# NazirNayal8/RbA

Measured on AMD Instinct MI355X. Metric: images/sec @1024x2048 Swin-B-1dl (RbA inference hot path), higher is better.
Workload: dtype f32 (f16x3 split-MFMA GEMMs, fp32 accumulate)

## Files before the change

include/rba_hip.h:

```cpp
#ifndef RBA_HIP_H
#define RBA_HIP_H

#include <stdint.h>

#ifdef __cplusplus
extern "C" {
#endif

int rba_hip_version(void);

int rba_set_concurrent_streams(int n);

int rba_reduce_f32(const float* mask, const float* cls_prob, float* rba, float* sem_seg, int32_t* argmax,
                   int Q, int K, int64_t HW, int score_mode, void* stream);

int rba_reduce_ws_f32(const float* mask, const float* cls_prob, float* rba, float* sem_seg, int32_t* argmax, int Q, int K,
                      int64_t HW, int score_mode, void* workspace, void* stream);

int rba_reduce_up4_f32(const float* mask_lowres, const float* cls_prob, float* rba, float* sem_seg,
                       int32_t* argmax, int Q, int K, int h, int w, int crop_h, int crop_w, int score_mode, void* stream);

int rba_reduce_bwd_workspace_f32(int Q, int K, int64_t HW, int64_t* bytes);
int rba_reduce_bwd_f32(const float* mask, const float* cls_prob, const float* grad_score,
                       float* grad_mask , float* grad_prob ,
                       int Q, int K, int64_t HW, int score_mode,
                       void* workspace, int64_t workspace_bytes, void* stream);

int rba_sem_seg_bwd_f32(const float* mask, const float* cls_prob, const float* grad_sem ,
                        float* grad_mask , float* grad_prob ,
                        int Q, int K, int64_t HW, void* workspace, int64_t workspace_bytes, void* stream);

int rba_resample_bilinear_f32(const float* in, const float* add, float* out, int C, int h, int w, int H, int W,
                              void* stream);

int rba_ms_deform_attn_fwd_f32(const float* value, const int64_t* spatial_shapes, const int64_t* level_start_index,
                               const float* sampling_loc, const float* attn_weight, float* out,
                               int N, int S, int M, int D, int L, int Lq, int P, void* stream);
int rba_ms_deform_attn_fwd_f64(const double* value, const int64_t* spatial_shapes, const int64_t* level_start_index,
                               const double* sampling_loc, const double* attn_weight, double* out,
                               int N, int S, int M, int D, int L, int Lq, int P, void* stream);

int rba_ms_deform_attn_bwd_f32(const float* value, const int64_t* spatial_shapes, const int64_t* level_start_index,
                               const float* sampling_loc, const float* attn_weight, const float* grad_out,
                               float* grad_value, float* grad_sampling_loc, float* grad_attn_weight,
                               int N, int S, int M, int D, int L, int Lq, int P, void* stream);
int rba_ms_deform_attn_bwd_f64(const double* value, const int64_t* spatial_shapes, const int64_t* level_start_index,
                               const double* sampling_loc, const double* attn_weight, const double* grad_out,
                               double* grad_value, double* grad_sampling_loc, double* grad_attn_weight,
                               int N, int S, int M, int D, int L, int Lq, int P, void* stream);

int rba_msda_prepare_f32(const float* raw, const float* reference_points, const int64_t* spatial_shapes, float* loc, float* attw,
                         int64_t rows, int M, int L, int P, void* stream);

int rba_msda_fused_f32(const float* value, const int64_t* spatial_shapes, const int64_t* level_start_index, const float* raw,
                       const float* reference_points, float* out, int N, int S, int M, int D, int L, int Lq, int P, void* stream);

int64_t rba_masked_xattn_workspace_bytes(int B, int Q, int S, int nH);
int rba_masked_xattn_f32(const float* q, const float* k, const float* v, const float* mask_logits, float* out,
                         float* workspace, int B, int Q, int S, int nH, int hd, void* stream);

int rba_mask_logits_f32(const float* embed, const float* feat, float* out, int B, int Q, int C, int64_t N,
                        void* stream);
int rba_mask_logits_f16x3_f32(const float* embed, const float* feat, float* out, int B, int Q, int C, int64_t N,
                              void* stream);

int rba_mask_logits_bwd_workspace_f32(int B, int Q, int C, int64_t N, int64_t* bytes);
int rba_mask_logits_bwd_f32(const float* embed, const float* feat, const float* grad_out,
                            float* grad_embed , float* grad_feat ,
                            int B, int Q, int C, int64_t N, void* workspace, int64_t workspace_bytes, void* stream);

int rba_point_sample_f32(const float* planes, const int64_t* plane_index , const float* coords, float* out,
                         int64_t num_planes, int N, int h, int w, int P, int shared_coords, void* stream);

int rba_mask_point_loss_fwd_f32(const float* pred_masks, const int64_t* plane_index, const float* coords, const float* labels,
                                float* sums, float* losses, int64_t num_planes, int N, int h, int w, int P, float num_masks, void* stream);
int rba_mask_point_loss_bwd_f32(const float* pred_masks, const int64_t* plane_index, const float* coords, const float* labels,
                                const float* sums, const float* grad_loss_mask , const float* grad_loss_dice ,
                                float* grad_masks, int64_t num_planes, int N, int h, int w, int P, float num_masks, void* stream);

int rba_match_cost_workspace_f32(int Q, int T, int P, int64_t* bytes);
int rba_match_cost_f32(const float* pred_masks, const float* tgt_masks, const float* coords, const float* cls_prob, const int64_t* tgt_ids,
                       float* cost, int Q, int T, int P, int h, int w, int H, int W, int K1, float w_mask, float w_class, float w_dice,
                       void* workspace, int64_t workspace_bytes, void* stream);

int rba_outlier_tail_workspace_f32(int B, int H, int W, int64_t* bytes);
int rba_outlier_tail_fwd_f32(const float* score, const void* labels, int label_bytes , int B, int h, int w, int H, int W, int func,
                             float thr_in, float thr_out, float* workspace, float* loss ,
                             float* stats , void* stream);
int rba_outlier_tail_bwd_f32(const float* score, const void* labels, int label_bytes, int B, int h, int w, int H, int W, int func,
                             float thr_in, float thr_out, const float* stats, const float* grad_loss ,
                             float* grad_score , void* stream);

int rba_dense_hybrid_loss_workspace_f32(int B, int H, int W, int64_t* bytes);
int rba_dense_hybrid_loss_fwd_f32(const float* sem, const float* ood, const void* labels, int label_bytes , int B, int K, int h, int w,
                                  int H, int W, float beta, float* workspace, float* losses , float* stats ,
                                  float* lse , void* stream);
int rba_dense_hybrid_loss_bwd_f32(const float* sem, const float* ood, const void* labels, int label_bytes, const float* lse, int B, int K, int h,
                                  int w, int H, int W, float beta, const float* stats, const float* grad_loss ,
                                  float* grad_sem , float* grad_ood , void* stream);

int rba_gambler_loss_workspace_f32(int B, int H, int W, int64_t* bytes);
int rba_gambler_loss_fwd_f32(const float* sem, const void* labels, int label_bytes , int B, int K, int h, int w, int H, int W,
                             float ood_reg, float* workspace, float* reward , float* losses , float* stats ,
                             float* R , void* stream);
int rba_gambler_loss_bwd_f32(const float* sem, const void* labels, int label_bytes, const float* R, int B, int K, int h, int w, int H, int W,
                             float ood_reg, const float* stats, const float* grad_loss , float* grad_R ,
                             float* grad_reward , float* grad_sem , void* stream);

int rba_gaussian_blur_planes_f32(const float* in, float* out, int B, int H, int W, int kernel_size, float sigma, void* stream);
int rba_gaussian_blur_planes_adjoint_f32(const float* grad_out, float* grad_in, int B, int H, int W, int kernel_size, float sigma, void* stream);

int rba_score_reg_workspace_f32(int B, int h, int w, int H, int W, int64_t* bytes);
int rba_score_reg_fwd_f32(const float* score, const void* labels , int label_bytes, int B, int h, int w, int H, int W, float* workspace,
                          float* losses , float* stats , void* stream);
int rba_score_reg_bwd_f32(const float* score, const void* labels , int label_bytes, int B, int h, int w, int H, int W,
                          const float* stats, const float* grad_smooth , const float* grad_sparse ,
                          float* grad_score , void* stream);

int rba_swin_window_attn_f32(const float* qkv, const float* qkv_bias, const float* bias, const float* bias_frag,
                             float* out, int B, int H, int W, int nH, int hd, int ws, int shift, void* stream);
int64_t rba_swin_bias_fragments_elems(int nH, int ws);
int rba_swin_bias_fragments_f32(const float* bias, float* frag, int nH, int ws, void* stream);

int64_t rba_group_norm_workspace_bytes(int B, int C, int HW, int G);
int rba_group_norm_f32(const float* x, const float* gamma, const float* beta, float* y, float* workspace,
                       int B, int C, int HW, int G, float eps, int relu, void* stream);

int64_t rba_group_norm_nhwc_workspace_bytes(int B, int P, int C, int G);
int rba_group_norm_nhwc_f32(const float* x, const float* gamma, const float* beta, float* y, float* workspace, int B, int P, int C,
                            int G, float eps, int relu, void* stream);
int rba_resample_bilinear_nhwc_f32(const float* in, const float* add, float* out, int C, int h, int w, int H, int W, void* stream);

int rba_add_layer_norm_f32(const float* x, const float* t, const float* t_bias, const float* gamma, const float* beta,
                           float* sum_out, float* y, int64_t rows, int C, float eps, void* stream);

int rba_merge_layer_norm_f32(const float* x, const float* gamma, const float* beta, float* y, int B, int H, int W, int Cin, float eps,
                             void* stream);

int rba_skinny_linear_f32(const float* x, const float* weight, const float* bias, float* out, int M, int N, int K,
                          int relu, void* stream);
int rba_skinny_linear_add_f32(const float* x, const float* x_add, int add_cols, const float* weight, const float* bias, float* out,
                              int M, int N, int K, int relu, int seg_n, void* stream);

int rba_split_weight_bf16x3(const float* weight, void* packed, int N, int K, void* stream);
int rba_split_linear_f32(const float* x, const void* weight_packed, const float* bias, float* out, int64_t M, int N, int K,
                         int act, void* stream);

int rba_split_weight_f16x2(const float* weight, void* packed, int N, int K, void* stream);
int rba_split_linear_f16x3_f32(const float* x, const void* weight_packed, const float* bias, float* out, int64_t M, int N, int K,
                               int act, void* stream);
int rba_split_linear_f16x3_res_f32(const float* x, const void* weight_packed, const float* bias, const float* residual, float* out,
                                   int64_t M, int N, int K, void* stream);

int rba_add_layer_norm_frag_f32(const float* x, const float* t, const float* t_bias, const float* gamma, const float* beta,
                                float* sum_out, void* y_frag, int64_t rows, int C, float eps, void* stream);
int rba_split_linear_f16x3_frag_f32(const void* x_frag, const void* weight_packed, const float* bias, const float* residual, float* out,
                                    int64_t M, int N, int K, int act, void* stream);
int rba_swin_window_attn_split_out_f32(const float* qkv, const float* qkv_bias, const float* bias_frag, void* out_frag, int B, int H, int W,
                                       int nH, int hd, int ws, int shift, void* stream);
int rba_swin_attn_block_supported(int C, int ws);
int64_t rba_swin_attn_block_weight_bytes(int C);
int rba_swin_attn_block_pack_f32(const float* qkv_weight, const float* proj_weight, void* image, int C, void* stream);
int rba_swin_attn_block_f32(float* x, float* y2, const float* norm1_weight, const float* norm1_bias, float eps1, const void* weight_image,
                            const float* qkv_bias, const float* bias_frag, const float* proj_bias, const float* norm2_weight,
                            const float* norm2_bias, float eps2, int B, int H, int W, int C, int ws, int shift, void* stream);
int rba_swin_attn_qkv_supported(int C, int ws);
int rba_swin_attn_qkv_split_out_f32(const float* x, void* out_frag, const float* norm1_weight, const float* norm1_bias, float eps1,
                                    const void* weight_image, const float* qkv_bias, const float* bias_frag, int B, int H, int W, int C, int ws,
                                    int shift, void* stream);
int rba_resample_bilinear_nhwc_split_out_f32(const float* in, const float* add, void* out_frag, int C, int h, int w, int H, int W,
                                             int64_t row0, void* stream);

int rba_resample_bilinear_nhwc_gn_f32(const float* in, const float* in_mr, const float* in_gamma, const float* in_beta, int in_relu,
                                      const float* add, const float* add_mr, const float* add_gamma, const float* add_beta, void* out,
                                      int split_out, int C, int G, int h, int w, int H, int W, int64_t row0, void* stream);
int rba_group_norm_nhwc_stats_f32(const float* x, float* mr, float* workspace, int B, int P, int C, int G, float eps, void* stream);
int rba_conv3x3_nhwc_f16x3_split_in_f32(const void* x_frag, const void* weight_packed, const float* bias, float* out, int B, int H, int W,
                                        int C, int N, void* stream);
int rba_swin_mlp_fused_f16x3_f32(const float* x, const void* w1_packed, const float* b1, const void* w2_packed, const float* b2,
                                 const float* residual, float* out, int64_t M, int C, int HID, void* stream);
int rba_swin_mlp_fused_ln_f16x3_f32(float* x, const float* norm_weight, const float* norm_bias, float eps, const void* w1_packed, const float* b1,
                                    const void* w2_packed, const float* b2, int64_t M, int C, int HID, void* stream);
int rba_split_linear_f16x3_gelu_split_out(const void* x, int x_is_split, const void* weight_packed, const float* bias, void* out_frag,
                                          int64_t M, int N, int K, void* stream);

int rba_split_linear_nchw_out_f32(const float* x, const void* weight_packed, const float* bias, float* out, int64_t M, int N,
                                  int K, int rows_per_image, void* stream);

int rba_split_linear_nchw_out_f16x3_f32(const float* x, const void* weight_packed, const float* bias, float* out, int64_t M, int N, int K,
                                        int rows_per_image, void* stream);

int rba_split_linear_nchw_out_gn_f16x3_f32(const float* x, const float* mr, const float* gamma, const float* beta, int G, int relu,
                                           const void* weight_packed, const float* bias, float* out, int64_t M, int N, int K,
                                           int rows_per_image, void* stream);

int rba_split_linear_nchw_out_gn_rows_f16x3_f32(const float* x, const float* mr, const float* gamma, const float* beta, int G, int relu,
                                                const void* weight_packed, int64_t weight_image_stride, const float* bias,
                                                int bias_image_stride, const int32_t* row_index, float* out, int B, int P, int R, int N,
                                                int K, void* stream);
int rba_compose_query_operand_f16x2(const float* embed, const float* weight, const float* bias, void* packed, float* bias_q, int B, int Q,
                                    int C, int K, void* stream);

int rba_conv3x3_nhwc_f32(const float* x, const void* weight_packed, const float* bias, float* out, int B, int H, int W, int C,
                         int N, void* stream);

int rba_conv3x3_nhwc_f16x3_f32(const float* x, const void* weight_packed, const float* bias, float* out, int B, int H, int W, int C,
                               int N, void* stream);

int rba_split_linear_f16x3_gn_moments_f32(const float* x, const void* weight_packed, const float* bias, float* out, int64_t M, int N, int K,
                                          int rows_per_image, int G, float* moments, void* stream);
int rba_conv3x3_nhwc_f16x3_split_in_gn_moments_f32(const void* x_frag, const void* weight_packed, const float* bias, float* out, int B, int H,
                                                   int W, int C, int N, int G, float* moments, void* stream);
int rba_group_norm_nhwc_merge_f32(const float* moments, float* mr, int B, int G, int splits, float eps, void* stream);

int rba_patch_im2col_u8(const uint8_t* image, float* out, int h, int w, int Hp, int Wp, const float* mean, const float* std, void* stream);
int rba_patch_im2col_f32(const float* image, float* out, int h, int w, int Hp, int Wp, const float* mean, const float* std, void* stream);

int rba_gaussian_blur_f32(const float* in, float* out, int H, int W, int kernel_size, float sigma, void* stream);

int rba_quad_mean_f32(const float* v, float* out, int64_t rows, int S, void* stream);
int rba_softmax_drop_last_f32(const float* logits, float* prob, int64_t rows, int K1, void* stream);

int rba_threshold_u8(const float* score, uint8_t* out, int64_t n, float threshold, void* stream);
int rba_morph3x3_u8(const uint8_t* in, uint8_t* out, int H, int W, int dilate, void* stream);
int rba_ccl4_roots_i32(const uint8_t* mask, int32_t* roots, int H, int W, void* stream);

int rba_bn_relu_conv1x1_f32(const float* x, const float* scale, const float* shift, const float* weight, const float* bias, float* out,
                            int B, int C, int O, int64_t P, void* stream);
int rba_resample_bilinear_ac_f32(const float* x, float* out, int C, int h, int w, int H, int W, void* stream);

typedef struct {
  const float* x_add;
  const void* packed;
  const float* bias;
  float* out;
  int N;
  int ld_out;
  int act;
} rba_token_linear_problem;
int rba_token_linear_pack_f16x2(const float* weight, void* packed, int N, int K, void* stream);
int rba_token_linear_f32(const float* x, const float* x_add, const void* packed, const float* bias, const float* residual,
                         const float* ln_weight, const float* ln_bias, float ln_eps, float* out, int64_t M, int N, int K, int act,
                         void* stream);
int rba_token_linear_multi_f32(const float* x, const rba_token_linear_problem* problems, int n_problems, int64_t M, int K, void* stream);

#define RBA_TTA_MAX_VIEWS 16
typedef struct {
  const float* sem[RBA_TTA_MAX_VIEWS];
  int h[RBA_TTA_MAX_VIEWS];
  int w[RBA_TTA_MAX_VIEWS];
  int flip[RBA_TTA_MAX_VIEWS];
} rba_tta_views;
int rba_tta_merge_f32(const rba_tta_views* views , int A, int K, int H, int W, int score_mode, float* score, float* sem_seg ,
                      int32_t* argmax , void* stream);

int rba_resize_u8_pil_bilinear(const uint8_t* in , uint8_t* out , uint8_t* tmp , int C, int h, int w,
                               int H, int W, const int32_t* kx, const int32_t* bx, int ksize_x, const int32_t* ky, const int32_t* by, int ksize_y,
                               int flip, void* stream);

int rba_confusion_accum(const int32_t* pred, const void* gt, int gt_bytes , int64_t n_pixels, int K,
                        int ignore_label , const uint8_t* lut , int64_t* conf ,
                        int64_t* bad , void* stream);

typedef struct {
  int enabled;
  int brightness;
  float beta;
  int order;
  int contrast;
  float contrast_alpha;
  int saturation;
  float saturation_alpha;
  int hue;
  int hue_delta;
} rba_train_view_color;
typedef struct {
  const uint8_t* img;
  const uint8_t* lab;
  const uint8_t* lut;
  const uint8_t* obj;
  const uint8_t* objmask;
  const int32_t* kx;
  const int32_t* bx;
  const int32_t* ky;
  const int32_t* by;
  const int32_t* ny;
  const int32_t* nx;
  uint8_t* image;
  int64_t* sem_seg;
  int64_t* outlier_mask;
  int32_t* hist;
  int h, w, bh, bw, py, px, new_h, new_w, ksize_x, ksize_y, y0, x0, ch, cw, flip, pad_h, pad_w, ignore_label, ood_label;
  rba_train_view_color color;
} rba_train_view;
int rba_train_view_u8(const rba_train_view* view , void* stream);

#ifdef __cplusplus
}
#endif
#endif
```

rba_amd/_lib.py:

```python
import ctypes
import os

_HERE = os.path.dirname(os.path.abspath(__file__))
LIB_PATH = os.environ.get("RBA_HIP_LIB") or os.path.join(_HERE, "csrc", "librba_hip.so")
KNOBS_LIB_PATH = os.path.join(_HERE, "csrc", "librba_hip_knobs.so")

_i = ctypes.c_int
_i64 = ctypes.c_int64
_vp = ctypes.c_void_p

SIGNATURES = {
    "rba_hip_version": [],
    "rba_set_concurrent_streams": [_i],
    "rba_reduce_f32": [_vp, _vp, _vp, _vp, _vp, _i, _i, _i64, _i, _vp],
    "rba_reduce_ws_f32": [_vp, _vp, _vp, _vp, _vp, _i, _i, _i64, _i, _vp, _vp],
    "rba_reduce_up4_f32": [_vp, _vp, _vp, _vp, _vp, _i, _i, _i, _i, _i, _i, _i, _vp],
    "rba_reduce_bwd_workspace_f32": [_i, _i, _i64, _vp],
    "rba_reduce_bwd_f32": [_vp, _vp, _vp, _vp, _vp, _i, _i, _i64, _i, _vp, _i64, _vp],
    "rba_sem_seg_bwd_f32": [_vp, _vp, _vp, _vp, _vp, _i, _i, _i64, _vp, _i64, _vp],
    "rba_resample_bilinear_f32": [_vp, _vp, _vp, _i, _i, _i, _i, _i, _vp],
    "rba_ms_deform_attn_fwd_f32": [_vp, _vp, _vp, _vp, _vp, _vp, _i, _i, _i, _i, _i, _i, _i, _vp],
    "rba_ms_deform_attn_fwd_f64": [_vp, _vp, _vp, _vp, _vp, _vp, _i, _i, _i, _i, _i, _i, _i, _vp],
    "rba_ms_deform_attn_bwd_f32": [_vp, _vp, _vp, _vp, _vp, _vp, _vp, _vp, _vp, _i, _i, _i, _i, _i, _i, _i, _vp],
    "rba_ms_deform_attn_bwd_f64": [_vp, _vp, _vp, _vp, _vp, _vp, _vp, _vp, _vp, _i, _i, _i, _i, _i, _i, _i, _vp],
    "rba_msda_prepare_f32": [_vp, _vp, _vp, _vp, _vp, _i64, _i, _i, _i, _vp],
    "rba_resample_bilinear_nhwc_gn_f32": [_vp, _vp, _vp, _vp, _i, _vp, _vp, _vp, _vp, _vp, _i, _i, _i, _i, _i, _i, _i, _i64, _vp],
    "rba_group_norm_nhwc_stats_f32": [_vp, _vp, _vp, _i, _i, _i, _i, ctypes.c_float, _vp],
    "rba_msda_fused_f32": [_vp, _vp, _vp, _vp, _vp, _vp, _i, _i, _i, _i, _i, _i, _i, _vp],
    "rba_masked_xattn_workspace_bytes": [_i, _i, _i, _i],
    "rba_masked_xattn_f32": [_vp, _vp, _vp, _vp, _vp, _vp, _i, _i, _i, _i, _i, _vp],
    "rba_mask_logits_f32": [_vp, _vp, _vp, _i, _i, _i, _i64, _vp],
    "rba_mask_logits_f16x3_f32": [_vp, _vp, _vp, _i, _i, _i, _i64, _vp],
    "rba_mask_logits_bwd_workspace_f32": [_i, _i, _i, _i64, _vp],
    "rba_mask_logits_bwd_f32": [_vp, _vp, _vp, _vp, _vp, _i, _i, _i, _i64, _vp, _i64, _vp],
    "rba_point_sample_f32": [_vp, _vp, _vp, _vp, _i64, _i, _i, _i, _i, _i, _vp],
    "rba_mask_point_loss_fwd_f32": [_vp, _vp, _vp, _vp, _vp, _vp, _i64, _i, _i, _i, _i, ctypes.c_float, _vp],
    "rba_mask_point_loss_bwd_f32": [_vp, _vp, _vp, _vp, _vp, _vp, _vp, _vp, _i64, _i, _i, _i, _i, ctypes.c_float, _vp],
    "rba_match_cost_workspace_f32": [_i, _i, _i, _vp],
    "rba_match_cost_f32": [_vp, _vp, _vp, _vp, _vp, _vp, _i, _i, _i, _i, _i, _i, _i, _i, ctypes.c_float, ctypes.c_float, ctypes.c_float, _vp, _i64, _vp],
    "rba_outlier_tail_workspace_f32": [_i, _i, _i, _vp],
    "rba_outlier_tail_fwd_f32": [_vp, _vp, _i, _i, _i, _i, _i, _i, _i, ctypes.c_float, ctypes.c_float, _vp, _vp, _vp, _vp],
    "rba_outlier_tail_bwd_f32": [_vp, _vp, _i, _i, _i, _i, _i, _i, _i, ctypes.c_float, ctypes.c_float, _vp, _vp, _vp, _vp],
    "rba_dense_hybrid_loss_workspace_f32": [_i, _i, _i, _vp],
    "rba_dense_hybrid_loss_fwd_f32": [_vp, _vp, _vp, _i, _i, _i, _i, _i, _i, _i, ctypes.c_float, _vp, _vp, _vp, _vp, _vp],
    "rba_dense_hybrid_loss_bwd_f32": [_vp, _vp, _vp, _i, _vp, _i, _i, _i, _i, _i, _i, ctypes.c_float, _vp, _vp, _vp, _vp, _vp],
    "rba_gambler_loss_workspace_f32": [_i, _i, _i, _vp],
    "rba_gambler_loss_fwd_f32": [_vp, _vp, _i, _i, _i, _i, _i, _i, _i, ctypes.c_float, _vp, _vp, _vp, _vp, _vp, _vp],
    "rba_gambler_loss_bwd_f32": [_vp, _vp, _i, _vp, _i, _i, _i, _i, _i, _i, ctypes.c_float, _vp, _vp, _vp, _vp, _vp, _vp],
    "rba_gaussian_blur_planes_f32": [_vp, _vp, _i, _i, _i, _i, ctypes.c_float, _vp],
    "rba_gaussian_blur_planes_adjoint_f32": [_vp, _vp, _i, _i, _i, _i, ctypes.c_float, _vp],
    "rba_score_reg_workspace_f32": [_i, _i, _i, _i, _i, _vp],
    "rba_score_reg_fwd_f32": [_vp, _vp, _i, _i, _i, _i, _i, _i, _vp, _vp, _vp, _vp],
    "rba_score_reg_bwd_f32": [_vp, _vp, _i, _i, _i, _i, _i, _i, _vp, _vp, _vp, _vp, _vp],
    "rba_tta_merge_f32": [_vp, _i, _i, _i, _i, _i, _vp, _vp, _vp, _vp],
    "rba_resize_u8_pil_bilinear": [_vp, _vp, _vp, _i, _i, _i, _i, _i, _vp, _vp, _i, _vp, _vp, _i, _i, _vp],
    "rba_confusion_accum": [_vp, _vp, _i, _i64, _i, _i, _vp, _vp, _vp, _vp],
    "rba_train_view_u8": [_vp, _vp],
    "rba_swin_window_attn_f32": [_vp, _vp, _vp, _vp, _vp, _i, _i, _i, _i, _i, _i, _i, _vp],
    "rba_swin_window_attn_split_out_f32": [_vp, _vp, _vp, _vp, _i, _i, _i, _i, _i, _i, _i, _vp],
    "rba_swin_bias_fragments_elems": [_i, _i],
    "rba_swin_attn_block_supported": [_i, _i],
    "rba_swin_attn_block_weight_bytes": [_i],
    "rba_swin_attn_qkv_supported": [_i, _i],
    "rba_swin_attn_qkv_split_out_f32": [_vp, _vp, _vp, _vp, ctypes.c_float, _vp, _vp, _vp, _i, _i, _i, _i, _i, _i, _vp],
    "rba_swin_attn_block_pack_f32": [_vp, _vp, _vp, _i, _vp],
    "rba_swin_attn_block_f32": [_vp, _vp, _vp, _vp, ctypes.c_float, _vp, _vp, _vp, _vp, _vp, _vp, ctypes.c_float, _i, _i, _i, _i, _i, _i, _vp],
    "rba_swin_bias_fragments_f32": [_vp, _vp, _i, _i, _vp],
    "rba_skinny_linear_f32": [_vp, _vp, _vp, _vp, _i, _i, _i, _i, _vp],
    "rba_skinny_linear_add_f32": [_vp, _vp, _i, _vp, _vp, _vp, _i, _i, _i, _i, _i, _vp],
    "rba_split_weight_bf16x3": [_vp, _vp, _i, _i, _vp],
    "rba_split_linear_f32": [_vp, _vp, _vp, _vp, _i64, _i, _i, _i, _vp],
    "rba_split_weight_f16x2": [_vp, _vp, _i, _i, _vp],
    "rba_split_linear_f16x3_f32": [_vp, _vp, _vp, _vp, _i64, _i, _i, _i, _vp],
    "rba_split_linear_f16x3_res_f32": [_vp, _vp, _vp, _vp, _vp, _i64, _i, _i, _vp],
    "rba_split_linear_f16x3_frag_f32": [_vp, _vp, _vp, _vp, _vp, _i64, _i, _i, _i, _vp],
    "rba_swin_mlp_fused_f16x3_f32": [_vp, _vp, _vp, _vp, _vp, _vp, _vp, _i64, _i, _i, _vp],
    "rba_swin_mlp_fused_ln_f16x3_f32": [_vp, _vp, _vp, ctypes.c_float, _vp, _vp, _vp, _vp, _i64, _i, _i, _vp],
    "rba_split_linear_f16x3_gelu_split_out": [_vp, _i, _vp, _vp, _vp, _i64, _i, _i, _vp],
    "rba_split_linear_nchw_out_f32": [_vp, _vp, _vp, _vp, _i64, _i, _i, _i, _vp],
    "rba_split_linear_nchw_out_f16x3_f32": [_vp, _vp, _vp, _vp, _i64, _i, _i, _i, _vp],
    "rba_split_linear_f16x3_gn_moments_f32": [_vp, _vp, _vp, _vp, _i64, _i, _i, _i, _i, _vp, _vp],
    "rba_conv3x3_nhwc_f16x3_split_in_gn_moments_f32": [_vp, _vp, _vp, _vp, _i, _i, _i, _i, _i, _i, _vp, _vp],
    "rba_group_norm_nhwc_merge_f32": [_vp, _vp, _i, _i, _i, ctypes.c_float, _vp],
    "rba_split_linear_nchw_out_gn_f16x3_f32": [_vp, _vp, _vp, _vp, _i, _i, _vp, _vp, _vp, _i64, _i, _i, _i, _vp],
    "rba_split_linear_nchw_out_gn_rows_f16x3_f32": [_vp, _vp, _vp, _vp, _i, _i, _vp, _i64, _vp, _i, _vp, _vp, _i, _i, _i, _i, _i, _vp],
    "rba_compose_query_operand_f16x2": [_vp, _vp, _vp, _vp, _vp, _i, _i, _i, _i, _vp],
    "rba_conv3x3_nhwc_f32": [_vp, _vp, _vp, _vp, _i, _i, _i, _i, _i, _vp],
    "rba_conv3x3_nhwc_f16x3_f32": [_vp, _vp, _vp, _vp, _i, _i, _i, _i, _i, _vp],
    "rba_conv3x3_nhwc_f16x3_split_in_f32": [_vp, _vp, _vp, _vp, _i, _i, _i, _i, _i, _vp],
    "rba_resample_bilinear_nhwc_split_out_f32": [_vp, _vp, _vp, _i, _i, _i, _i, _i, _i64, _vp],
    "rba_patch_im2col_u8": [_vp, _vp, _i, _i, _i, _i, _vp, _vp, _vp],
    "rba_patch_im2col_f32": [_vp, _vp, _i, _i, _i, _i, _vp, _vp, _vp],
    "rba_group_norm_nhwc_workspace_bytes": [_i, _i, _i, _i],
    "rba_group_norm_nhwc_f32": [_vp, _vp, _vp, _vp, _vp, _i, _i, _i, _i, ctypes.c_float, _i, _vp],
    "rba_resample_bilinear_nhwc_f32": [_vp, _vp, _vp, _i, _i, _i, _i, _i, _vp],
    "rba_bn_relu_conv1x1_f32": [_vp, _vp, _vp, _vp, _vp, _vp, _i, _i, _i, _i64, _vp],
    "rba_resample_bilinear_ac_f32": [_vp, _vp, _i, _i, _i, _i, _i, _vp],
    "rba_gaussian_blur_f32": [_vp, _vp, _i, _i, _i, ctypes.c_float, _vp],
    "rba_quad_mean_f32": [_vp, _vp, _i64, _i, _vp],
    "rba_softmax_drop_last_f32": [_vp, _vp, _i64, _i, _vp],
    "rba_threshold_u8": [_vp, _vp, _i64, ctypes.c_float, _vp],
    "rba_morph3x3_u8": [_vp, _vp, _i, _i, _i, _vp],
    "rba_ccl4_roots_i32": [_vp, _vp, _i, _i, _vp],
    "rba_add_layer_norm_f32": [_vp, _vp, _vp, _vp, _vp, _vp, _vp, _i64, _i, ctypes.c_float, _vp],
    "rba_add_layer_norm_frag_f32": [_vp, _vp, _vp, _vp, _vp, _vp, _vp, _i64, _i, ctypes.c_float, _vp],
    "rba_merge_layer_norm_f32": [_vp, _vp, _vp, _vp, _i, _i, _i, _i, ctypes.c_float, _vp],
    "rba_group_norm_workspace_bytes": [_i, _i, _i, _i],
    "rba_group_norm_f32": [_vp, _vp, _vp, _vp, _vp, _i, _i, _i, _i, ctypes.c_float, _i, _vp],
    "rba_token_linear_pack_f16x2": [_vp, _vp, _i, _i, _vp],
    "rba_token_linear_f32": [_vp, _vp, _vp, _vp, _vp, _vp, _vp, ctypes.c_float, _vp, _i64, _i, _i, _i, _vp],
    "rba_token_linear_multi_f32": [_vp, _vp, _i, _i64, _i, _vp],
}

class TokenLinearProblem(ctypes.Structure):
    _fields_ = [("x_add", ctypes.c_void_p), ("packed", ctypes.c_void_p), ("bias", ctypes.c_void_p), ("out", ctypes.c_void_p),
                ("N", ctypes.c_int), ("ld_out", ctypes.c_int), ("act", ctypes.c_int)]


TTA_MAX_VIEWS = 16


class TtaViews(ctypes.Structure):
    _fields_ = [("sem", ctypes.c_void_p * TTA_MAX_VIEWS), ("h", ctypes.c_int * TTA_MAX_VIEWS), ("w", ctypes.c_int * TTA_MAX_VIEWS),
                ("flip", ctypes.c_int * TTA_MAX_VIEWS)]


class TrainViewColor(ctypes.Structure):
    _fields_ = [("enabled", ctypes.c_int), ("brightness", ctypes.c_int), ("beta", ctypes.c_float), ("order", ctypes.c_int),
                ("contrast", ctypes.c_int), ("contrast_alpha", ctypes.c_float), ("saturation", ctypes.c_int), ("saturation_alpha", ctypes.c_float),
                ("hue", ctypes.c_int), ("hue_delta", ctypes.c_int)]


TRAIN_VIEW_POINTERS = ("img", "lab", "lut", "obj", "objmask", "kx", "bx", "ky", "by", "ny", "nx", "image", "sem_seg", "outlier_mask", "hist")
TRAIN_VIEW_INTS = ("h", "w", "bh", "bw", "py", "px", "new_h", "new_w", "ksize_x", "ksize_y", "y0", "x0", "ch", "cw", "flip", "pad_h", "pad_w",
                   "ignore_label", "ood_label")


class TrainView(ctypes.Structure):
    _fields_ = ([(n, ctypes.c_void_p) for n in TRAIN_VIEW_POINTERS] + [(n, ctypes.c_int) for n in TRAIN_VIEW_INTS] + [("color", TrainViewColor)])


EXPECTED_ABI = 191

_lib = None


class RbaHipError(RuntimeError):
    pass


def load():
    global _lib
    if _lib is not None:
        return _lib
    _lib = _open(LIB_PATH)
    return _lib


_handles = {}


def _open(path):
    if path in _handles:
        return _handles[path]
    import torch
    if not os.path.exists(path):
        raise RbaHipError(
            f"{path} not found: build it with `python -m rba_amd.csrc.build` (hipcc --offload-arch=gfx950; --knobs for the knobs build). "
            "rba_amd has no CPU or PyTorch fallback for its HIP kernels.")
    lib = ctypes.CDLL(path)
    for name, argtypes in SIGNATURES.items():
        try:
            fn = getattr(lib, name)
        except AttributeError as e:
            raise RbaHipError(f"{path} does not export {name}; rebuild it") from e
        fn.argtypes = argtypes
        fn.restype = ctypes.c_int64 if name.endswith(("_bytes", "_elems")) else ctypes.c_int
    abi = int(lib.rba_hip_version())
    if abi != EXPECTED_ABI:
        raise RbaHipError(f"{path} has ABI version {abi}, these bindings are written for {EXPECTED_ABI}; rebuild it "
                          "(python -m rba_amd.csrc.build)")
    _handles[path] = lib
    return lib


class use_library:

    def __init__(self, path):
        self.path = path

    def __enter__(self):
        global _lib
        self.prev = _lib
        _lib = _open(self.path)
        return _lib

    def __exit__(self, *exc):
        global _lib
        _lib = self.prev
        return False


def knob(name):
    try:
        return ctypes.c_int.in_dll(load(), name)
    except ValueError as e:
        raise RbaHipError(f"{name} is a compile-time constant in the product library: run on the knobs build (RBA_HIP_LIB={KNOBS_LIB_PATH} or "
                          "rba_amd._lib.use_library(KNOBS_LIB_PATH); python -m rba_amd.csrc.build --knobs)") from e


def hip_error_string(code: int) -> str:
    try:
        hip = ctypes.CDLL("libamdhip64.so")
        hip.hipGetErrorString.restype = ctypes.c_char_p
        hip.hipGetErrorString.argtypes = [ctypes.c_int]
        return hip.hipGetErrorString(code).decode()
    except Exception:
        return "hipError"


def check(code: int, what: str):
    if code != 0:
        raise RbaHipError(f"{what} failed: hipError {code} ({hip_error_string(code)})")
```

rba_amd/csrc/build.py:

```python
import os
import subprocess
import sys
from concurrent.futures import ThreadPoolExecutor

HERE = os.path.dirname(os.path.abspath(__file__))
SOURCES = ["rba_reduce.hip", "rba_reduce_bwd.hip", "resample.hip", "ms_deform_attn.hip", "ms_deform_attn_bwd.hip", "masked_xattn.hip", "mask_logits.hip", "mask_logits_bwd.hip", "point_loss.hip", "outlier_tail.hip", "dense_hybrid_loss.hip", "pebal_loss.hip", "tta_merge.hip", "resize_u8.hip", "confusion.hip", "train_view.hip",
           "swin_window_attn.hip", "swin_attn_block.hip", "group_norm.hip", "layer_norm.hip", "skinny_linear.hip", "split_linear.hip", "split_linear_dma.hip", "split_linear_gnf.hip", "gaussian_blur.hip", "open_panoptic.hip", "dense_hybrid.hip", "patch_embed.hip", "token_linear.hip", "decoder_small.hip"]
HEADERS = ["common.h", "knobs.h", "bilinear_ac.h", "rba_reduce_kernels.h", "split_linear_dma.h", "split_linear_h3.h", "split_linear_h3q.h", "mlp_fused_h3.h", "swin_window_attn_h3.h", "swin_attn_block.h",
           os.path.join("..", "..", "include", "rba_hip.h")]
TUNE_SOURCES = [os.path.join("tune", "rba_reduce_tune.hip"), os.path.join("tune", "split_linear_tune.hip"), os.path.join("tune", "split_linear_ws.hip"), os.path.join("tune", "mlp_fused_h1.hip"), os.path.join("tune", "k5_timing.hip"), os.path.join("tune", "k5_wpe_ab.hip"), os.path.join("tune", "k5_wpe_plain.hip"), os.path.join("tune", "k5_persist.hip"), os.path.join("tune", "k7_timing.hip")] + [os.path.join("tune", f"gnf_form{f}_dbg{d}.hip") for f in (0, 1) for d in (0, 1)] + [os.path.join("tune", "gnf_form0_dbg1_unpacked.hip"), os.path.join("tune", "gnf_form1_dbg0_unpacked.hip")]
TUNE_LIB = os.path.join(HERE, "tune", "librba_tune.so")
LIB = os.path.join(HERE, "librba_hip.so")
KNOBS_LIB = os.path.join(HERE, "librba_hip_knobs.so")
KNOBS = ["-DRBA_TUNE_KNOBS"]
OBJ = os.path.join(HERE, "build")
HIPCC = os.environ.get("HIPCC", "/opt/rocm/bin/hipcc")
FLAGS = ["--offload-arch=gfx950", "-O3", "-std=c++17", "-fPIC", "-ffp-contract=fast", "-Wno-unused-result"]
NO_PACKED_FP32 = ["-Xclang", "-target-feature", "-Xclang", "-packed-fp32-ops"]
MFMA_SOURCES = ({"split_linear.hip", "split_linear_dma.hip", "mask_logits.hip", "mask_logits_bwd.hip", "masked_xattn.hip", "skinny_linear.hip"}
                if os.environ.get("RBA_NO_PACKED_FP32") == "1" else set())
UNPACKED_ALWAYS = {"split_linear_gnf.hip", "ms_deform_attn_bwd.hip", "point_loss.hip", "outlier_tail.hip", "dense_hybrid_loss.hip"}
UNPACKED_SOURCES = MFMA_SOURCES | UNPACKED_ALWAYS


def _run(cmd):
    r = subprocess.run(cmd, cwd=HERE, stderr=subprocess.PIPE, text=True)
    err = "\n".join(ln for ln in r.stderr.splitlines() if "not a recognized feature for this target" not in ln)
    if err.strip():
        print(err, file=sys.stderr, flush=True)
    if r.returncode:
        raise subprocess.CalledProcessError(r.returncode, cmd)


def _stale(target, deps) -> bool:
    if not os.path.exists(target):
        return True
    t = os.path.getmtime(target)
    return any(os.path.getmtime(d) > t for d in deps)


def stale() -> bool:
    return _stale(LIB, [os.path.join(HERE, f) for f in SOURCES + HEADERS])


def build(force: bool = False, verbose: bool = True, knobs: bool = False) -> str:
    lib = KNOBS_LIB if knobs else LIB
    if not force and not _stale(lib, [os.path.join(HERE, f) for f in SOURCES + HEADERS]):
        return lib
    obj_dir = os.path.join(OBJ, "knobs") if knobs else OBJ
    os.makedirs(obj_dir, exist_ok=True)
    hdrs = [os.path.join(HERE, h) for h in HEADERS]

    def compile_one(src):
        s, o = os.path.join(HERE, src), os.path.join(obj_dir, src.replace(".hip", ".o"))
        if force or _stale(o, [s] + hdrs):
            cmd = [HIPCC] + FLAGS + (KNOBS if knobs else []) + (NO_PACKED_FP32 if src in UNPACKED_SOURCES else []) + ["-c", s, "-o", o]
            if verbose:
                print(" ".join(cmd), flush=True)
            _run(cmd)
        return o

    with ThreadPoolExecutor(max_workers=min(8, os.cpu_count() or 1)) as ex:
        objs = list(ex.map(compile_one, SOURCES))
    _link_and_gate(objs, lib, verbose)
    return lib


def _link_and_gate(objs, lib, verbose):
    tmp = lib + ".unscanned"
    cmd = [HIPCC, "--offload-arch=gfx950", "-shared", "-fPIC"] + objs + ["-o", tmp]
    if verbose:
        print(" ".join(cmd), flush=True)
    subprocess.run(cmd, check=True, cwd=HERE)
    try:
        from . import isa_hazards
    except ImportError:
        sys.path.insert(0, HERE)
        import isa_hazards
    try:
        r = isa_hazards.gate(tmp)
    except Exception:
        os.remove(tmp)
        raise
    if verbose:
        print(f"isa_hazards: {os.path.basename(lib)}: {r['code_objects']} code objects clean (rules D, T, P)", flush=True)
    os.replace(tmp, lib)


def build_knobs(force: bool = False, verbose: bool = True) -> str:
    return build(force=force, verbose=verbose, knobs=True)


def build_tune(force: bool = False, verbose: bool = True) -> str:
    deps = [os.path.join(HERE, f) for f in TUNE_SOURCES + HEADERS + [os.path.join("tune", "split_linear_experiments.h"), os.path.join("tune", "rba_reduce_experiments.h")]]
    if not force and not _stale(TUNE_LIB, deps):
        return TUNE_LIB
    os.makedirs(OBJ, exist_ok=True)
    objs = []
    for src in TUNE_SOURCES:
        o = os.path.join(OBJ, "tune_" + os.path.basename(src).replace(".hip", ".o"))
        cmd = [HIPCC] + FLAGS + KNOBS + (NO_PACKED_FP32 if (MFMA_SOURCES and "split_linear" in src) or src.endswith("split_linear_ws.hip") or src.endswith("_unpacked.hip") or (src.endswith("mlp_fused_h1.hip") and os.environ.get("RBA_MLP1_UNPACKED") == "1") else []) + ["-c", os.path.join(HERE, src), "-o", o]
        if verbose:
            print(" ".join(cmd), flush=True)
        _run(cmd)
        objs.append(o)
    cmd = [HIPCC, "--offload-arch=gfx950", "-shared", "-fPIC"] + objs + ["-o", TUNE_LIB]
    if verbose:
        print(" ".join(cmd), flush=True)
    subprocess.run(cmd, check=True, cwd=HERE)
    return TUNE_LIB


if __name__ == "__main__":
    print(build(force="--force" in sys.argv))
    if "--knobs" in sys.argv:
        print(build_knobs(force="--force" in sys.argv))
    if "--tune" in sys.argv:
        print(build_tune(force="--force" in sys.argv))
```

rba_amd/csrc/layer_norm.hip:

```cpp
#include "common.h"
#include "../../include/rba_hip.h"

namespace {

struct MergeGeom {
  int H, W, Cin;
};

template <int G, int NV, bool MERGE = false, bool FRAG = false, int WAVES = 4>
__global__ __launch_bounds__(64 * WAVES) void add_layer_norm_kernel(const float* x, const float* __restrict__ t,
                                                             const float* __restrict__ tb, const float* __restrict__ gamma,
                                                             const float* __restrict__ beta, float* sum_out ,
                                                             float* __restrict__ y, int64_t rows, int C, float eps,
                                                             MergeGeom mg = MergeGeom{0, 0, 0}) {
  constexpr int RPW = 64 / G;
  const int lane = threadIdx.x & 63, sub = lane % G, rsel = lane / G;
  const int64_t row = ((int64_t)blockIdx.x * WAVES + (threadIdx.x >> 6)) * RPW + rsel;
  constexpr bool TR = FRAG && WAVES == 8 && G == 64;
  __shared__ __attribute__((aligned(16))) rba_u32x4 tr_lds[TR ? NV * 64 * 8 : 1];
  const bool rvalid = row < rows;
  const int64_t base = (rvalid ? row : 0) * C;
  const int nv4 = C >> 2;
  int mi = 0, mj = 0;
  int64_t mb = 0;
  if (MERGE) {
    const int H2 = (mg.H + 1) >> 1, W2 = (mg.W + 1) >> 1;
    const int64_t r = rvalid ? row : 0;
    const int64_t bimg = r / ((int64_t)H2 * W2);
    const int rem = (int)(r - bimg * H2 * W2);
    mi = rem / W2;
    mj = rem - mi * W2;
    mb = bimg * mg.H * mg.W;
  }
  constexpr bool EARLY = NV <= 2;
  f32x4 v[NV], g4[EARLY ? NV : 1], b4[EARLY ? NV : 1];
  float sum = 0.f;
#pragma unroll
  for (int j = 0; j < (EARLY ? NV : 0); ++j) {
    const int c4 = sub + j * G;
    g4[j] = b4[j] = (f32x4){0.f, 0.f, 0.f, 0.f};
    if (c4 < nv4) {
      g4[j] = *reinterpret_cast<const f32x4*>(gamma + 4 * c4);
      b4[j] = *reinterpret_cast<const f32x4*>(beta + 4 * c4);
    }
  }
#pragma unroll
  for (int j = 0; j < NV; ++j) {
    const int c4 = sub + j * G;
    f32x4 a = {0.f, 0.f, 0.f, 0.f};
    if (c4 < nv4) {
      if (MERGE) {
        const int seg = (4 * c4) / mg.Cin, off = 4 * c4 - seg * mg.Cin;
        const int si = 2 * mi + (seg & 1), sj = 2 * mj + (seg >> 1);
        if (si < mg.H && sj < mg.W) a = *reinterpret_cast<const f32x4*>(x + (mb + (int64_t)si * mg.W + sj) * mg.Cin + off);
      } else {
        a = *reinterpret_cast<const f32x4*>(x + base + 4 * c4);
      }
      if (t) a += *reinterpret_cast<const f32x4*>(t + base + 4 * c4);
      if (tb) a += *reinterpret_cast<const f32x4*>(tb + 4 * c4);
      sum += (a.x + a.y) + (a.z + a.w);
    }
    v[j] = a;
  }
#pragma unroll
  for (int o = G / 2; o > 0; o >>= 1) sum += __shfl_xor(sum, o, RBA_WAVE);
  const float mean = sum / (float)C;
  float sq = 0.f;
#pragma unroll
  for (int j = 0; j < NV; ++j) {
    const int c4 = sub + j * G;
    if (c4 < nv4) {
      const f32x4 d = v[j] - mean;
      sq += (d.x * d.x + d.y * d.y) + (d.z * d.z + d.w * d.w);
    }
  }
#pragma unroll
  for (int o = G / 2; o > 0; o >>= 1) sq += __shfl_xor(sq, o, RBA_WAVE);
  const float rstd = 1.0f / sqrtf(sq / (float)C + eps);
  if (!TR && !rvalid) return;
#pragma unroll
  for (int j = 0; j < NV; ++j) {
    const int c4 = sub + j * G;
    if (c4 < nv4) {
      if (sum_out && rvalid) *reinterpret_cast<f32x4*>(sum_out + base + 4 * c4) = v[j];
      const f32x4 gj = EARLY ? g4[EARLY ? j : 0] : *reinterpret_cast<const f32x4*>(gamma + 4 * c4);
      const f32x4 bj = EARLY ? b4[EARLY ? j : 0] : *reinterpret_cast<const f32x4*>(beta + 4 * c4);
      const f32x4 o = (v[j] - mean) * rstd * gj + bj;
      if (FRAG) {
        uint32_t h[2], l[2];
        rba_split_f16x2(o.x, o.y, h[0], l[0]);
        rba_split_f16x2(o.z, o.w, h[1], l[1]);
        const bool odd = c4 & 1;
        const uint32_t s0 = odd ? h[0] : l[0], s1 = odd ? h[1] : l[1];
        const uint32_t r0 = __builtin_amdgcn_mov_dpp(s0, 0xB1, 0xf, 0xf, true), r1 = __builtin_amdgcn_mov_dpp(s1, 0xB1, 0xf, 0xf, true);
        const rba_u32x4 piece = odd ? (rba_u32x4){r0, r1, l[0], l[1]} : (rba_u32x4){h[0], h[1], r0, r1};
        const int k8 = c4 >> 1;
        if (TR) {
          const int pcol = (((k8 >> 2) * 4 + (k8 & 1) * 2 + (odd ? 1 : 0)) << 1) + ((k8 >> 1) & 1);
          const int r8 = threadIdx.x >> 6;
          tr_lds[pcol * 8 + (r8 ^ (pcol & 7))] = piece;
        } else {
          const int64_t off = ((row >> 5) * (int64_t)(C >> 5) + (k8 >> 2)) * 4096 + ((k8 & 1) * 2 + (odd ? 1 : 0)) * 1024 +
                              (((k8 >> 1) & 1) * 32 + (int)(row & 31)) * 16;
          *reinterpret_cast<rba_u32x4*>(reinterpret_cast<char*>(y) + off) = piece;
        }
      } else {
        *reinterpret_cast<f32x4*>(y + base + 4 * c4) = o;
      }
    }
  }
  if (TR) {
    __syncthreads();
    const int64_t row0 = (int64_t)blockIdx.x * 8;
    char* img = reinterpret_cast<char*>(y) + ((row0 >> 5) * (int64_t)(C >> 5)) * 4096 + (int)(row0 & 31) * 16;
    const int npc = nv4;
    for (int u = threadIdx.x; u < npc * 8; u += 64 * WAVES) {
      const int pcol = u >> 3, r8 = u & 7;
      const int x = pcol >> 1;
      if (row0 + r8 < rows)
        *reinterpret_cast<rba_u32x4*>(img + (int64_t)(x >> 2) * 4096 + (x & 3) * 1024 + (pcol & 1) * 512 + r8 * 16) = tr_lds[pcol * 8 + (r8 ^ (pcol & 7))];
    }
  }
}

template <int G, int NV, bool FRAG = false>
int launch(const float* x, const float* t, const float* tb, const float* gamma, const float* beta, float* sum_out, float* y,
           int64_t rows, int C, float eps, hipStream_t st) {
  const int64_t rpb = 4 * (64 / G);
  const int64_t blocks = (rows + rpb - 1) / rpb;
  if (blocks > 0x7fffffffLL) return (int)hipErrorInvalidValue;
  hipLaunchKernelGGL((add_layer_norm_kernel<G, NV, false, FRAG>), dim3((unsigned)blocks), dim3(256), 0, st, x, t, tb, gamma, beta, sum_out, y,
                     rows, C, eps);
  return rba_launch_status();
}

template <int NV>
int launch_frag8(const float* x, const float* t, const float* tb, const float* gamma, const float* beta, float* sum_out, float* y,
                 int64_t rows, int C, float eps, hipStream_t st) {
  const int64_t blocks = (rows + 7) / 8;
  if (blocks > 0x7fffffffLL) return (int)hipErrorInvalidValue;
  hipLaunchKernelGGL((add_layer_norm_kernel<64, NV, false, true, 8>), dim3((unsigned)blocks), dim3(512), 0, st, x, t, tb, gamma, beta, sum_out,
                     y, rows, C, eps);
  return rba_launch_status();
}

template <int G, int NV>
int launch_merge(const float* x, const float* gamma, const float* beta, float* y, int64_t rows, int C, float eps, MergeGeom mg,
                 hipStream_t st) {
  const int64_t rpb = 4 * (64 / G);
  const int64_t blocks = (rows + rpb - 1) / rpb;
  if (blocks > 0x7fffffffLL) return (int)hipErrorInvalidValue;
  hipLaunchKernelGGL((add_layer_norm_kernel<G, NV, true>), dim3((unsigned)blocks), dim3(256), 0, st, x, nullptr, nullptr, gamma, beta, nullptr,
                     y, rows, C, eps, mg);
  return rba_launch_status();
}

}

extern "C" int rba_merge_layer_norm_f32(const float* x, const float* gamma, const float* beta, float* y, int B, int H, int W, int Cin,
                                        float eps, void* stream) {
  RBA_CHECK_ARG(B >= 0 && H >= 1 && W >= 1 && Cin >= 4 && Cin % 4 == 0 && 4 * Cin <= 8192);
  if (B == 0) return 0;
  RBA_CHECK_ARG(x && gamma && beta && y);
  RBA_CHECK_ARG((((uintptr_t)x | (uintptr_t)gamma | (uintptr_t)beta | (uintptr_t)y) & 15) == 0);
  rba_begin();
  hipStream_t st = (hipStream_t)stream;
  const int C = 4 * Cin, nv4 = C / 4;
  const int64_t rows = (int64_t)B * ((H + 1) / 2) * ((W + 1) / 2);
  const MergeGeom mg{H, W, Cin};
#define RBA_L(G, NV) return launch_merge<G, NV>(x, gamma, beta, y, rows, C, eps, mg, st)
  if (nv4 <= 16) RBA_L(16, 1);
  if (nv4 <= 32) RBA_L(32, 1);
  if (nv4 <= 64) RBA_L(64, 1);
  if (nv4 <= 128) RBA_L(64, 2);
  if (nv4 <= 256) RBA_L(64, 4);
  if (nv4 <= 512) RBA_L(64, 8);
  if (nv4 <= 1024) RBA_L(64, 16);
  RBA_L(64, 32);
#undef RBA_L
}

extern "C" int rba_add_layer_norm_f32(const float* x, const float* t, const float* t_bias, const float* gamma, const float* beta,
                                      float* sum_out, float* y, int64_t rows, int C, float eps, void* stream) {
  RBA_CHECK_ARG(rows >= 0 && C >= 4 && C % 4 == 0 && C <= 8192);
  if (rows == 0) return 0;
  RBA_CHECK_ARG(x && gamma && beta && y);
  RBA_CHECK_ARG((((uintptr_t)x | (uintptr_t)t | (uintptr_t)t_bias | (uintptr_t)gamma | (uintptr_t)beta | (uintptr_t)sum_out |
                  (uintptr_t)y) & 15) == 0);
  rba_begin();
  hipStream_t st = (hipStream_t)stream;
  const int nv4 = C / 4;
#define RBA_L(G, NV) return launch<G, NV>(x, t, t_bias, gamma, beta, sum_out, y, rows, C, eps, st)
  if (nv4 <= 16) RBA_L(16, 1);
  if (nv4 <= 32) RBA_L(32, 1);
  if (nv4 <= 64) RBA_L(64, 1);
  if (nv4 <= 128) RBA_L(64, 2);
  if (nv4 <= 256) RBA_L(64, 4);
  if (nv4 <= 512) RBA_L(64, 8);
  if (nv4 <= 1024) RBA_L(64, 16);
  RBA_L(64, 32);
#undef RBA_L
}

extern "C" int rba_add_layer_norm_frag_f32(const float* x, const float* t, const float* t_bias, const float* gamma, const float* beta,
                                           float* sum_out, void* y_frag, int64_t rows, int C, float eps, void* stream) {
  RBA_CHECK_ARG(rows >= 0 && C >= 32 && C % 32 == 0 && C <= 8192);
  if (rows == 0) return 0;
  RBA_CHECK_ARG(x && gamma && beta && y_frag);
  RBA_CHECK_ARG((((uintptr_t)x | (uintptr_t)t | (uintptr_t)t_bias | (uintptr_t)gamma | (uintptr_t)beta | (uintptr_t)sum_out |
                  (uintptr_t)y_frag) & 15) == 0);
  rba_begin();
  hipStream_t st = (hipStream_t)stream;
  const int nv4 = C / 4;
  float* y = reinterpret_cast<float*>(y_frag);
  if (nv4 > 64 && nv4 <= 128) return launch_frag8<2>(x, t, t_bias, gamma, beta, sum_out, y, rows, C, eps, st);
  if (nv4 > 128 && nv4 <= 256) return launch_frag8<4>(x, t, t_bias, gamma, beta, sum_out, y, rows, C, eps, st);
  if (nv4 > 256 && nv4 <= 512) return launch_frag8<8>(x, t, t_bias, gamma, beta, sum_out, y, rows, C, eps, st);
#define RBA_L(G, NV) return launch<G, NV, true>(x, t, t_bias, gamma, beta, sum_out, y, rows, C, eps, st)
  if (nv4 <= 16) RBA_L(16, 1);
  if (nv4 <= 32) RBA_L(32, 1);
  if (nv4 <= 64) RBA_L(64, 1);
  if (nv4 <= 128) RBA_L(64, 2);
  if (nv4 <= 256) RBA_L(64, 4);
  if (nv4 <= 512) RBA_L(64, 8);
  if (nv4 <= 1024) RBA_L(64, 16);
  RBA_L(64, 32);
#undef RBA_L
}
```

rba_amd/csrc/split_linear_gnf.hip:

```cpp
#include "split_linear_h3.h"

extern "C" int rba_split_linear_nchw_out_gn_f16x3_f32(const float* x, const float* mr, const float* gamma, const float* beta, int G, int relu,
                                                      const void* weight_packed, const float* bias, float* out, int64_t M, int N, int K,
                                                      int rows_per_image, void* stream) {
  RBA_CHECK_ARG(N >= 1 && rows_per_image >= 1 && G >= 1 && (K % G) == 0 && ((K / G) % 4) == 0);
  RBA_GEMM_PROLOGUE(M, K, x && mr && gamma && beta && weight_packed && out && (M % rows_per_image) == 0 && (rows_per_image % 128) == 0, x, weight_packed, out,
                    gamma, beta);
  H3Args a{x, reinterpret_cast<const u32x4_t*>(weight_packed), bias, out, M, N, K, (hipStream_t)stream};
  a.rows_per_image = rows_per_image;
  a.gn = GnFold{mr, gamma, beta, G, K / G, relu ? 1 : 0};
  return rba_gemm_status(h3_wide(M, N) ? launch_h3l<0, 4, H3_NCHW | H3_GNF>(a) : launch_h3l<0, 2, H3_NCHW | H3_GNF>(a));
}

extern "C" int rba_split_linear_nchw_out_gn_rows_f16x3_f32(const float* x, const float* mr, const float* gamma, const float* beta, int G, int relu,
                                                           const void* weight_packed, int64_t weight_image_stride, const float* bias, int bias_image_stride,
                                                           const int32_t* row_index, float* out, int B, int P, int R, int N, int K, void* stream) {
  RBA_CHECK_ARG(B >= 0 && N >= 1 && P >= 1 && R >= 1 && G >= 1 && (K % G) == 0 && ((K / G) % 4) == 0);
  RBA_CHECK_ARG(weight_image_stride >= 0 && (weight_image_stride % 16) == 0 && bias_image_stride >= 0 && (row_index || R == P));
  const int64_t M = (int64_t)B * R;
  RBA_GEMM_PROLOGUE(M, K, x && mr && gamma && beta && weight_packed && out && (P % 128) == 0 && (R % 128) == 0 && (int64_t)P * K < (int64_t)1 << 30, x,
                    weight_packed, out, gamma, beta);
  H3Args a{x, reinterpret_cast<const u32x4_t*>(weight_packed), bias, out, M, N, K, (hipStream_t)stream};
  a.rows_per_image = R;
  a.gn = GnFold{mr, gamma, beta, G, K / G, relu ? 1 : 0};
  a.rw = H3Rows{row_index, P, bias_image_stride, weight_image_stride};
  const bool per_image = weight_image_stride != 0 || bias_image_stride != 0, wide = h3_wide(M, N);
  constexpr unsigned F = H3_NCHW | H3_GNF;
  if (row_index && per_image) return rba_gemm_status(wide ? launch_h3l<0, 4, F | H3_ROWIDX | H3_PERIMG>(a) : launch_h3l<0, 2, F | H3_ROWIDX | H3_PERIMG>(a));
  if (row_index) return rba_gemm_status(wide ? launch_h3l<0, 4, F | H3_ROWIDX>(a) : launch_h3l<0, 2, F | H3_ROWIDX>(a));
  if (per_image) return rba_gemm_status(wide ? launch_h3l<0, 4, F | H3_PERIMG>(a) : launch_h3l<0, 2, F | H3_PERIMG>(a));
  return rba_gemm_status(wide ? launch_h3l<0, 4, F>(a) : launch_h3l<0, 2, F>(a));
}
```

rba_amd/csrc/split_linear_h3.h:

```cpp
#pragma once
#include <type_traits>

#include "split_linear_dma.h"

RBA_KNOB_EXTERN(rba_k6_stagger, 0);

namespace {

typedef _Float16 f16x8_t __attribute__((ext_vector_type(8)));

__device__ __forceinline__ void split_h3(const f32x4 u, const f32x4 v, f16x8_t& h, f16x8_t& l) {
  const float x[8] = {u.x, u.y, u.z, u.w, v.x, v.y, v.z, v.w};
  u32x4_t hp, lp;
#pragma unroll
  for (int i = 0; i < 4; ++i) {
    uint32_t a, r;
    rba_split_f16x2(x[2 * i], x[2 * i + 1], a, r);
    hp[i] = a;
    lp[i] = r;
  }
  h = __builtin_bit_cast(f16x8_t, hp);
  l = __builtin_bit_cast(f16x8_t, lp);
}

__device__ __forceinline__ f32x2 gelu_erf2(f32x2 v) {
  const f32x2 a = {fabsf(v.x), fabsf(v.y)};
  const f32x2 d = a * 0.23164189f + 1.0f;
  const f32x2 t = {__builtin_amdgcn_rcpf(d.x), __builtin_amdgcn_rcpf(d.y)};
  f32x2 p = t * 0.5307027145f + -0.7265760135f;
  p = p * t + 0.7107068705f;
  p = p * t + -0.142248368f;
  p = p * t + 0.127414796f;
  const f32x2 u = a * 0.8493218003f;
  const f32x2 s = -u * u;
  const f32x2 ex = {__builtin_amdgcn_exp2f(s.x), __builtin_amdgcn_exp2f(s.y)};
  const f32x2 q = p * t * ex;
  const f32x2 r = (v + a) * 0.5f;
  return r - a * q;
}

#ifndef RBA_H3_HELPERS_ONLY
__global__ void split_weight_f16x2_kernel(const float* __restrict__ w, u32x4_t* __restrict__ packed, int N, int K) {
  const int S = K >> 4;
  const int64_t total = (int64_t)((N + 127) >> 7) * S * 256;
  for (int64_t i = (int64_t)blockIdx.x * blockDim.x + threadIdx.x; i < total; i += (int64_t)gridDim.x * blockDim.x) {
    const int slot = (int)(i & 1), r = (int)((i >> 1) & 127);
    const int64_t ts = i >> 8;
    const int s = (int)(ts % S), nt = (int)(ts / S);
    const int h = slot ^ ((r >> 3) & 1);
    const int k0 = 32 * (s >> 1) + 16 * h + 8 * (s & 1);
    const int n = nt * 128 + r;
    f16x8_t p0, p1;
    if (n < N) {
      const f32x4* src = reinterpret_cast<const f32x4*>(w + (int64_t)n * K + k0);
      split_h3(src[0], src[1], p0, p1);
    } else {
#pragma unroll
      for (int e = 0; e < 8; ++e) p0[e] = p1[e] = (_Float16)0.f;
    }
    u32x4_t* dst = packed + ts * 512 + r * 2 + slot;
    dst[0] = __builtin_bit_cast(u32x4_t, p0);
    dst[256] = __builtin_bit_cast(u32x4_t, p1);
  }
}

#endif

struct GnMoments {
  float* ws;
  int G, cpg, P;
};
template <int ACT, int CT, int PROBE, bool RES, bool GNM = false>
__device__ __forceinline__ void h3_epilogue(const f32x16_t (&accm)[CT], const f32x16_t (&accl)[CT], const float* __restrict__ bias,
                                            float* C, const float* R, int M, int N, int m0, int n0, int BM, int BN, int wave, int l31,
                                            int lh, GnMoments gm = GnMoments{nullptr, 1, 1, 128}, float* sh = nullptr) {
  const bool interior = m0 + BM <= M && n0 + BN <= N;
  if (GNM) __syncthreads();
#pragma unroll
  for (int j = 0; j < CT; ++j) {
    const int col = n0 + 32 * j + l31;
    const float bv = (bias && col < N) ? bias[col] : 0.f;
    const int rbase = m0 + 32 * wave + 4 * lh;
    float* dst = C + (int64_t)rbase * N + col;
    f32x16_t res;
    if (RES) {
      const float* src = R + (int64_t)rbase * N + col;
#pragma unroll
      for (int r = 0; r < 16; ++r) {
        const int ro = 8 * (r >> 2) + (r & 3);
        res[r] = (interior || (col < N && rbase + ro < M)) ? src[(int64_t)ro * N] : 0.f;
      }
    }
    f32x16_t v;
#pragma unroll
    for (int r = 0; r < 16; r += 2) {
      f32x2 y = (f32x2){accl[j][r], accl[j][r + 1]} * 0.00048828125f + (f32x2){accm[j][r], accm[j][r + 1]};
      if (RES) y = (f32x2){res[r], res[r + 1]} + y;
      y = y + bv;
      if (ACT == 1) y = gelu_erf2(y);
      if (ACT == 2) y = (f32x2){rba_relu(y.x), rba_relu(y.y)};
      v[r] = y.x;
      v[r + 1] = y.y;
    }
    if (GNM) {
      float sm = 0.f, sq = 0.f;
#pragma unroll
      for (int r = 0; r < 16; ++r) {
        sm += v[r];
        sq = fmaf(v[r], v[r], sq);
      }
      sm += __shfl_xor(sm, 32, 64);
      sq += __shfl_xor(sq, 32, 64);
      for (int o = 1; o < gm.cpg; o <<= 1) {
        sm += __shfl_xor(sm, o, 64);
        sq += __shfl_xor(sq, o, 64);
      }
      if (lh == 0 && (l31 & (gm.cpg - 1)) == 0) {
        float* d = sh + ((wave * (BN / gm.cpg)) + (32 * j + l31) / gm.cpg) * 2;
        d[0] = sm;
        d[1] = sq;
      }
    }
    if (PROBE & 4) {
      float sum = 0.f;
#pragma unroll
      for (int r = 0; r < 16; ++r) sum += v[r];
      if (sum == 1234.5f) dst[0] = sum;
    } else if (interior) {
#pragma unroll
      for (int r = 0; r < 16; ++r) dst[(int64_t)(8 * (r >> 2) + (r & 3)) * N] = v[r];
    } else if (col < N) {
#pragma unroll
      for (int r = 0; r < 16; ++r) {
        const int ro = 8 * (r >> 2) + (r & 3);
        if (rbase + ro < M) dst[(int64_t)ro * N] = v[r];
      }
    }
  }
  if (GNM) {
    __syncthreads();
    const int gpt = BN / gm.cpg, t = 64 * wave + 32 * lh + l31;
    if (t < gpt && m0 < M) {
      double ds = 0, dq = 0;
#pragma unroll
      for (int w = 0; w < 4; ++w) {
        ds += (double)sh[(w * gpt + t) * 2];
        dq += (double)sh[(w * gpt + t) * 2 + 1];
      }
      const double n = 128.0 * gm.cpg, mean = ds / n, m2 = dq - ds * mean;
      const int b = m0 / gm.P, sp = (m0 - b * gm.P) >> 7, splits = gm.P >> 7, g = n0 / gm.cpg + t;
      float* o = gm.ws + (((int64_t)b * gm.G + g) * splits + sp) * 3;
      o[0] = (float)n;
      o[1] = (float)mean;
      o[2] = (float)(m2 > 0 ? m2 : 0);
    }
  }
}

#ifndef RBA_H3_HELPERS_ONLY
template <int CT>
__device__ __forceinline__ void h3_epilogue_nchw(const f32x16_t (&accm)[CT], const f32x16_t (&accl)[CT], const float* __restrict__ bias, float* C,
                                                 int M, int N, int P, int m0, int n0, int wave, int l31, int lh) {
  const bool vec = (P & 3) == 0;
#pragma unroll
  for (int j = 0; j < CT; ++j) {
    const int col = n0 + 32 * j + l31;
    if (col >= N) continue;
    const float bv = bias ? bias[col] : 0.f;
#pragma unroll
    for (int q = 0; q < 4; ++q) {
      const int row = m0 + 32 * wave + 8 * q + 4 * lh;
      if (row >= M) continue;
      f32x4 v;
#pragma unroll
      for (int i = 0; i < 4; ++i) v[i] = fmaf(accl[j][4 * q + i], 0.00048828125f, accm[j][4 * q + i]) + bv;
      if (vec && row + 3 < M) {
        const int b = row / P, p = row - b * P;
        *reinterpret_cast<f32x4*>(C + ((int64_t)b * N + col) * P + p) = v;
      } else {
#pragma unroll
        for (int i = 0; i < 4; ++i)
          if (row + i < M) {
            const int b = (row + i) / P, p = row + i - b * P;
            C[((int64_t)b * N + col) * P + p] = v[i];
          }
      }
    }
  }
}

enum : unsigned {
  H3_TIMING = 1u << 0,
  H3_RES = 1u << 1,
  H3_GNM = 1u << 2,
  H3_CONV = 1u << 3,
  H3_NCHW = 1u << 4,
  H3_GNF = 1u << 5,
  H3_PRE = 1u << 6,
  H3_FOUT = 1u << 7,
  H3_CONVP = 1u << 8,
  H3_OCC1 = 1u << 9,
  H3_KS2 = 1u << 10,
  H3_RS2 = 1u << 11,
  H3_ROWIDX = 1u << 12,
  H3_PERIMG = 1u << 13,
  H3_PROBE_SHIFT = 16,
};
constexpr unsigned h3_probe(int p) { return (unsigned)p << H3_PROBE_SHIFT; }
constexpr int h3_probe_of(unsigned form) { return (int)(form >> H3_PROBE_SHIFT); }
constexpr unsigned H3_FORMS = H3_TIMING | H3_RES, H3L_FORMS = H3_FORMS | H3_GNM | H3_CONV | H3_NCHW | H3_GNF | H3_ROWIDX | H3_PERIMG,
                   H3P_FORMS = H3_FORMS | H3_GNM | H3_PRE | H3_FOUT | H3_CONVP | H3_OCC1 | H3_KS2 | H3_RS2;
constexpr bool h3_form_within(unsigned form, unsigned allowed) { return (form & ~allowed & ((1u << H3_PROBE_SHIFT) - 1)) == 0; }
constexpr int h3_tile_rows(unsigned form) { return (form & H3_RS2) ? 256 : 128; }
constexpr int h3_threads(unsigned form) { return (form & (H3_KS2 | H3_RS2)) ? 512 : 256; }
constexpr int h3_occupancy(unsigned form) { return (form & (H3_KS2 | H3_RS2 | H3_OCC1)) ? 1 : 2; }

template <int ACT, int CT, unsigned FORM = 0>
__global__ __launch_bounds__(256, 2) void split_linear_h3_kernel(const float* __restrict__ A, const u32x4_t* __restrict__ Wp,
                                                                const float* __restrict__ bias, float* C, int M, int N,
                                                                int K, int MT, int NT, unsigned long long* dbg = nullptr,
                                                                const float* R = nullptr) {
  static_assert(h3_form_within(FORM, H3_FORMS), "split_linear_h3_kernel: H3_TIMING, H3_RES, h3_probe()");
  constexpr int PROBE = h3_probe_of(FORM);
  constexpr bool TIMING = FORM & H3_TIMING, RES = FORM & H3_RES;
  unsigned long long tm[4];
  if (TIMING) tm[0] = wall_clock64();
  constexpr int BM = 128, BN = 32 * CT;
  constexpr int SUBW = 4 * BN;
  constexpr int BLK = 2 * SUBW;
  constexpr int UPL = BLK / 256;
  static_assert(BLK % 256 == 0 && 128 % BN == 0, "tile width");
  __shared__ __attribute__((aligned(16))) u32x4_t lds[2 * BLK];

  const int tid = threadIdx.x, lane = tid & 63;
  const int wave = __builtin_amdgcn_readfirstlane(tid >> 6);
  int bid = blockIdx.x;
  const int nb = MT * NT;
  if ((nb & 7) == 0) bid = (bid & 7) * (nb >> 3) + (bid >> 3);
  const int mt = bid / NT, nt = bid - mt * NT;
  const int m0 = mt * BM, n0 = nt * BN;
  const int NB = K >> 5, S16 = K >> 4;
  const int l31 = lane & 31, lh = lane >> 5;

  constexpr int QSTEP = (CT == 4) ? 256 : 512;
  const char* wbase = reinterpret_cast<const char*>(Wp + (int64_t)(n0 >> 7) * S16 * 512 + (n0 & 127) * 2);
  uint32_t woff;
  {
    const int g = tid / SUBW, rem = tid - g * SUBW, p = rem / (2 * BN), rr = rem - p * (2 * BN);
    woff = (uint32_t)(g * 512 + p * 256 + rr) * 16u;
  }
  int row = m0 + 32 * wave + l31;
  row = (row < M ? row : M - 1) - m0;
  const char* xbase = reinterpret_cast<const char*>(A + (int64_t)m0 * K);
  const uint32_t xoff = ((uint32_t)row * (uint32_t)K + 16u * lh) * 4u;

  f32x16_t accm[CT], accl[CT];
#pragma unroll
  for (int j = 0; j < CT; ++j)
#pragma unroll
    for (int r = 0; r < 16; ++r) accm[j][r] = accl[j][r] = 0.f;

  u32x4_t wr[UPL];
  f32x4 xr[2][4];
  const int last = NB - 1;
  auto wload = [&](int c, u32x4_t (&r)[UPL]) {
    const char* src = wbase + (int64_t)(c < last ? c : last) * 16384;
#pragma unroll
    for (int q = 0; q < UPL; ++q) r[q] = *reinterpret_cast<const u32x4_t*>(src + q * (QSTEP * 16) + woff);
  };
  auto xload = [&](int c, f32x4 (&r)[4]) {
    const char* src = xbase + (c < last ? c : last) * 128;
#pragma unroll
    for (int q = 0; q < 4; ++q) r[q] = *reinterpret_cast<const f32x4*>(src + q * 16 + xoff);
  };
  wload(0, wr);
  xload(0, xr[0]);
  xload(1, xr[1]);
#pragma unroll
  for (int q = 0; q < UPL; ++q) lds[tid + 256 * q] = wr[q];
  wload(1, wr);
  asm volatile("s_waitcnt lgkmcnt(0)\n\ts_barrier" ::: "memory");

  const int fb = l31 * 2 + (lh ^ ((l31 >> 3) & 1));
  if (TIMING) tm[1] = wall_clock64();
  auto block = [&](int b, const u32x4_t* img, u32x4_t* nxt, f32x4 (&xc)[4]) {
    if (!(PROBE & 32)) {
#pragma unroll
      for (int q = 0; q < UPL; ++q) nxt[tid + 256 * q] = wr[q];
    }
    if (!(PROBE & 1)) wload(b + 2, wr);
    f16x8_t ah[2], al[2];
    if (PROBE & 16) {
      ah[0] = __builtin_bit_cast(f16x8_t, xc[0]); al[0] = __builtin_bit_cast(f16x8_t, xc[1]);
      ah[1] = __builtin_bit_cast(f16x8_t, xc[2]); al[1] = __builtin_bit_cast(f16x8_t, xc[3]);
    } else {
      split_h3(xc[0], xc[1], ah[0], al[0]);
      split_h3(xc[2], xc[3], ah[1], al[1]);
    }
    if (!(PROBE & 2)) xload(b + 2, xc);
#pragma unroll
    for (int g = 0; g < 2; ++g) {
      __builtin_amdgcn_sched_barrier(0);
      f16x8_t bh[CT], bl[CT];
#pragma unroll
      for (int j = 0; j < CT; ++j) {
        const u32x4_t* im = (PROBE & 8) ? lds : img;
        bh[j] = __builtin_bit_cast(f16x8_t, im[g * SUBW + fb + 64 * j]);
        bl[j] = __builtin_bit_cast(f16x8_t, im[g * SUBW + fb + 2 * BN + 64 * j]);
      }
#pragma unroll
      for (int j = 0; j < CT; ++j) accm[j] = __builtin_amdgcn_mfma_f32_32x32x16_f16(ah[g], bh[j], accm[j], 0, 0, 0);
#pragma unroll
      for (int j = 0; j < CT; ++j) accl[j] = __builtin_amdgcn_mfma_f32_32x32x16_f16(ah[g], bl[j], accl[j], 0, 0, 0);
#pragma unroll
      for (int j = 0; j < CT; ++j) accl[j] = __builtin_amdgcn_mfma_f32_32x32x16_f16(al[g], bh[j], accl[j], 0, 0, 0);
    }
    if (!(PROBE & 64)) asm volatile("s_waitcnt lgkmcnt(0)\n\ts_barrier" ::: "memory");
  };
  int b = 0;
  if (NB & 1) {
    block(0, lds, lds + BLK, xr[0]);
    b = 1;
    for (; b < NB; b += 2) {
      block(b, lds + BLK, lds, xr[1]);
      block(b + 1, lds, lds + BLK, xr[0]);
    }
  } else {
    for (; b < NB; b += 2) {
      block(b, lds, lds + BLK, xr[0]);
      block(b + 1, lds + BLK, lds, xr[1]);
    }
  }

  if (TIMING) tm[2] = wall_clock64();
  h3_epilogue<ACT, CT, PROBE, RES>(accm, accl, bias, C, R, M, N, m0, n0, BM, BN, wave, l31, lh);
  if (TIMING && tid == 0) {
    tm[3] = wall_clock64();
    unsigned xcc;
    asm volatile("s_getreg_b32 %0, hwreg(HW_REG_XCC_ID)" : "=s"(xcc));
    unsigned hw;
    asm volatile("s_getreg_b32 %0, hwreg(HW_REG_HW_ID)" : "=s"(hw));
#pragma unroll
    for (int i = 0; i < 4; ++i) dbg[6 * blockIdx.x + i] = tm[i];
    dbg[6 * blockIdx.x + 4] = xcc;
    dbg[6 * blockIdx.x + 5] = hw;
  }
}

struct ConvShape {
  int H, W, Cin;
};
struct GnFold {
  const float* mr;
  const float* gamma;
  const float* beta;
  int G, cpg, relu;
};
struct H3Rows {
  const int* idx;
  int P;
  int bstride;
  int64_t wstride;
};
template <int ACT, int CT, unsigned FORM = 0>
__global__ __launch_bounds__(256, 2) void split_linear_h3l_kernel(const float* __restrict__ A, const u32x4_t* __restrict__ Wp,
                                                                 const float* __restrict__ bias, float* C, int M, int N,
                                                                 int K, int MT, int NT, unsigned long long* dbg = nullptr,
                                                                 ConvShape cs = ConvShape{0, 0, 0}, const float* R = nullptr, int rows_per_image = 0,
                                                                 GnFold gn = GnFold{nullptr, nullptr, nullptr, 1, 1, 0},
                                                                 GnMoments gm = GnMoments{nullptr, 1, 1, 128}, H3Rows rw = H3Rows{nullptr, 0, 0, 0}) {
  static_assert(h3_form_within(FORM, H3L_FORMS), "split_linear_h3l_kernel: H3_TIMING, H3_RES, H3_GNM, H3_CONV, H3_NCHW, H3_GNF, H3_ROWIDX, H3_PERIMG, h3_probe()");
  constexpr int PROBE = h3_probe_of(FORM);
  constexpr bool TIMING = FORM & H3_TIMING, CONV = FORM & H3_CONV, RES = FORM & H3_RES, NCHW = FORM & H3_NCHW, GNF = FORM & H3_GNF, GNM = FORM & H3_GNM;
  constexpr bool ROWIDX = FORM & H3_ROWIDX, PERIMG = FORM & H3_PERIMG;
  static_assert(!(ROWIDX || PERIMG) || (NCHW && GNF && !CONV && !RES && !GNM), "H3_ROWIDX / H3_PERIMG: forms of the GroupNorm-folded channel-major projection");
  unsigned long long tm[4];
  if (TIMING) tm[0] = wall_clock64();
  constexpr int BM = 128, BN = 32 * CT;
  constexpr int SUBW = 4 * BN;
  constexpr int BLK = 2 * SUBW;
  constexpr int UPL = BLK / 256;
  constexpr int XBLK = BM * 8;
  constexpr int BUF = BLK + XBLK;
  static_assert(BLK % 256 == 0 && 128 % BN == 0, "tile width");
  __shared__ __attribute__((aligned(16))) u32x4_t lds[2 * BUF];

  const int tid = threadIdx.x, lane = tid & 63;
  const int wave = __builtin_amdgcn_readfirstlane(tid >> 6);
  int bid = blockIdx.x;
  const int nb = MT * NT;
  if ((nb & 7) == 0) bid = (bid & 7) * (nb >> 3) + (bid >> 3);
  const int mt = bid / NT, nt = bid - mt * NT;
  const int m0 = mt * BM, n0 = nt * BN;
  const int NB = K >> 5, S16 = K >> 4;
  const int l31 = lane & 31, lh = lane >> 5;

  constexpr int QSTEP = (CT == 4) ? 256 : 512;
  const char* wbase = reinterpret_cast<const char*>(Wp + (int64_t)(n0 >> 7) * S16 * 512 + (n0 & 127) * 2);
  const int img = (ROWIDX || PERIMG) ? m0 / rows_per_image : 0;
  if (PERIMG) {
    wbase += (int64_t)img * rw.wstride;
    if (bias) bias += (int64_t)img * rw.bstride;
  }
  uint32_t woff;
  {
    const int g = tid / SUBW, rem = tid - g * SUBW, p = rem / (2 * BN), rr = rem - p * (2 * BN);
    woff = (uint32_t)(g * 512 + p * 256 + rr) * 16u;
  }
  const char* xbase = reinterpret_cast<const char*>(CONV ? A : ROWIDX ? A + (int64_t)img * rw.P * K : A + (int64_t)m0 * K);
  uint32_t xoff[4];
  int py[4], px[4];
#pragma unroll
  for (int q = 0; q < 4; ++q) {
    int r = m0 + (tid >> 3) + 32 * q;
    r = r < M ? r : M - 1;
    if (CONV) {
      const int pix = r % (cs.H * cs.W);
      py[q] = pix / cs.W;
      px[q] = pix - py[q] * cs.W;
      xoff[q] = ((uint32_t)r * (uint32_t)cs.Cin + 4u * (tid & 7)) * 4u;
    } else if (ROWIDX) {
      int s = rw.idx[r];
      s = s < 0 ? 0 : (s < rw.P ? s : rw.P - 1);
      xoff[q] = ((uint32_t)s * (uint32_t)K + 4u * (tid & 7)) * 4u;
    } else {
      xoff[q] = ((uint32_t)(r - m0) * (uint32_t)K + 4u * (tid & 7)) * 4u;
    }
  }
  const int xdst = BLK + (tid >> 3) * 8 + ((tid & 7) ^ ((tid >> 4) & 7));
  const int frow = 32 * wave + l31;
  const int fa = BLK + frow * 8, fsw = (frow >> 1) & 7;

  f32x16_t accm[CT], accl[CT];
#pragma unroll
  for (int j = 0; j < CT; ++j)
#pragma unroll
    for (int r = 0; r < 16; ++r) accm[j][r] = accl[j][r] = 0.f;

  u32x4_t wr[UPL];
  f32x4 xr[4];
  f32x4 gga = {0.f, 0.f, 0.f, 0.f}, gbe = {0.f, 0.f, 0.f, 0.f};
  float gmean = 0.f, grstd = 0.f;
  const float* gmr = GNF ? gn.mr + (int64_t)(m0 / rows_per_image) * gn.G * 2 : nullptr;
  const int last = NB - 1;
  auto gload = [&](int c) {
    const int cc = c < last ? c : last;
    const char* ws = wbase + (int64_t)cc * 16384;
#pragma unroll
    for (int q = 0; q < UPL; ++q) wr[q] = *reinterpret_cast<const u32x4_t*>(ws + q * (QSTEP * 16) + woff);
    if (GNF) {
      const int ch = cc * 32 + 4 * (tid & 7);
      gga = *reinterpret_cast<const f32x4*>(gn.gamma + ch);
      gbe = *reinterpret_cast<const f32x4*>(gn.beta + ch);
      const int g = ch / gn.cpg;
      gmean = gmr[2 * g];
      grstd = gmr[2 * g + 1];
    }
    if (CONV) {
      const int k0 = cc * 32, tap = k0 / cs.Cin, ch0 = k0 - tap * cs.Cin;
      const int ky = tap / 3, dy = ky - 1, dx = tap - 3 * ky - 1;
      const int delta = ((dy * cs.W + dx) * cs.Cin + ch0) * 4;
#pragma unroll
      for (int q = 0; q < 4; ++q) {
        const bool ok = (unsigned)(py[q] + dy) < (unsigned)cs.H && (unsigned)(px[q] + dx) < (unsigned)cs.W;
        const f32x4 v = *reinterpret_cast<const f32x4*>(xbase + (int64_t)(ok ? delta : ch0 * 4) + xoff[q]);
        xr[q] = ok ? v : (f32x4){0.f, 0.f, 0.f, 0.f};
      }
    } else {
      const char* xs = xbase + cc * 128;
#pragma unroll
      for (int q = 0; q < 4; ++q) xr[q] = *reinterpret_cast<const f32x4*>(xs + xoff[q]);
    }
  };
  f32x4 xst[4];
#if defined(RBA_GNF_DEBUG)
  int gnf_blk = 0;
#endif
  auto lstore = [&](u32x4_t* buf) {
#pragma unroll
    for (int q = 0; q < UPL; ++q) buf[tid + 256 * q] = wr[q];
    if (GNF) {
      f32x4 a, b;
      const float relu_floor = gn.relu ? 0.f : -INFINITY;
      const float poison = (grstd - grstd) + (gmean - gmean);
#pragma unroll
      for (int i = 0; i < 4; ++i) {
        a[i] = gga[i] * grstd;
        b[i] = fmaf(-gmean, a[i], gbe[i]);
      }
#pragma unroll
      for (int q = 0; q < 4; ++q)
#pragma unroll
        for (int i = 0; i < 4; ++i) {
#if defined(RBA_GNF_FORM) && RBA_GNF_FORM == 1
          const float y = fmaf(xr[q][i], a[i], b[i]);
          xst[q][i] = fmaxf(y, relu_floor) + (y - y);
#else
          xst[q][i] = fmaxf(fmaf(xr[q][i], a[i], b[i]), relu_floor) + poison;
#endif
        }
#if defined(RBA_GNF_DEBUG)
      if (dbg && gnf_blk < NB) {
        float* d = reinterpret_cast<float*>(dbg) + (((int64_t)(mt * NT + nt) * NB + gnf_blk) * 256 + tid) * 40;
#pragma unroll
        for (int q = 0; q < 4; ++q) {
          *reinterpret_cast<f32x4*>(d + 4 * q) = xr[q];
          *reinterpret_cast<f32x4*>(d + 16 + 4 * q) = xst[q];
        }
        *reinterpret_cast<f32x4*>(d + 32) = a;
        *reinterpret_cast<f32x4*>(d + 36) = b;
      }
      ++gnf_blk;
#endif
#pragma unroll
      for (int q = 0; q < 4; ++q) buf[xdst + 256 * q] = __builtin_bit_cast(u32x4_t, xst[q]);
    } else {
#pragma unroll
      for (int q = 0; q < 4; ++q) buf[xdst + 256 * q] = __builtin_bit_cast(u32x4_t, xr[q]);
    }
  };
  gload(0);
  lstore(lds);
  gload(1);
  asm volatile("s_waitcnt lgkmcnt(0)\n\ts_barrier" ::: "memory");

  const int fb = l31 * 2 + (lh ^ ((l31 >> 3) & 1));
  if (TIMING) tm[1] = wall_clock64();
  for (int b = 0; b < NB; ++b) {
    const u32x4_t* img = lds + (b & 1) * BUF;
    if (!(PROBE & 32)) lstore(lds + ((b + 1) & 1) * BUF);
    if (!(PROBE & 1)) gload(b + 2);
    f16x8_t ah[2], al[2];
#pragma unroll
    for (int g = 0; g < 2; ++g) {
      const f32x4 u = __builtin_bit_cast(f32x4, img[fa + ((4 * lh + 2 * g) ^ fsw)]);
      const f32x4 v = __builtin_bit_cast(f32x4, img[fa + ((4 * lh + 2 * g + 1) ^ fsw)]);
      if (PROBE & 16) {
        ah[g] = __builtin_bit_cast(f16x8_t, u);
        al[g] = __builtin_bit_cast(f16x8_t, v);
      } else {
        split_h3(u, v, ah[g], al[g]);
      }
    }
#pragma unroll
    for (int g = 0; g < 2; ++g) {
      if (PROBE & 128) __builtin_amdgcn_sched_barrier(0);
      f16x8_t bh[CT], bl[CT];
#pragma unroll
      for (int j = 0; j < CT; ++j) {
        bh[j] = __builtin_bit_cast(f16x8_t, img[g * SUBW + fb + 64 * j]);
        bl[j] = __builtin_bit_cast(f16x8_t, img[g * SUBW + fb + 2 * BN + 64 * j]);
      }
#pragma unroll
      for (int j = 0; j < CT; ++j) accm[j] = __builtin_amdgcn_mfma_f32_32x32x16_f16(ah[g], bh[j], accm[j], 0, 0, 0);
#pragma unroll
      for (int j = 0; j < CT; ++j) accl[j] = __builtin_amdgcn_mfma_f32_32x32x16_f16(ah[g], bl[j], accl[j], 0, 0, 0);
#pragma unroll
      for (int j = 0; j < CT; ++j) accl[j] = __builtin_amdgcn_mfma_f32_32x32x16_f16(al[g], bh[j], accl[j], 0, 0, 0);
    }
    if (!(PROBE & 64)) asm volatile("s_waitcnt lgkmcnt(0)\n\ts_barrier" ::: "memory");
  }

  if (TIMING) tm[2] = wall_clock64();
  if (NCHW) h3_epilogue_nchw<CT>(accm, accl, bias, C, M, N, rows_per_image, m0, n0, wave, l31, lh);
  else h3_epilogue<ACT, CT, PROBE, RES, GNM>(accm, accl, bias, C, R, M, N, m0, n0, BM, BN, wave, l31, lh, gm, reinterpret_cast<float*>(lds));
  if (TIMING && tid == 0) {
    tm[3] = wall_clock64();
#pragma unroll
    for (int i = 0; i < 4; ++i) dbg[6 * blockIdx.x + i] = tm[i];
    dbg[6 * blockIdx.x + 4] = dbg[6 * blockIdx.x + 5] = 0;
  }
}

#endif

template <int ACT, int CT>
__device__ __forceinline__ void h3_epilogue_split(const f32x16_t (&accm)[CT], const f32x16_t (&accl)[CT], const float* __restrict__ bias,
                                                  void* out_frag, int M, int N, int m0, int n0, int wave, int l31, int lh) {
  const int row = m0 + 32 * wave + l31;
  const bool full = m0 + 128 <= M;
  const int NBo = N >> 5;
  char* base = reinterpret_cast<char*>(out_frag) + ((int64_t)((m0 >> 5) + wave) * NBo) * 4096 + l31 * 16 + lh * 1024;
#pragma unroll
  for (int j = 0; j < CT; ++j) {
    const int nj = n0 + 32 * j;
    if (nj >= N) break;
#pragma unroll
    for (int q = 0; q < 4; ++q) {
      const int n = nj + 8 * q + 4 * lh;
      const f32x4 bv = bias ? *reinterpret_cast<const f32x4*>(bias + n) : (f32x4){0.f, 0.f, 0.f, 0.f};
      f32x2 y0 = (f32x2){accl[j][4 * q], accl[j][4 * q + 1]} * 0.00048828125f + (f32x2){accm[j][4 * q], accm[j][4 * q + 1]};
      f32x2 y1 = (f32x2){accl[j][4 * q + 2], accl[j][4 * q + 3]} * 0.00048828125f + (f32x2){accm[j][4 * q + 2], accm[j][4 * q + 3]};
      y0 = y0 + (f32x2){bv.x, bv.y};
      y1 = y1 + (f32x2){bv.z, bv.w};
      if (ACT == 1) {
        y0 = gelu_erf2(y0);
        y1 = gelu_erf2(y1);
      }
      if (ACT == 2) {
        y0 = (f32x2){rba_relu(y0.x), rba_relu(y0.y)};
        y1 = (f32x2){rba_relu(y1.x), rba_relu(y1.y)};
      }
      uint32_t h0, l0, h1, l1;
      rba_split_f16x2(y0.x, y0.y, h0, l0);
      rba_split_f16x2(y1.x, y1.y, h1, l1);
      const auto p0 = __builtin_amdgcn_permlane32_swap(h0, l0, false, false), p1 = __builtin_amdgcn_permlane32_swap(h1, l1, false, false);
      const u32x4_t piece = {p0[0], p1[0], p0[1], p1[1]};
      if (full || row < M) *reinterpret_cast<u32x4_t*>(base + (int64_t)((nj >> 5)) * 4096 + (q & 1) * 2048 + (q >> 1) * 512) = piece;
    }
  }
}

#ifndef RBA_H3_HELPERS_ONLY
template <int ACT, unsigned FORM = 0>
__global__ __launch_bounds__(h3_threads(FORM), h3_occupancy(FORM)) void split_linear_h3p_kernel(const float* __restrict__ A, const u32x4_t* __restrict__ Wp,
                                                                 const float* __restrict__ bias, float* C, int M, int N,
                                                                 int K, int MT, int NT, unsigned long long* dbg = nullptr,
                                                                 const float* R = nullptr, ConvShape cs = ConvShape{0, 0, 0}, int stagger = 0,
                                                                 GnMoments gm = GnMoments{nullptr, 1, 1, 128}) {
  static_assert(h3_form_within(FORM, H3P_FORMS), "split_linear_h3p_kernel: H3_TIMING, H3_RES, H3_GNM, H3_PRE, H3_FOUT, H3_CONVP, H3_OCC1, H3_KS2, H3_RS2, h3_probe()");
  constexpr int PROBE = h3_probe_of(FORM), OCC = (FORM & H3_OCC1) ? 1 : 2, KS = (FORM & H3_KS2) ? 2 : 1, RS = (FORM & H3_RS2) ? 2 : 1;
  constexpr bool TIMING = FORM & H3_TIMING, RES = FORM & H3_RES, PRE = FORM & H3_PRE, FOUT = FORM & H3_FOUT, CONVP = FORM & H3_CONVP, GNM = FORM & H3_GNM;
  static_assert(!GNM || (KS == 1 && !FOUT), "output moments: fp32-row epilogue, one wave set per K");
  unsigned long long tm[4];
  if (TIMING) tm[0] = wall_clock64();
  if (stagger > 0 && blockIdx.x >= 256 && blockIdx.x < 512) {
    const unsigned long long t0 = wall_clock64();
    while (wall_clock64() - t0 < (unsigned long long)stagger) __builtin_amdgcn_s_sleep(8);
  }
  constexpr int CT = 4, BM = 128, BN = 128;
  constexpr int SUBW = 4 * BN, BLK = 2 * SUBW, UPL = BLK / 256;
  __shared__ __attribute__((aligned(16))) u32x4_t lds_all[2 * BLK * KS];

  static_assert(KS * RS <= 2, "K split and row split are alternatives");
  const int tid = threadIdx.x & 255, lane = tid & 63;
  const int ks = KS == 2 ? __builtin_amdgcn_readfirstlane(threadIdx.x >> 8) : 0;
  const int rs = RS == 2 ? __builtin_amdgcn_readfirstlane(threadIdx.x >> 8) : 0;
  const int wtid = RS == 2 ? (int)threadIdx.x : tid;
  constexpr int UPLW = UPL / RS;
  u32x4_t* const lds = lds_all + ks * 2 * BLK;
  const int wave = __builtin_amdgcn_readfirstlane(tid >> 6);
  int bid = blockIdx.x;
  const int nb = MT * NT;
  if ((nb & 7) == 0) bid = (bid & 7) * (nb >> 3) + (bid >> 3);
  const int mt = bid / NT, nt = bid - mt * NT;
  const int m0 = (mt * RS + rs) * BM, n0 = nt * BN;
  const int NB = (K >> 5) / KS, S16 = K >> 4;
  const int l31 = lane & 31, lh = lane >> 5;

  const char* wbase = reinterpret_cast<const char*>(Wp + (int64_t)(n0 >> 7) * S16 * 512);
  const uint32_t woff = (uint32_t)wtid * 16u;
  int row = m0 + 32 * wave + l31;
  row = (row < M ? row : M - 1) - m0;
  const char* xbase = reinterpret_cast<const char*>(A + (int64_t)m0 * K);
  const uint32_t xoff = ((uint32_t)row * (uint32_t)K + 16u * lh) * 4u;

  f32x16_t accm[CT], accl[CT];
#pragma unroll
  for (int j = 0; j < CT; ++j)
#pragma unroll
    for (int r = 0; r < 16; ++r) accm[j][r] = accl[j][r] = 0.f;

  u32x4_t wr[UPLW];
  constexpr bool TWO = OCC == 2 || KS == 2 || RS == 2;
  constexpr bool DEEP = !TWO;
  constexpr bool DIRECT = PRE && TWO;
  f32x4 xr[DEEP ? 2 : 1][4];
  f16x8_t ah[2][2], al[2][2];
  u32x4_t bq[2][4];
  const int last = NB - 1;
  auto bix = [&](int c) { return (c < last ? c : last) * KS + ks; };
  auto wload = [&](int c) {
    const char* src = wbase + (int64_t)bix(c) * 16384;
#pragma unroll
    for (int q = 0; q < UPLW; ++q) wr[q] = *reinterpret_cast<const u32x4_t*>(src + q * (4096 * RS) + woff);
  };
  const int rgrp = min((m0 >> 5) + wave, ((M + 31) >> 5) - 1);
  const char* fbase = reinterpret_cast<const char*>(A) + ((int64_t)rgrp * (K >> 5)) * 4096 + lane * 16;
  auto xload = [&](int c, f32x4 (&d)[4]) {
    if (PRE) {
      const char* src = fbase + bix(c) * 4096;
#pragma unroll
      for (int q = 0; q < 4; ++q) d[q] = *reinterpret_cast<const f32x4*>(src + q * 1024);
      return;
    }
    if (PROBE & 2048) {
      const char* src = xbase + (uint32_t)(32 * wave) * (uint32_t)K * 4u + bix(c) * 4096 + lane * 16;
#pragma unroll
      for (int q = 0; q < 4; ++q) d[q] = *reinterpret_cast<const f32x4*>(src + q * 1024);
      return;
    }
    const char* src = xbase + bix(c) * 128;
#pragma unroll
    for (int q = 0; q < 4; ++q) d[q] = *reinterpret_cast<const f32x4*>(src + q * 16 + xoff);
  };
  const int fb = l31 * 2 + (lh ^ ((l31 >> 3) & 1));
  auto bread = [&](const u32x4_t* img, int j, u32x4_t (&d)[4]) {
    d[0] = img[fb + 64 * j];
    d[1] = img[fb + 2 * BN + 64 * j];
    d[2] = img[SUBW + fb + 64 * j];
    d[3] = img[SUBW + fb + 2 * BN + 64 * j];
  };

  int cpy = 0, cpx = 0, crow = 0, cNB = 1, cinv = 0;
  if (CONVP) {
    crow = min(m0 + 32 * wave + l31, M - 1);
    const int pix = crow % (cs.H * cs.W);
    cpy = pix / cs.W;
    cpx = pix - cpy * cs.W;
    cNB = cs.Cin >> 5;
    cinv = (65536 + cNB - 1) / cNB;
  }
  auto xloadset = [&](int c, int p) {
    if (CONVP) {
      const int cc = bix(c);
      const int tap = (cc * cinv) >> 16, cb = cc - tap * cNB;
      const int ky = (tap * 11) >> 5, dy = ky - 1, dx = tap - 3 * ky - 1;
      const bool ok = (unsigned)(cpy + dy) < (unsigned)cs.H && (unsigned)(cpx + dx) < (unsigned)cs.W;
      const int rs = ok ? crow + dy * cs.W + dx : crow;
      const char* src = reinterpret_cast<const char*>(A) + ((int64_t)(rs >> 5) * cNB + cb) * 4096 + (lh * 32 + (rs & 31)) * 16;
      const f16x8_t z = {0, 0, 0, 0, 0, 0, 0, 0};
      const f16x8_t v0 = *reinterpret_cast<const f16x8_t*>(src), v1 = *reinterpret_cast<const f16x8_t*>(src + 1024);
      const f16x8_t v2 = *reinterpret_cast<const f16x8_t*>(src + 2048), v3 = *reinterpret_cast<const f16x8_t*>(src + 3072);
      ah[p][0] = ok ? v0 : z;
      al[p][0] = ok ? v1 : z;
      ah[p][1] = ok ? v2 : z;
      al[p][1] = ok ? v3 : z;
      return;
    }
    const char* src = fbase + bix(c) * 4096;
    ah[p][0] = *reinterpret_cast<const f16x8_t*>(src);
    al[p][0] = *reinterpret_cast<const f16x8_t*>(src + 1024);
    ah[p][1] = *reinterpret_cast<const f16x8_t*>(src + 2048);
    al[p][1] = *reinterpret_cast<const f16x8_t*>(src + 3072);
  };
  auto psplit = [&](const f32x4 u, const f32x4 v, f16x8_t& h, f16x8_t& l) {
    if (PRE || (PROBE & 512)) {
      h = __builtin_bit_cast(f16x8_t, u);
      l = __builtin_bit_cast(f16x8_t, v);
    } else {
      split_h3(u, v, h, l);
    }
  };
  auto pbread = [&](const u32x4_t* img, int j, u32x4_t (&d)[4]) {
    if (!(PROBE & 1024)) bread(img, j, d);
  };
  wload(0);
  if (DIRECT) xloadset(0, 0);
  else xload(0, xr[0]);
#pragma unroll
  for (int q = 0; q < UPLW; ++q) lds[wtid + 256 * RS * q] = wr[q];
  if (!DIRECT) {
    psplit(xr[0][0], xr[0][1], ah[0][0], al[0][0]);
    psplit(xr[0][2], xr[0][3], ah[0][1], al[0][1]);
  }
  wload(1);
  if (DIRECT) {
  } else if (DEEP) {
    xload(1, xr[DEEP ? 1 : 0]);
    xload(2, xr[0]);
  } else {
    xload(1, xr[0]);
  }
  asm volatile("s_waitcnt lgkmcnt(0)\n\ts_barrier" ::: "memory");
  bread(lds, 0, bq[0]);
  bread(lds, 1, bq[1]);
  unsigned long long cyc = 0;
  if (TIMING) {
    tm[1] = wall_clock64();
    cyc = __builtin_readcyclecounter();
  }

  auto mm = [](const f16x8_t a, const f16x8_t b, const f32x16_t c) {
    return FOUT ? __builtin_amdgcn_mfma_f32_32x32x16_f16(b, a, c, 0, 0, 0) : __builtin_amdgcn_mfma_f32_32x32x16_f16(a, b, c, 0, 0, 0);
  };
#define RBA_MFMA6(J, Q, P)                                                                                              \
  {                                                                                                                     \
    const f16x8_t bh0 = __builtin_bit_cast(f16x8_t, bq[Q][0]), bl0 = __builtin_bit_cast(f16x8_t, bq[Q][1]);             \
    const f16x8_t bh1 = __builtin_bit_cast(f16x8_t, bq[Q][2]), bl1 = __builtin_bit_cast(f16x8_t, bq[Q][3]);             \
    accm[J] = mm(ah[P][0], bh0, accm[J]);                                                                               \
    accl[J] = mm(ah[P][0], bl0, accl[J]);                                                                               \
    accm[J] = mm(ah[P][1], bh1, accm[J]);                                                                               \
    accl[J] = mm(al[P][0], bh0, accl[J]);                                                                               \
    accl[J] = mm(ah[P][1], bl1, accl[J]);                                                                               \
    accl[J] = mm(al[P][1], bh1, accl[J]);                                                                               \
  }
#define RBA_PIPE_MFMA_DSR                                                                                               \
  _Pragma("unroll") for (int i_ = 0; i_ < 4; ++i_) {                                                                    \
    __builtin_amdgcn_sched_group_barrier(0x008, 1, 0);                                                                  \
    __builtin_amdgcn_sched_group_barrier(0x100, 1, 0);                                                                  \
  }                                                                                                                     \
  __builtin_amdgcn_sched_group_barrier(0x008, 2, 0);
#define RBA_PIPE_MFMA_DSR_VALU                                                                                          \
  _Pragma("unroll") for (int i_ = 0; i_ < 4; ++i_) {                                                                    \
    __builtin_amdgcn_sched_group_barrier(0x008, 1, 0);                                                                  \
    __builtin_amdgcn_sched_group_barrier(0x100, 1, 0);                                                                  \
    __builtin_amdgcn_sched_group_barrier(0x002, 4, 0);                                                                  \
  }                                                                                                                     \
  __builtin_amdgcn_sched_group_barrier(0x008, 1, 0);                                                                    \
  __builtin_amdgcn_sched_group_barrier(0x002, 4, 0);                                                                    \
  __builtin_amdgcn_sched_group_barrier(0x008, 1, 0);
#define RBA_XI(P) (DEEP ? (P) ^ 1 : 0)
#define RBA_BLOCK(B, P, CUR, NXT)                                                                                       \
  {                                                                                                                     \
    if (!(PROBE & 256)) { _Pragma("unroll") for (int q = 0; q < UPLW; ++q)(NXT)[wtid + 256 * RS * q] = wr[q]; }        \
    if (!(PROBE & 1)) wload((B) + 2);                                                                                   \
    if (DIRECT) xloadset((B) + 1, (P) ^ 1);                                                                             \
    __builtin_amdgcn_sched_barrier(0);                                                                                  \
    RBA_MFMA6(0, 0, P)                                                                                                  \
    pbread(CUR, 2, bq[0]);                                                                                              \
    if (!DIRECT) psplit(xr[RBA_XI(P)][0], xr[RBA_XI(P)][1], ah[(P) ^ 1][0], al[(P) ^ 1][0]);                                                           \
    RBA_PIPE_MFMA_DSR_VALU                                                                                              \
    __builtin_amdgcn_sched_barrier(0);                                                                                  \
    RBA_MFMA6(1, 1, P)                                                                                                  \
    pbread(CUR, 3, bq[1]);                                                                                              \
    if (!DIRECT) psplit(xr[RBA_XI(P)][2], xr[RBA_XI(P)][3], ah[(P) ^ 1][1], al[(P) ^ 1][1]);                                                           \
    RBA_PIPE_MFMA_DSR_VALU                                                                                              \
    __builtin_amdgcn_sched_barrier(0);                                                                                  \
    if (!DIRECT && !(PROBE & 2)) xload((B) + (DEEP ? 3 : 2), xr[RBA_XI(P)]);                                                                                 \
    RBA_MFMA6(2, 0, P)                                                                                                  \
    if (!(PROBE & 64)) asm volatile("s_waitcnt lgkmcnt(0)\n\ts_barrier" ::: "memory");                               \
    __builtin_amdgcn_sched_barrier(0);                                                                                  \
    RBA_MFMA6(3, 1, P)                                                                                                  \
    pbread(NXT, 0, bq[0]);                                                                                              \
    RBA_PIPE_MFMA_DSR                                                                                                   \
    __builtin_amdgcn_sched_barrier(0);                                                                                  \
    pbread(NXT, 1, bq[1]);                                                                                              \
    __builtin_amdgcn_sched_barrier(0);                                                                                  \
  }
  int b = 0;
  if (NB & 1) {
    RBA_BLOCK(0, 0, lds, lds + BLK)
    for (b = 1; b < NB; b += 2) {
      RBA_BLOCK(b, 1, lds + BLK, lds)
      RBA_BLOCK(b + 1, 0, lds, lds + BLK)
    }
  } else {
    for (; b < NB; b += 2) {
      RBA_BLOCK(b, 0, lds, lds + BLK)
      RBA_BLOCK(b + 1, 1, lds + BLK, lds)
    }
  }
#undef RBA_BLOCK
#undef RBA_XI
#undef RBA_PIPE_MFMA_DSR
#undef RBA_PIPE_MFMA_DSR_VALU
#undef RBA_MFMA6

  if (TIMING) {
    tm[2] = wall_clock64();
    cyc = __builtin_readcyclecounter() - cyc;
  }
  if (KS == 2) {
    f32x4* red = reinterpret_cast<f32x4*>(lds_all);
#pragma unroll
    for (int pass = 0; pass < 2; ++pass) {
      __syncthreads();
      if (ks == 1) {
#pragma unroll
        for (int j = 0; j < CT; ++j)
#pragma unroll
          for (int q = 0; q < 4; ++q) {
            const f32x16_t& a = pass ? accl[j] : accm[j];
            red[(j * 4 + q) * 256 + tid] = (f32x4){a[4 * q], a[4 * q + 1], a[4 * q + 2], a[4 * q + 3]};
          }
      }
      __syncthreads();
      if (ks == 0) {
#pragma unroll
        for (int j = 0; j < CT; ++j)
#pragma unroll
          for (int q = 0; q < 4; ++q) {
            const f32x4 v = red[(j * 4 + q) * 256 + tid];
            f32x16_t& a = pass ? accl[j] : accm[j];
            a[4 * q] += v.x;
            a[4 * q + 1] += v.y;
            a[4 * q + 2] += v.z;
            a[4 * q + 3] += v.w;
          }
      }
    }
    if (ks == 1) return;
  }
  if (FOUT) h3_epilogue_split<ACT, CT>(accm, accl, bias, C, M, N, m0, n0, wave, l31, lh);
  else h3_epilogue<ACT, CT, PROBE, RES, GNM>(accm, accl, bias, C, R, M, N, m0, n0, BM, BN, wave, l31, lh, gm, reinterpret_cast<float*>(lds_all) + rs * 512);
  if (TIMING && tid == 0) {
    tm[3] = wall_clock64();
#pragma unroll
    for (int i = 0; i < 4; ++i) dbg[6 * blockIdx.x + i] = tm[i];
    dbg[6 * blockIdx.x + 4] = cyc;
    dbg[6 * blockIdx.x + 5] = 0;
  }
}

struct H3Args {
  const void* x;
  const u32x4_t* wp;
  const float* bias;
  void* out;
  int64_t M;
  int N, K;
  hipStream_t stream;
  const float* res = nullptr;
  unsigned long long* dbg = nullptr;
  ConvShape cs = ConvShape{0, 0, 0};
  int rows_per_image = 0;
  GnFold gn = GnFold{nullptr, nullptr, nullptr, 1, 1, 0};
  GnMoments gm = GnMoments{nullptr, 1, 1, 128};
  int stagger = 0;
  H3Rows rw = H3Rows{nullptr, 0, 0, 0};
};

inline bool h3_grid(const H3Args& a, int rows, int cols, int& MT, int& NT) {
  const int64_t mt = (a.M + rows - 1) / rows;
  MT = (int)mt;
  NT = (a.N + cols - 1) / cols;
  return mt * NT < (int64_t)1 << 31;
}

template <int ACT, int CT, unsigned FORM = 0>
int launch_h3(const H3Args& a) {
  int MT, NT;
  if (!h3_grid(a, 128, 32 * CT, MT, NT)) return (int)hipErrorInvalidValue;
  hipLaunchKernelGGL((split_linear_h3_kernel<ACT, CT, FORM>), dim3((unsigned)MT * NT), dim3(256), 0, a.stream, reinterpret_cast<const float*>(a.x), a.wp, a.bias,
                     reinterpret_cast<float*>(a.out), (int)a.M, a.N, a.K, MT, NT, a.dbg, a.res);
  return 0;
}

template <int ACT, int CT, unsigned FORM = 0>
int launch_h3l(const H3Args& a) {
  int MT, NT;
  if (!h3_grid(a, 128, 32 * CT, MT, NT)) return (int)hipErrorInvalidValue;
  hipLaunchKernelGGL((split_linear_h3l_kernel<ACT, CT, FORM>), dim3((unsigned)MT * NT), dim3(256), 0, a.stream, reinterpret_cast<const float*>(a.x), a.wp, a.bias,
                     reinterpret_cast<float*>(a.out), (int)a.M, a.N, a.K, MT, NT, a.dbg, a.cs, a.res, a.rows_per_image, a.gn, a.gm, a.rw);
  return 0;
}

template <int ACT, unsigned FORM = 0>
int launch_h3p(const H3Args& a) {
  int MT, NT;
  if (!h3_grid(a, h3_tile_rows(FORM), 128, MT, NT)) return (int)hipErrorInvalidValue;
  hipLaunchKernelGGL((split_linear_h3p_kernel<ACT, FORM>), dim3((unsigned)MT * NT), dim3(h3_threads(FORM)), 0, a.stream, reinterpret_cast<const float*>(a.x), a.wp,
                     a.bias, reinterpret_cast<float*>(a.out), (int)a.M, a.N, a.K, MT, NT, a.dbg, a.res, a.cs, h3_threads(FORM) == 256 ? a.stagger : 0, a.gm);
  return 0;
}

template <class F>
int h3_with_act(int act, F&& f) {
  if (act == 1) return f(std::integral_constant<int, 1>{});
  if (act == 2) return f(std::integral_constant<int, 2>{});
  return f(std::integral_constant<int, 0>{});
}

inline int64_t tiles128(int64_t M, int N) { return ((M + 127) / 128) * ((N + 127) / 128); }

RBA_KNOB_EXTERN(rba_k6_occ, 2);
inline bool h3p_single_resident(int64_t M, int N) { return rba_k6_occ == 1 && tiles128(M, N) <= 256; }

RBA_KNOB_EXTERN(rba_k6_rs, 0);
RBA_KNOB_EXTERN(rba_k6_rs_min_k, 512);
extern "C" int rba_concurrent_streams_hint;
inline bool h3p_multi_stream() { return rba_k6_rs == 3 || (rba_k6_rs == 0 && rba_concurrent_streams_hint >= 2); }
inline bool h3p_use_rs2(int64_t M, int N, int K) {
  if (rba_k6_rs == 1 || K < rba_k6_rs_min_k) return false;
  const int64_t t = ((M + 255) / 256) * ((N + 127) / 128);
  if (h3p_multi_stream()) return t >= 64;
  if (t < 160) return false;
  if (rba_k6_rs == 2) return true;
  const int64_t last = t % 256;
  return last == 0 || last >= 192;
}

RBA_KNOB_EXTERN(rba_k6_ks, 0);
inline bool h3p_use_ks2(int64_t M, int N, int K) {
  if (rba_k6_ks == 1 || (K & 63) || K < 128) return false;
  if (rba_k6_ks == 2) return true;
  const int64_t t = tiles128(M, N);
  return !h3p_multi_stream() && t > 128 && t <= 256 && K >= 1024;
}

template <int ACT, unsigned FORM, unsigned ALT>
int launch_h3p_by_shape(const H3Args& a) {
  static_assert((ALT & ~(H3_OCC1 | H3_KS2 | H3_RS2)) == 0 && (FORM & (H3_OCC1 | H3_KS2 | H3_RS2)) == 0, "FORM: the base form; ALT: geometry bits");
  if constexpr ((ALT & H3_OCC1) != 0) {
    if (h3p_single_resident(a.M, a.N)) return launch_h3p<ACT, FORM | H3_OCC1>(a);
  }
  if constexpr ((ALT & H3_KS2) != 0) {
    if (h3p_use_ks2(a.M, a.N, a.K)) return launch_h3p<ACT, FORM | H3_KS2>(a);
  }
  if constexpr ((ALT & H3_RS2) != 0) {
    if ((!(FORM & H3_GNM) || (a.M & 255) == 0) && h3p_use_rs2(a.M, a.N, a.K)) return launch_h3p<ACT, FORM | H3_RS2>(a);
  }
  return launch_h3p<ACT, FORM>(a);
}

inline bool h3_wide(int64_t M, int N) { return tiles128(M, N) >= 160 || N <= 64; }
template <int ACT, unsigned FORM>
int launch_h3_rows(const H3Args& a) {
  const bool wide = h3_wide(a.M, a.N);
  if (a.K <= 256) return wide ? launch_h3l<ACT, 4, FORM>(a) : launch_h3l<ACT, 2, FORM>(a);
  return wide ? launch_h3p_by_shape<ACT, FORM, H3_OCC1>(a) : launch_h3<ACT, 2, FORM>(a);
}

inline int h3_forms_compiled_in_every_unit(const H3Args& a) {
  return h3_with_act(0, [&](auto ACT) { return launch_h3p_by_shape<ACT, 0, H3_OCC1>(a); }) | launch_h3p_by_shape<0, H3_RES, H3_OCC1>(a) |
         launch_h3p_by_shape<0, H3_PRE | H3_CONVP, H3_RS2>(a) | launch_h3p_by_shape<0, H3_PRE | H3_CONVP | H3_GNM, H3_RS2>(a) | launch_h3l<0, 4, H3_GNM>(a);
}

#endif

}
```

rba_amd/maskformer_model.py:

```python
import itertools

import torch
import torch.nn as nn
import torch.nn.functional as F

from . import ops
from .h2d import to_device
from .arch import backbone_name as _backbone_name, complete
from .graph_replay import GraphKey, GraphReplay, capture
from .lru import ShapeCache
from .modeling.backbone import resnet as _resnet
from .modeling.backbone import swin as _swin
from .modeling.meta_arch import mask_former_head as _head
from .registry import BACKBONE_REGISTRY, META_ARCH_REGISTRY, SEM_SEG_HEADS_REGISTRY

_REGISTRATIONS = [0]
_EPOCHS = itertools.count(1)


def _registered(*_):
    _REGISTRATIONS[0] += 1


for _hook in (nn.modules.module.register_module_parameter_registration_hook, nn.modules.module.register_module_buffer_registration_hook,
              nn.modules.module.register_module_module_registration_hook):
    _hook(_registered)


def _class_prob(mask_cls):
    if 2 <= mask_cls.shape[-1] <= 64:
        return ops.softmax_drop_last(mask_cls.contiguous())
    return F.softmax(mask_cls, dim=-1)[..., :-1].contiguous()


@META_ARCH_REGISTRY.register()
class MaskFormer(nn.Module):
    def __init__(self, arch, backbone_name=None, head_name="MaskFormerHead"):
        super().__init__()
        a = complete(arch)
        self.arch = a
        self.backbone = BACKBONE_REGISTRY.get(backbone_name or _backbone_name(a))(a)
        self.sem_seg_head = SEM_SEG_HEADS_REGISTRY.get(head_name)(a)
        self.num_queries = a["num_queries"]
        self.size_divisibility = a["size_divisibility"] if a["size_divisibility"] > 0 else self.backbone.size_divisibility
        self.register_buffer("pixel_mean", torch.tensor(a["pixel_mean"], dtype=torch.float32).view(-1, 1, 1), False)
        self.register_buffer("pixel_std", torch.tensor(a["pixel_std"], dtype=torch.float32).view(-1, 1, 1), False)
        self._mean3 = tuple(float(torch.tensor(v, dtype=torch.float32)) for v in a["pixel_mean"])
        self._std3 = tuple(float(torch.tensor(v, dtype=torch.float32)) for v in a["pixel_std"])
        self.fused_front_end = True
        self.graph_replay = "auto"
        self.fused_upsample = True
        self.panoptic_on, self.open_panoptic = bool(a["panoptic_on"]), bool(a["open_panoptic"])
        self.sem_seg_postprocess_before_inference = bool(a["postprocess_before_inference"]) or self.panoptic_on
        self.object_mask_threshold, self.overlap_threshold = float(a["object_mask_threshold"]), float(a["overlap_threshold"])
        self.thing_classes = frozenset(int(c) for c in a["thing_classes"])
        self.eval()

    @property
    def device(self):
        return self.pixel_mean.device

    def preprocess(self, batched_inputs):
        images = [(to_device(x["image"], self.device).float() - self.pixel_mean) / self.pixel_std for x in batched_inputs]
        sizes = [tuple(int(v) for v in im.shape[-2:]) for im in images]
        d = self.size_divisibility
        H = (max(s[0] for s in sizes) + d - 1) // d * d
        W = (max(s[1] for s in sizes) + d - 1) // d * d
        batch = images[0].new_zeros((len(images), images[0].shape[0], H, W))
        for i, im in enumerate(images):
            batch[i, :, : sizes[i][0], : sizes[i][1]] = im
        return batch, sizes

    @torch.no_grad()
    def _predict_outputs(self, batched_inputs):
        pe = getattr(self.backbone, "patch_embed", None)
        if (self.fused_front_end and pe is not None and hasattr(self.backbone, "forward_images") and pe.fused_ok()
                and all(x["image"].dim() == 3 and x["image"].shape[0] == 3 and x["image"].dtype in (torch.uint8, torch.float32)
                        for x in batched_inputs)):
            images = [to_device(x["image"], self.device).contiguous() for x in batched_inputs]
            sizes = [tuple(int(v) for v in im.shape[-2:]) for im in images]
            d = self.size_divisibility
            H = (max(s[0] for s in sizes) + d - 1) // d * d
            W = (max(s[1] for s in sizes) + d - 1) // d * d
            features = self.backbone.forward_images(images, self._mean3, self._std3, H, W)
            return self.sem_seg_head(features), sizes, (H, W)
        batch, sizes = self.preprocess(batched_inputs)
        features = self.backbone(batch)
        return self.sem_seg_head(features), sizes, tuple(batch.shape[-2:])

    @torch.no_grad()
    def predict(self, batched_inputs):
        outputs, sizes, padded = self._predict_outputs(batched_inputs)
        return outputs["pred_logits"], outputs["pred_masks"], sizes, padded

    def finetune_outputs(self, batched_inputs):
        predictor = self.sem_seg_head.predictor
        if not getattr(predictor, "differentiable_heads", False):
            if getattr(predictor, "deep_supervision", False):
                raise ops.RbaHipError("finetune_outputs: predictor.deep_supervision is set without predictor.differentiable_heads; deep supervision "
                                      "is the differentiable heads' aux_outputs, so set differentiable_heads = True as well")
            raise ops.RbaHipError("finetune_outputs: set model.sem_seg_head.predictor.differentiable_heads = True first (without it the outputs "
                                  "carry no autograd graph)")
        with torch.no_grad():
            pe = getattr(self.backbone, "patch_embed", None)
            if (self.fused_front_end and pe is not None and hasattr(self.backbone, "forward_images") and pe.fused_ok()
                    and all(x["image"].dim() == 3 and x["image"].shape[0] == 3 and x["image"].dtype in (torch.uint8, torch.float32)
                            for x in batched_inputs)):
                images = [to_device(x["image"], self.device).contiguous() for x in batched_inputs]
                sizes = [tuple(int(v) for v in im.shape[-2:]) for im in images]
                d = self.size_divisibility
                padded = ((max(s[0] for s in sizes) + d - 1) // d * d, (max(s[1] for s in sizes) + d - 1) // d * d)
                features = self.backbone.forward_images(images, self._mean3, self._std3, *padded)
            else:
                batch, sizes = self.preprocess(batched_inputs)
                padded = tuple(batch.shape[-2:])
                features = self.backbone(batch)
            mask_features, _, multi_scale_features = self.sem_seg_head.pixel_decoder.forward_features(features)
        return predictor(multi_scale_features, mask_features), sizes, padded

    def prepare_targets(self, batched_inputs, padded):
        h_pad, w_pad = int(padded[0]), int(padded[1])
        dev = self.device
        new_targets = []
        for x in batched_inputs:
            gt_masks = to_device(x["instances"].gt_masks, dev)
            if gt_masks.shape[1] > h_pad or gt_masks.shape[2] > w_pad:
                raise ValueError(f"prepare_targets: masks of size {tuple(gt_masks.shape[1:])} do not fit the padded size {(h_pad, w_pad)}")
            padded_masks = torch.zeros((gt_masks.shape[0], h_pad, w_pad), dtype=gt_masks.dtype, device=dev)
            padded_masks[:, : gt_masks.shape[1], : gt_masks.shape[2]] = gt_masks
            entry = {"labels": to_device(x["instances"].gt_classes, dev), "masks": padded_masks}
            if "outlier_mask" in x:
                entry["outlier_masks"] = to_device(x["outlier_mask"], dev)
            if "sem_seg" in x:
                entry["sem_seg"] = to_device(x["sem_seg"], dev)
            new_targets.append(entry)
        return new_targets

    def _post(self, mask_cls, mask_pred, image_size, padded, want_sem_seg, want_argmax, score="rba"):
        prob = _class_prob(mask_cls)
        H, W = padded
        exact4 = mask_pred.shape[-2] * 4 == H and mask_pred.shape[-1] * 4 == W
        if self.fused_upsample and exact4 and prob.shape[1] <= 32:
            return ops.rba_reduce_up4(mask_pred.contiguous(), prob, image_size, want_sem_seg, want_argmax, score)
        up = ops.resample_bilinear(mask_pred.contiguous(), (H, W))
        rba, sem, arg = ops.rba_reduce(up, prob, want_sem_seg, want_argmax, score)
        h, w = image_size
        if (h, w) != (H, W):
            rba = rba[:h, :w].contiguous()
            sem = sem[:, :h, :w].contiguous() if sem is not None else None
            arg = arg[:h, :w].contiguous() if arg is not None else None
        return rba, sem, arg

    @torch.no_grad()
    def panoptic_inference(self, mask_cls, mask_pred, open_panoptic=False, ood_threshold=-0.1, pixel_min=300,
                           return_ood_pred=False):
        Q, H, W = mask_pred.shape
        K = mask_cls.shape[-1] - 1
        prob_all = F.softmax(mask_cls, dim=-1)
        scores, labels = prob_all.max(-1)
        keep = labels.ne(K) & (scores > self.object_mask_threshold)
        panoptic_seg = torch.zeros((H, W), dtype=torch.int32, device=mask_pred.device)
        segments_info = []
        if not bool(keep.any()):
            return panoptic_seg, segments_info
        cur_scores, cur_classes = scores[keep], labels[keep]
        cur_masks = mask_pred[keep].sigmoid()
        cur_mask_ids = (cur_scores.view(-1, 1, 1) * cur_masks).argmax(0)
        current = 0
        stuff_ids = {}
        for k in range(cur_classes.shape[0]):
            cls = int(cur_classes[k])
            won = cur_mask_ids == k
            solid = cur_masks[k] >= 0.5
            mask = won & solid
            mask_area, original_area, inter = int(won.sum()), int(solid.sum()), int(mask.sum())
            if mask_area == 0 or original_area == 0 or inter == 0 or mask_area / original_area < self.overlap_threshold:
                continue
            isthing = cls in self.thing_classes
            if not isthing:
                if cls in stuff_ids:
                    panoptic_seg[mask] = stuff_ids[cls]
                    continue
                stuff_ids[cls] = current + 1
            current += 1
            panoptic_seg[mask] = current
            segments_info.append({"id": current, "isthing": bool(isthing), "category_id": cls})
        if not open_panoptic:
            return panoptic_seg, segments_info
        ood_mask = ops.rba_reduce(mask_pred.contiguous(), prob_all[:, :-1].contiguous())[0]
        comp, n = ops.ood_components(ood_mask, ood_threshold)
        if n:
            free = panoptic_seg == 0
            sizes = torch.bincount(comp[free].long(), minlength=n + 1)
            ok = sizes >= pixel_min
            ok[0] = False
            new_id = current + torch.cumsum(ok.to(torch.int32), 0, dtype=torch.int32)
            sel = free & ok[comp.long()]
            panoptic_seg[sel] = new_id[comp.long()][sel]
            for _ in range(int(ok.sum())):
                current += 1
                segments_info.append({"id": current, "isthing": True, "category_id": 255})
        if return_ood_pred:
            return panoptic_seg, segments_info, ood_mask
        return panoptic_seg, segments_info

    @torch.no_grad()
    def forward(self, batched_inputs, include_void=False, return_separately=False, return_aux=False,
                return_ood_pred=False, return_argmax=False, panoptic_ood_threshold=-0.3, panoptic_pixel_min=200,
                return_panoptic_ood=False, **kwargs):
        if include_void or return_separately or return_aux or kwargs:
            raise NotImplementedError("only the semantic and (open-set) panoptic inference paths of MaskFormer.forward are provided")
        outputs, sizes, padded = self._predict_outputs(batched_inputs)
        mask_cls, mask_pred = outputs["pred_logits"], outputs["pred_masks"]
        ood_pred = None
        if return_ood_pred:
            if "ood_pred" not in outputs:
                raise KeyError("ood_pred: the model has no DenseHybrid head (MODEL.MASK_FORMER.DENSE_HYBRID_LOSS)")
            ood_pred = ops.resample_bilinear_ac(outputs["ood_pred"].contiguous(), sizes[0])
        results = []
        for i, inp in enumerate(batched_inputs):
            height, width = inp.get("height", sizes[i][0]), inp.get("width", sizes[i][1])
            if (height, width) != sizes[i] and self.sem_seg_postprocess_before_inference:
                up = ops.resample_bilinear(mask_pred[i].contiguous(), padded)[:, : sizes[i][0], : sizes[i][1]].contiguous()
                up = ops.resample_bilinear(up, (height, width))
                prob = _class_prob(mask_cls[i])
                rba, sem, arg = ops.rba_reduce(up, prob, True, return_argmax)
            else:
                rba, sem, arg = self._post(mask_cls[i], mask_pred[i], sizes[i], padded, True, return_argmax)
                if (height, width) != sizes[i]:
                    sem = ops.resample_bilinear(sem, (height, width))
                    rba = -sem.tanh().sum(dim=0)
                    arg = sem.argmax(0).to(torch.int32) if return_argmax else None
            r = {"sem_seg": sem, "rba": rba}
            if return_argmax:
                r["argmax"] = arg
            if self.panoptic_on:
                mp = ops.resample_bilinear(mask_pred[i].contiguous(), padded)[:, : sizes[i][0], : sizes[i][1]].contiguous()
                if (height, width) != sizes[i]:
                    mp = ops.resample_bilinear(mp, (height, width))
                r["panoptic_seg"] = self.panoptic_inference(mask_cls[i], mp, self.open_panoptic, panoptic_ood_threshold,
                                                            panoptic_pixel_min, return_panoptic_ood)
            results.append(r)
        if return_ood_pred:
            return results, ood_pred
        return results

    GRAPH_MAX = 8
    GRAPH_THRASH_MAX = 4
    LAUNCH_BOUND_RATIO = 0.95
    GRAPH_REMEASURE_EVERY = 32

    def _replay_state(self):
        return self.__dict__.get("_replay") or self.__dict__.setdefault("_replay", GraphReplay())

    def graph_decisions(self):
        return dict(self._replay_state().decisions)

    def _measured_eager(self, key, batched_inputs, return_argmax, score):
        import time
        dev = self.device
        e0, e1 = torch.cuda.Event(enable_timing=True), torch.cuda.Event(enable_timing=True)
        t0 = time.perf_counter()
        e0.record(torch.cuda.current_stream(dev))
        out = self._rba_scores_eager(batched_inputs, return_argmax, score)
        e1.record(torch.cuda.current_stream(dev))
        self._replay_state().measured(key, time.perf_counter() - t0, e0, e1)
        return out

    def _weights_version(self):
        st = self.__dict__.get("_param_flat")
        gen = _REGISTRATIONS[0]
        if st is None or st[0] != gen:
            flat = list(self.parameters()) + list(self.buffers())
            same = st is not None and len(flat) == len(st[2]) and all(a is b for a, b in zip(flat, st[2]))
            st = self.__dict__["_param_flat"] = [gen, st[1] if same else next(_EPOCHS), flat, st[3] if same else None]
        v = 0
        for t_ in st[2]:
            v += t_._version
        ptrs = [t_.data_ptr() for t_ in st[2]]
        if ptrs != st[3]:
            if st[3] is not None:
                st[1] = next(_EPOCHS)
            st[3] = ptrs
        return st[1], v

    def _graph_key(self, image, return_argmax, score):
        return GraphKey(tuple(image.shape), image.dtype, image.device, torch.cuda.current_stream(image.device).cuda_stream, bool(return_argmax), score,
                        self.fused_upsample, self.fused_front_end, ops.SPLIT_MODE, ops.SPLIT_ACTIVATIONS, ops.TILES_MIN, ops.MLP_FUSED_MIN_ROWS,
                        ops.concurrent_streams(), ops.SWIN_ATTN_FUSED,
                        (getattr(self.sem_seg_head.predictor, "sparse_intermediate_heads", None), ops.COMPOSED_MASK_HEAD), self._weights_version())

    def drop_graphs(self, release_constants=False):
        if release_constants:
            for m_ in self.modules():
                for v_ in vars(m_).values():
                    if isinstance(v_, ShapeCache):
                        v_.unpin()
        self._replay_state().drop()

    _TRANSIENT = ("_replay", "_param_flat")

    def __getstate__(self):
        st = dict(super().__getstate__() if hasattr(super(), "__getstate__") else self.__dict__)
        for k in self._TRANSIENT:
            st.pop(k, None)
        return st

    def __deepcopy__(self, memo):
        import copy
        cls = self.__class__
        new = cls.__new__(cls)
        memo[id(self)] = new
        for k, v in self.__dict__.items():
            if k not in self._TRANSIENT:
                new.__dict__[k] = copy.deepcopy(v, memo)
        return new

    def _apply(self, fn, *args, **kwargs):
        self.__dict__.pop("_param_flat", None)
        self.drop_graphs(release_constants=True)
        return super()._apply(fn, *args, **kwargs)

    def _graphed_scores(self, image, return_argmax, score):
        state = self._replay_state()
        key = self._graph_key(image, return_argmax, score)
        what = state.step(key, self.graph_replay == "auto", self)
        if what == "measure":
            return key
        if what == "capture":
            try:
                cap = torch.cuda.Stream(device=image.device)
                state.captured(key, *capture(lambda x: self._rba_scores_eager([{"image": x}], return_argmax, score)[0], image, cap), stream=cap)
            except Exception as e:
                import sys
                print(f"[rba_amd] hipGraph capture failed for image shape {tuple(image.shape)} ({type(e).__name__}: {e}); eager launches",
                      file=sys.stderr)
                torch.cuda.synchronize(image.device)
                state.captured(key)
        rec = state.graphs.get(key) if what in ("replay", "capture") else None
        if rec is None or rec.state != "captured":
            return None
        rec.static_in.copy_(image, non_blocking=True)
        rec.graph.replay()
        r = rec.static_out
        return (r[0].clone(), r[1].clone()) if return_argmax else r.clone()

    def live_graphs(self):
        return self._replay_state().live()

    @torch.no_grad()
    def rba_scores(self, batched_inputs, return_argmax=False, score="rba"):
        if (self.graph_replay and len(batched_inputs) == 1 and self.device.type == "cuda"
                and not torch.cuda.is_current_stream_capturing()):
            image = batched_inputs[0]["image"]
            if torch.is_tensor(image) and image.dim() == 3 and image.dtype in (torch.uint8, torch.float32) \
                    and set(batched_inputs[0]) <= {"image"}:
                image = to_device(image, self.device).contiguous()
                batched_inputs = [{"image": image}]
                if self.graph_replay == "auto":
                    fast = self._replay_state().eager_left
                    fk = (tuple(image.shape), image.dtype, bool(return_argmax), score, ops.SPLIT_MODE, torch.cuda.current_stream(image.device).cuda_stream)
                    left = fast.get(fk, 0)
                    if left > 0:
                        fast[fk] = left - 1
                        return self._rba_scores_eager(batched_inputs, return_argmax, score)
                r = self._graphed_scores(image, return_argmax, score)
                if isinstance(r, GraphKey):
                    return self._measured_eager(r, batched_inputs, return_argmax, score)
                if r is not None:
                    return [r]
        return self._rba_scores_eager(batched_inputs, return_argmax, score)

    @torch.no_grad()
    def _rba_scores_eager(self, batched_inputs, return_argmax=False, score="rba"):
        mask_cls, mask_pred, sizes, padded = self.predict(batched_inputs)
        out = []
        for i in range(len(batched_inputs)):
            rba, _, arg = self._post(mask_cls[i], mask_pred[i], sizes[i], padded, False, return_argmax, score)
            out.append((rba, arg) if return_argmax else rba)
        return out
```

rba_amd/modeling/backbone/swin.py:

```python
from types import SimpleNamespace

import torch
import torch.nn as nn
import torch.nn.functional as F

from ... import ops
from ...lru import derived
from ...registry import BACKBONE_REGISTRY


def relative_position_index(ws: int) -> torch.Tensor:
    ar = torch.arange(ws)
    gy, gx = torch.meshgrid(ar, ar, indexing="ij")
    gy, gx = gy.reshape(-1), gx.reshape(-1)
    dy = gy[:, None] - gy[None, :] + (ws - 1)
    dx = gx[:, None] - gx[None, :] + (ws - 1)
    return dy * (2 * ws - 1) + dx


class WindowAttention(nn.Module):
    def __init__(self, dim, window_size, num_heads):
        super().__init__()
        self.dim, self.window_size, self.num_heads = dim, window_size, num_heads
        self.relative_position_bias_table = nn.Parameter(torch.zeros((2 * window_size - 1) ** 2, num_heads))
        self.register_buffer("relative_position_index", relative_position_index(window_size))
        self.qkv = nn.Linear(dim, dim * 3)
        self.proj = nn.Linear(dim, dim)

    def block_image(self):
        wq, wp = self.qkv.weight, self.proj.weight
        return derived(self, "block_image", (wq, wp), lambda: ops.swin_attn_block_weights(wq.detach().contiguous(), wp.detach().contiguous()))

    def gathered_bias(self):
        t, idx = self.relative_position_bias_table, self.relative_position_index

        def build():
            N = self.window_size ** 2
            b = t[idx.view(-1)].view(N, N, -1).permute(2, 0, 1).contiguous()
            return b, ops.swin_bias_fragments(b, self.window_size) if b.is_cuda else None

        return derived(self, "gathered_bias", (t, idx), build)


class Mlp(nn.Module):
    def __init__(self, dim, hidden):
        super().__init__()
        self.fc1 = nn.Linear(dim, hidden)
        self.fc2 = nn.Linear(hidden, dim)


class SwinTransformerBlock(nn.Module):
    def __init__(self, dim, num_heads, window_size, shift_size, mlp_ratio):
        super().__init__()
        self.window_size, self.shift_size, self.num_heads = window_size, shift_size, num_heads
        self.norm1 = nn.LayerNorm(dim)
        self.attn = WindowAttention(dim, window_size, num_heads)
        self.norm2 = nn.LayerNorm(dim)
        self.mlp = Mlp(dim, int(dim * mlp_ratio))

    def forward(self, x, H, W, pending=None):
        M, C, hidden = x.numel() // x.shape[-1], x.shape[-1], self.mlp.fc2.in_features
        attn, mlp = self._select(x, pending, M, C, hidden)
        x, y = self._attention(attn, mlp, x, H, W, pending, M, C)
        return self._mlp(mlp, x, y, M, C, hidden)

    def _select(self, x, pending, M, C, hidden):
        if x.is_cuda and x.dim() == 3:
            if ops.swin_attn_block_ok(C, self.num_heads, self.window_size):
                return "A1", "M1" if ops.mlp_fused_ok(M, C, hidden) else "M2" if ops.linear_residual_fused(M, C, hidden) else "M3"
            if pending is None and ops.swin_attn_qkv_ok(C, self.num_heads, self.window_size) and ops.linear_residual_fused(M, C, C) and ops.linear_takes_split(M, C, C):
                return "A2", "M4"
        if not ops.linear_residual_fused(M, C, C):
            return "A3", "M6"
        return "A3", "M5" if ops.mlp_fused_ok(M, C, hidden) else "M4"

    def _attention(self, path, mlp, x, H, W, pending, M, C):
        a, n1, n2 = self.attn, self.norm1, self.norm2
        if path == "A1":
            if pending is not None:
                x = x + pending[0] + pending[1]
            bias_frag = a.gathered_bias()[1]
            return ops.swin_attn_block(x.contiguous(), (n1.weight, n1.bias, n1.eps), a.block_image(), a.qkv.bias, bias_frag, a.proj.bias, H, W,
                                       self.window_size, self.shift_size, norm2=None if mlp == "M1" else (n2.weight, n2.bias, n2.eps))
        if path == "A2":
            x = x.contiguous()
            y = ops.swin_attn_qkv(x, (n1.weight, n1.bias, n1.eps), a.block_image(), a.qkv.bias, a.gathered_bias()[1], H, W, self.window_size, self.shift_size)
            return ops.linear(y, a.proj, residual=x), None
        t, tb = pending if pending is not None else (None, None)
        x, y = ops.add_layer_norm(x, n1.weight, n1.bias, n1.eps, t, tb, inplace_sum=True, frag=ops.linear_takes_split(M, 3 * C, C))
        qkv = ops.linear(y, a.qkv)
        bias, bias_frag = a.gathered_bias()
        y = ops.swin_window_attn(qkv, a.qkv.bias, bias, H, W, self.num_heads, self.window_size, self.shift_size, bias_frag=bias_frag,
                                 split_out=mlp != "M6" and bias_frag is not None and ops.linear_takes_split(M, C, C) and
                                 ops.swin_window_attn_split_ok(C // self.num_heads, self.window_size))
        if mlp == "M6":
            return x, ops.linear(y, a.proj, use_bias=False)
        return ops.linear(y, a.proj, residual=x), None

    def _mlp(self, path, x, y, M, C, hidden):
        fc1, fc2, n2 = self.mlp.fc1, self.mlp.fc2, self.norm2
        if path == "M1":
            return ops.mlp_fused_ln(x, (n2.weight, n2.bias, n2.eps), fc1, fc2), None
        if path == "M5":
            y = ops.add_layer_norm(x, n2.weight, n2.bias, n2.eps)[1]
            return ops.mlp_fused(y, fc1, fc2, x), None
        if path in ("M2", "M4"):
            if path == "M4":
                y = ops.add_layer_norm(x, n2.weight, n2.bias, n2.eps, frag=ops.linear_takes_split(M, hidden, C))[1]
            y = ops.linear(y, fc1, gelu=True, split_out=ops.linear_takes_split(M, C, hidden))
            return ops.linear(y, fc2, residual=x), None
        if path == "M6":
            x, y = ops.add_layer_norm(x, n2.weight, n2.bias, n2.eps, y, self.attn.proj.bias, inplace_sum=True)
        y = ops.linear(y, fc1, gelu=True)
        return x, (ops.linear(y, fc2, use_bias=False), fc2.bias)


class PatchMerging(nn.Module):
    def __init__(self, dim):
        super().__init__()
        self.reduction = nn.Linear(4 * dim, 2 * dim, bias=False)
        self.norm = nn.LayerNorm(4 * dim)

    def forward(self, x, H, W):
        x = ops.merge_layer_norm(x.contiguous(), H, W, self.norm.weight, self.norm.bias, self.norm.eps)
        return ops.linear(x, self.reduction)


class BasicLayer(nn.Module):
    def __init__(self, dim, depth, num_heads, window_size, mlp_ratio, downsample):
        super().__init__()
        self.blocks = nn.ModuleList(
            SwinTransformerBlock(dim, num_heads, window_size, 0 if i % 2 == 0 else window_size // 2, mlp_ratio)
            for i in range(depth))
        self.downsample = PatchMerging(dim) if downsample else None


class PatchEmbed(nn.Module):
    def __init__(self, patch_size, in_chans, embed_dim):
        super().__init__()
        self.patch_size = patch_size
        self.proj = nn.Conv2d(in_chans, embed_dim, kernel_size=patch_size, stride=patch_size)
        self.norm = nn.LayerNorm(embed_dim)

    def forward(self, x):
        ps = self.patch_size
        _, _, H, W = x.shape
        if W % ps or H % ps:
            x = F.pad(x, (0, (ps - W % ps) % ps, 0, (ps - H % ps) % ps))
        B, Cin, H, W = x.shape
        Wh, Ww = H // ps, W // ps
        cols = x.reshape(B, Cin, Wh, ps, Ww, ps).permute(0, 2, 4, 1, 3, 5).reshape(B, Wh * Ww, Cin * ps * ps).contiguous()
        x = ops.linear(cols, self._linear_view())
        return ops.add_layer_norm(x, self.norm.weight, self.norm.bias, self.norm.eps)[1], Wh, Ww

    def _linear_view(self):
        w, b = self.proj.weight, self.proj.bias
        return derived(self, "linear_view", (w, b), lambda: SimpleNamespace(weight=w.detach().reshape(w.shape[0], -1), bias=b))

    def fused_ok(self):
        w = self.proj.weight
        return self.patch_size == 4 and w.shape[1] == 3 and w.is_cuda and w.dtype == torch.float32 and ops.SPLIT_MODE == "f16x3"

    def forward_images(self, images, mean, std, Hp, Wp):
        w = self.proj.weight

        def build():
            w64 = torch.zeros((w.shape[0], 64), dtype=torch.float32, device=w.device)
            w64[:, :48] = w.detach().reshape(w.shape[0], 48)
            return ops.split_weight(w64, mode="f16x3")

        planes = derived(self, "planes64", (w,), build)
        cols = torch.stack([ops.patch_im2col(im, mean, std, Hp, Wp) for im in images]) if len(images) > 1 \
            else ops.patch_im2col(images[0], mean, std, Hp, Wp)[None]
        x = ops.split_linear(cols, planes, self.proj.bias, out_features=w.shape[0])
        return ops.add_layer_norm(x, self.norm.weight, self.norm.bias, self.norm.eps)[1], Hp // 4, Wp // 4


@BACKBONE_REGISTRY.register()
class D2SwinTransformer(nn.Module):

    def __init__(self, arch):
        super().__init__()
        E, depths = arch["embed_dim"], arch["depths"]
        self.patch_embed = PatchEmbed(arch["patch_size"], 3, E)
        self.layers = nn.ModuleList(
            BasicLayer(E * 2 ** i, depths[i], arch["num_heads"][i], arch["window_size"], arch["mlp_ratio"],
                       downsample=i < len(depths) - 1) for i in range(len(depths)))
        self.num_features = [E * 2 ** i for i in range(len(depths))]
        for i, c in enumerate(self.num_features):
            self.add_module(f"norm{i}", nn.LayerNorm(c))

    @property
    def size_divisibility(self):
        return 32

    def forward_images(self, images, mean, std, Hp, Wp):
        return self._stages(*self.patch_embed.forward_images(images, mean, std, Hp, Wp))

    def forward(self, x):
        if x.dim() != 4:
            raise ValueError(f"SwinTransformer takes an input of shape (N, C, H, W). Got {tuple(x.shape)} instead!")
        return self._stages(*self.patch_embed(x))

    def _stages(self, x, Wh, Ww):
        outs = {}
        for i, layer in enumerate(self.layers):
            pending = None
            for blk in layer.blocks:
                x, pending = blk(x, Wh, Ww, pending)
            norm = getattr(self, f"norm{i}")
            t, tb = pending if pending is not None else (None, None)
            x, y = ops.add_layer_norm(x, norm.weight, norm.bias, norm.eps, t, tb, inplace_sum=True)
            outs[f"res{i + 2}"] = y.view(-1, Wh, Ww, self.num_features[i]).permute(0, 3, 1, 2)
            if layer.downsample is not None:
                x = layer.downsample(x, Wh, Ww)
                Wh, Ww = (Wh + 1) // 2, (Ww + 1) // 2
        return outs
```

rba_amd/modeling/pixel_decoder/msdeformattn.py:

```python
import torch
import torch.nn as nn
import torch.nn.functional as F

from ... import ops
from ...arch import FEATURE_NAMES, feature_channels, num_fpn_levels
from ...lru import ShapeCache, derived, source_key
from ...registry import SEM_SEG_HEADS_REGISTRY
from ..transformer_decoder.position_encoding import PositionEmbeddingSine
from .ops.ms_deform_attn import MSDeformAttn


class DeferredMaskFeatures:

    def __init__(self, prev, mr, norm, conv, planes, hw, num_groups=32, relu=True):
        self.prev, self.mr, self.norm, self.conv, self.planes, self.hw = prev, mr, norm, conv, planes, hw
        self.num_groups, self.relu = num_groups, relu
        self.batch = mr.shape[0]
        self._tensor = None

    @property
    def shape(self):
        return torch.Size((self.batch, self.conv.weight.shape[0]) + tuple(self.hw))

    @property
    def device(self):
        return self.prev.device

    @property
    def rows_per_image(self):
        return self.hw[0] * self.hw[1]

    def _project(self, planes, bias, N, rows=None):
        return ops.split_linear_nchw_out_gn_rows(self.prev, self.mr, self.norm.weight, self.norm.bias, self.num_groups, self.relu, planes, bias,
                                                 self.rows_per_image, out_features=N, rows=rows)

    def materialize(self):
        if self._tensor is None:
            md = self.conv.weight.shape[0]
            self._tensor = ops.split_linear_nchw_out_gn(self.prev, self.mr, self.norm.weight, self.norm.bias, self.num_groups, self.relu, self.planes,
                                                        self.conv.bias, self.rows_per_image, out_features=md).view(self.shape)
        return self._tensor

    def gather(self, rows):
        return self._project(self.planes, self.conv.bias, self.conv.weight.shape[0], rows)

    def contract(self, embed):
        w = self.conv.weight
        planes, bias_q = ops.compose_query_operand(embed, w.detach().view(w.shape[0], -1), self.conv.bias)
        return self._project(planes, bias_q, embed.shape[1]).view((self.batch, embed.shape[1]) + tuple(self.hw))


class _LinearView:

    def __init__(self, weight, bias):
        self.weight, self.bias = weight, bias


def _cached_linear_view(mod):
    w, b = mod.weight, mod.bias
    return derived(mod, "linear_view", (w, b), lambda: _LinearView(w.view(w.shape[0], -1), b))


def _conv3x3_planes(mod):
    w = mod.weight
    return derived(mod, ("conv3x3", ops.SPLIT_MODE), (w, mod.bias), lambda: ops.conv3x3_weight(w.detach()))


def _conv1x1_nchw(x, mod):
    B, C, h, w = x.shape
    y = ops.linear(x.permute(0, 2, 3, 1).reshape(B * h * w, C), _cached_linear_view(mod))
    return y.view(B, h, w, -1).permute(0, 3, 1, 2).contiguous()


class ConvNorm(nn.Module):

    def __init__(self, cin, cout, k, bias, norm, relu=False):
        super().__init__()
        self.weight = nn.Parameter(torch.zeros(cout, cin, k, k))
        self.bias = nn.Parameter(torch.zeros(cout)) if bias else None
        self.norm = nn.GroupNorm(32, cout) if norm else None
        self.padding, self.relu = k // 2, relu

    def forward(self, x):
        if self.padding == 0:
            x = _conv1x1_nchw(x, self)
        elif self.weight.shape[1] % 32 == 0:
            y = ops.conv3x3_nhwc(x.permute(0, 2, 3, 1).contiguous(), _conv3x3_planes(self), self.bias, out_features=self.weight.shape[0])
            x = y.permute(0, 3, 1, 2).contiguous()
        else:
            x = F.conv2d(x, self.weight, self.bias, padding=self.padding)
        if self.norm is not None:
            return ops.group_norm(x.contiguous(), 32, self.norm.weight, self.norm.bias, self.norm.eps, relu=self.relu)
        return F.relu(x) if self.relu else x


class MSDeformAttnTransformerEncoderLayer(nn.Module):
    def __init__(self, d_model, d_ffn, n_levels, n_heads, n_points):
        super().__init__()
        self.self_attn = MSDeformAttn(d_model, n_levels, n_heads, n_points)
        self.norm1 = nn.LayerNorm(d_model)
        self.linear1 = nn.Linear(d_model, d_ffn)
        self.linear2 = nn.Linear(d_ffn, d_model)
        self.norm2 = nn.LayerNorm(d_model)

    def forward(self, src, pos, reference_points, spatial_shapes, level_start_index):
        src = self.self_attn(src, reference_points, src, spatial_shapes, level_start_index, query_pos=pos, post=(src, self.norm1))
        hid = ops.linear(src, self.linear1, relu=True)
        N2, K2 = self.linear2.weight.shape
        if ops.token_linear_pays(hid.numel() // K2, N2, K2):
            return ops.token_linear(hid, self.linear2, residual=src, norm=self.norm2)
        src2 = ops.linear(hid, self.linear2, use_bias=False)
        return ops.add_layer_norm(src, self.norm2.weight, self.norm2.bias, self.norm2.eps, src2, self.linear2.bias)[1]


class MSDeformAttnTransformerEncoder(nn.Module):
    def __init__(self, layer_args, num_layers):
        super().__init__()
        self.layers = nn.ModuleList(MSDeformAttnTransformerEncoderLayer(*layer_args) for _ in range(num_layers))

    @staticmethod
    def get_reference_points(spatial_shapes, device):
        refs = []
        for H_, W_ in spatial_shapes:
            ry = (torch.arange(H_, dtype=torch.float32, device=device) + 0.5) / H_
            rx = (torch.arange(W_, dtype=torch.float32, device=device) + 0.5) / W_
            refs.append(torch.stack((rx[None, :].expand(H_, W_), ry[:, None].expand(H_, W_)), -1).reshape(-1, 2))
        ref = torch.cat(refs, 0)[None]
        return ref[:, :, None, :].repeat(1, 1, len(spatial_shapes), 1).contiguous()


class MSDeformAttnTransformerEncoderOnly(nn.Module):
    def __init__(self, d_model, nhead, num_encoder_layers, dim_feedforward, num_feature_levels, enc_n_points):
        super().__init__()
        self.encoder = MSDeformAttnTransformerEncoder(
            (d_model, dim_feedforward, num_feature_levels, nhead, enc_n_points), num_encoder_layers)
        self.level_embed = nn.Parameter(torch.zeros(num_feature_levels, d_model))
        self._ref_cache = ShapeCache(8)
        self._pos_cache = ShapeCache(8)

    def forward(self, srcs, pos_embeds, tokens=None):
        dev = srcs[0].device
        shapes = [tuple(int(v) for v in s.shape[-2:]) for s in srcs]
        B = srcs[0].shape[0]
        if tokens is not None:
            src = tokens[0].contiguous() if len(tokens) == 1 else torch.cat(tokens, 1)
        else:
            src = torch.cat([s.flatten(2).transpose(1, 2) for s in srcs], 1)

        def build_pos():
            p_ = torch.cat([p.flatten(2).transpose(1, 2) + self.level_embed[l].view(1, 1, -1) for l, p in enumerate(pos_embeds)], 1)
            return p_.expand(B, -1, -1).contiguous()

        pos = self._pos_cache.get((tuple(shapes), B, dev, source_key(self.level_embed)), build_pos)

        def build():
            sh_ = torch.as_tensor(shapes, dtype=torch.long, device=dev)
            lsi_ = torch.cat((sh_.new_zeros((1,)), sh_.prod(1).cumsum(0)[:-1]))
            return sh_, lsi_, MSDeformAttnTransformerEncoder.get_reference_points(shapes, dev)

        sh, lsi, ref = self._ref_cache.get((tuple(shapes), dev), build)
        if B > 1:
            ref = ref.expand(B, -1, -1, -1).contiguous()
        out = src
        for layer in self.encoder.layers:
            out = layer(out, pos, ref, sh, lsi)
        return out, shapes


@SEM_SEG_HEADS_REGISTRY.register()
class MSDeformAttnPixelDecoder(nn.Module):
    def __init__(self, arch):
        super().__init__()
        a = arch
        d = a["conv_dim"]
        chans = feature_channels(a)
        self.in_features = list(FEATURE_NAMES)
        self.transformer_in_features = list(a["enc_in"])
        self.transformer_num_feature_levels = len(a["enc_in"])
        self.maskformer_num_feature_levels = len(a["enc_in"])
        self.input_proj = nn.ModuleList(
            nn.Sequential(nn.Conv2d(chans[f], d, kernel_size=1), nn.GroupNorm(32, d)) for f in a["enc_in"][::-1])
        self.transformer = MSDeformAttnTransformerEncoderOnly(
            d, a["nheads"], a["enc_layers"], a["enc_dim_feedforward"], len(a["enc_in"]), a["enc_points"])
        self.pe_layer = PositionEmbeddingSine(d // 2, normalize=True)
        self.mask_features = nn.Conv2d(d, a["mask_dim"], kernel_size=1)
        self.num_fpn_levels = num_fpn_levels(a)
        for j in range(1, self.num_fpn_levels + 1):
            self.add_module(f"adapter_{j}", ConvNorm(chans[FEATURE_NAMES[j - 1]], d, 1, bias=False, norm=True))
            self.add_module(f"layer_{j}", ConvNorm(d, d, 3, bias=False, norm=True, relu=True))

    @staticmethod
    def _tokens(x):
        t = x.permute(0, 2, 3, 1)
        return t.reshape(x.shape[0], -1, x.shape[1]) if (x.is_cuda and x.dtype == torch.float32 and t.is_contiguous()) else None

    def _conv1x1(self, tok, mod, use_bias=True):
        lin = _cached_linear_view(mod)
        N, K = lin.weight.shape
        M = tok.numel() // K
        if not ops.split_linear_pays(M, N, K) and ops.token_linear_pays(M, N, K) and tok.is_contiguous():
            return ops.token_linear(tok, lin, use_bias=use_bias)
        return ops.linear(tok, lin, use_bias=use_bias)

    def _channels_last_ok(self, features):
        d = self.mask_features.weight.shape[1]
        if d % 32 or (d // 32) % 4 or 256 % (d // 4) or d > 1024:
            return False
        need = set(self.transformer_in_features) | set(self.in_features[:self.num_fpn_levels])
        return all(self._tokens(features[f]) is not None and features[f].shape[1] % 32 == 0 for f in need)

    def _encode_channels_last(self, features):
        srcs, pos, tks = [], [], []
        for idx, f in enumerate(self.transformer_in_features[::-1]):
            x = features[f]
            B, _, h, w = x.shape
            conv, gn = self.input_proj[idx][0], self.input_proj[idx][1]
            y = ops.group_norm_nhwc(self._conv1x1(self._tokens(x), conv), 32, gn.weight, gn.bias, gn.eps)
            tks.append(y.view(B, h * w, -1))
            srcs.append(y.view(B, h, w, -1).permute(0, 3, 1, 2))
            pos.append(self.pe_layer(x))
        y, shapes = self.transformer(srcs, pos, tokens=tks)
        B, d = y.shape[0], y.shape[2]
        toks = [z.contiguous() for z in torch.split(y, [h * w for h, w in shapes], dim=1)]
        outs = [z.view(B, h, w, d).permute(0, 3, 1, 2) for z, (h, w) in zip(toks, shapes)]
        return outs, toks[-1].view(B, *shapes[-1], d)

    def _top_down_level(self, prev, prev_norm, j, x):
        B, d = prev.shape[0], prev.shape[-1]
        h, w = int(x.shape[-2]), int(x.shape[-1])
        ad, ly = getattr(self, f"adapter_{j}"), getattr(self, f"layer_{j}")
        tok = self._tokens(x)
        if tok.is_contiguous() and ops.linear_emits_gn_moments(B * h * w, d, tok.shape[-1], h * w, 32):
            lat, lat_mr = ops.linear_gn_stats(tok, _cached_linear_view(ad), 32, ad.norm.eps, h * w, use_bias=False)
        else:
            lat = self._conv1x1(tok, ad, use_bias=False)
            lat_mr = ops.group_norm_nhwc_stats(lat, 32, ad.norm.eps)
        split = ops.conv3x3_takes_split(B * h * w, d) and d % 32 == 0
        yy = ops.SplitActivations.empty((B, h, w, d), prev.device) if split else None
        ups = []
        for b in range(B):
            xn = None if prev_norm is None else (prev_norm[0][b], prev_norm[1].weight, prev_norm[1].bias, True)
            ups.append(ops.resample_bilinear_nhwc_gn(prev[b], (h, w), lat[b].view(h, w, d), 32, x_norm=xn,
                                                     add_norm=(lat_mr[b], ad.norm.weight, ad.norm.bias), split_into=yy, image=b))
        if not split:
            yy = ups[0][None] if B == 1 else torch.stack(ups)
        planes = _conv3x3_planes(ly)
        if split and ops.conv3x3_emits_gn_moments(B, h, w, d, 32):
            prev, mr = ops.conv3x3_nhwc_gn_stats(yy, planes, 32, ly.norm.eps, None, out_features=d)
            return prev, (mr, ly.norm)
        prev = ops.conv3x3_nhwc(yy, planes, None, out_features=d)
        return prev, (ops.group_norm_nhwc_stats(prev.flatten(1, 2), 32, ly.norm.eps) if j > 1 else None, ly.norm)

    def _mask_features(self, prev, prev_norm, defer):
        B, ph, pw, d = prev.shape
        mr, norm = prev_norm
        mfw = self.mask_features.weight
        planes = derived(self.mask_features, ("mf_planes", ops.SPLIT_MODE), (mfw, self.mask_features.bias),
                         lambda: ops.split_weight(mfw.detach().view(mfw.shape[0], -1).contiguous()))
        if ops.split_linear_nchw_out_takes_gn(planes, ph * pw, d, 32):
            if mr is None:
                mr = ops.group_norm_nhwc_stats(prev.flatten(1, 2), 32, norm.eps)
            mf = DeferredMaskFeatures(prev.view(B * ph * pw, d), mr, norm, self.mask_features, planes, (ph, pw), num_groups=32, relu=True)
            return mf if defer else mf.materialize()
        prev = ops.group_norm_nhwc(prev.flatten(1, 2), 32, norm.weight, norm.bias, norm.eps, relu=True)
        return ops.split_linear_nchw_out(prev.view(B * ph * pw, d), planes, self.mask_features.bias, ph * pw,
                                         out_features=mfw.shape[0]).view(B, mfw.shape[0], ph, pw)

    def _forward_features_channels_last(self, features, defer_mask_features=False):
        outs, prev = self._encode_channels_last(features)
        prev_norm = None
        for j in range(self.num_fpn_levels, 0, -1):
            prev, prev_norm = self._top_down_level(prev, prev_norm, j, features[self.in_features[j - 1]])
        return self._mask_features(prev, prev_norm, defer_mask_features), outs[0], outs[:self.maskformer_num_feature_levels]

    def forward_features(self, features, defer_mask_features=False):
        if self.num_fpn_levels > 0 and self._channels_last_ok(features):
            return self._forward_features_channels_last(features, defer_mask_features)
        srcs, pos = [], []
        for idx, f in enumerate(self.transformer_in_features[::-1]):
            x = features[f].float().contiguous()
            conv, gn = self.input_proj[idx][0], self.input_proj[idx][1]
            srcs.append(ops.group_norm(_conv1x1_nchw(x, conv), 32, gn.weight, gn.bias, gn.eps))
            pos.append(self.pe_layer(x))
        y, shapes = self.transformer(srcs, pos)
        B = y.shape[0]
        outs = [z.transpose(1, 2).reshape(B, -1, shapes[i][0], shapes[i][1]).contiguous()
                for i, z in enumerate(torch.split(y, [h * w for h, w in shapes], dim=1))]
        for idx, f in enumerate(self.in_features[:self.num_fpn_levels][::-1]):
            j = self.num_fpn_levels - idx
            cur = getattr(self, f"adapter_{j}")(features[f].float().contiguous())
            yy = ops.resample_bilinear(outs[-1], cur.shape[-2:], add=cur.contiguous())
            outs.append(getattr(self, f"layer_{j}")(yy))
        mf = _conv1x1_nchw(outs[-1], self.mask_features)
        return mf, outs[0], outs[:self.maskformer_num_feature_levels]
```

rba_amd/ops.py:

```python
import contextlib
import ctypes
import threading
import functools
import math
import os

import torch

from . import _lib
from ._lib import RbaHipError
from .lru import derived


def _stream():
    return torch.cuda.current_stream().cuda_stream


def _launch(name, *args, stream=None):
    code = getattr(_lib.load(), name)(*args, torch.cuda.current_stream().cuda_stream if stream is None else stream)
    if code:
        _lib.check(code, name)


def _query(name, *args):
# ... 1060 lines not shown
        if segments != 1 or tuple(out.shape) != lead + (N,):
            raise RbaHipError("out must be a contiguous fp32 [..., N] tensor with x's leading shape (segments = 1)")
    if x_add is None and segments == 1:
        if out is None:
            out = torch.empty(lead + (N,), dtype=torch.float32, device=x.device)
        _launch("rba_skinny_linear_f32", _p(x), _p(weight), _p(bias), _p(out), M, N, K, int(bool(relu)))
        return out
    _shaped(x_add, "x_add", x.shape, optional=True)
    add_cols = N if add_cols is None else int(add_cols)
    if add_cols % 16 or not 0 <= add_cols <= N:
        raise RbaHipError("add_cols must be a multiple of 16 in [0, N]")
    seg_n = N // segments
    segs = None
    if out is None:
        out = segs = torch.empty((segments,) + lead + (seg_n,), dtype=torch.float32, device=x.device)
    _launch("rba_skinny_linear_add_f32", _p(x), _p(x_add), add_cols, _p(weight), _p(bias), _p(out), M, N, K, int(bool(relu)), seg_n if segments > 1 else 0)
    if segs is None:
        return out
    return segs[0] if segments == 1 else tuple(segs[i] for i in range(segments))


class SplitActivations:
    __slots__ = ("data", "shape")

    def __init__(self, data, shape):
        self.data, self.shape = data, tuple(shape)

    @staticmethod
    def empty(shape, device):
        M, K = math.prod(shape[:-1]), shape[-1]
        return SplitActivations(torch.empty((((M + 31) // 32) * 32 * K,), dtype=torch.int32, device=device), shape)

    @property
    def device(self):
        return self.data.device

    def numel(self):
        return math.prod(self.shape)

    @staticmethod
    def pack(x):
        K = x.shape[-1]
        x2 = x.reshape(-1, K).float()
        M = x2.shape[0]
        Mp = (M + 31) // 32 * 32
        xp = torch.zeros((Mp, K), dtype=torch.float32, device=x.device)
        xp[:M] = x2
        h = xp.half()
        l = ((xp - h.float()) * 2048.0).half()
        hl = torch.stack([h, l], 0).reshape(2, Mp // 32, 32, K // 32, 2, 2, 8)
        img = hl.permute(1, 3, 5, 0, 4, 2, 6).contiguous()
        return SplitActivations(img.reshape(-1).view(torch.int32), x.shape)

    def unpack(self):
        K = self.shape[-1]
        M = self.numel() // K
        Mp = (M + 31) // 32 * 32
        img = self.data.view(torch.float16).reshape(Mp // 32, K // 32, 2, 2, 2, 32, 8)
        hl = img.permute(3, 0, 5, 1, 4, 2, 6).reshape(2, Mp, K).float()
        return (hl[0] + hl[1] / 2048.0)[:M].reshape(self.shape)


_SPLIT = threading.local()
_SPLIT_DEFAULT = "f16x3"
"""ops.SPLIT_MODE: arithmetic of the token Linear (K6), PER THREAD (round 5: it was a process global; a re-score on another thread, or a tool
flipping it, changed the kernels of every forward in flight).  Read it as `ops.SPLIT_MODE`, set it for a block with `ops.split_mode(mode)`.  "f16x3": two f16 pieces per operand, three f16 MFMAs per product -- as accurate as an
fp32 GEMM for |x|, |w| < 65504 (beyond f16's range the output is NaN, never silently wrong), twice the speed of "bf16x6": three
bf16 pieces, six MFMAs, fp32's full range."""


def _split_mode():
    return getattr(_SPLIT, "mode", _SPLIT_DEFAULT)


def __getattr__(name):
    if name == "SPLIT_MODE":
        return _split_mode()
    raise AttributeError(f"module {__name__!r} has no attribute {name!r}")


class _OpsModule(type(os)):

    def __setattr__(self, name, value):
        if name == "SPLIT_MODE":
            raise AttributeError('ops.SPLIT_MODE is read-only (the arithmetic mode is per thread): run the block inside `with ops.split_mode("bf16x6"):`')
        super().__setattr__(name, value)


import sys as _sys
_sys.modules[__name__].__class__ = _OpsModule


@_hip_op
def split_weight(weight, mode=None):
    _chk(weight, "weight", dim=2)
    N, K = weight.shape
    if not split_linear_supported(N, K):
        raise RbaHipError("split_weight needs weight [N,K] with K % 32 == 0")
    mode = _split_mode() if mode is None else mode
    if mode not in ("f16x3", "bf16x6"):
        raise RbaHipError(f"unknown split mode {mode!r}")
    f16 = mode == "f16x3"
    packed = torch.empty(((N + 127) // 128, K // 16, 2 if f16 else 3, 128, 2, 8), dtype=torch.float16 if f16 else torch.bfloat16, device=weight.device)
    _launch("rba_split_weight_f16x2" if f16 else "rba_split_weight_bf16x3", _p(weight), _p(packed), N, K)
    return packed


@_hip_op
def unpack_split_weight(packed):
    nt, S, P = packed.shape[:3]
    r = torch.arange(128, device=packed.device)
    flip = ((r >> 3) & 1).bool()
    un = torch.where(flip.view(1, 1, 1, 128, 1, 1), packed.flip(4), packed)
    if P == 2:
        un = un.reshape(nt, S // 2, 2, P, 128, 2, 8).permute(3, 0, 4, 1, 5, 2, 6)
        return un.reshape(P, nt * 128, S * 16)
    return un.permute(2, 0, 3, 1, 4, 5).reshape(3, nt * 128, S * 16)


def split_linear_supported(N, K):
    return K % 32 == 0 and N >= 1 and K >= 32


TILES_MIN = 64


def split_linear_pays(M, N, K, gelu=False):
    if not split_linear_supported(N, K) or K < 64:
        return False
    return _tiles128(M, N) >= TILES_MIN


@_hip_op
def linear(x, lin, use_bias=True, gelu=False, relu=False, residual=None, split_out=False):
    w = lin.weight
    N, K = w.shape
    M = x.numel() // K if K else 0
    bias = lin.bias if use_bias else None
    if isinstance(x, SplitActivations):
        if _split_mode() != "f16x3" or x.shape[-1] != K:
            raise RbaHipError("SplitActivations feed the f16x3 Linear only (check linear_takes_split(M, N, K) before producing them)")
        return split_linear(x, _cached_planes(lin, w), bias, gelu=gelu, out_features=N, relu=relu, residual=residual, split_out=split_out)
    _chk(x, "x") if x.is_contiguous() else _chk(x.contiguous(), "x")
    if split_out:
        if _split_mode() != "f16x3" or not split_linear_supported(N, K):
            raise RbaHipError("linear(split_out=True) needs the f16x3 mode and K % 32 == 0")
        return split_linear(x.contiguous(), _cached_planes(lin, w), bias, gelu=gelu, out_features=N, split_out=True)
    if residual is not None and not linear_residual_fused(M, N, K):
        raise RbaHipError("linear(residual=...) needs the fused f16x3 path: check linear_residual_fused(M, N, K) first")
    if split_linear_supported(N, K):
        return split_linear(x.contiguous(), _cached_planes(lin, w), bias, gelu=gelu, out_features=N, relu=relu, residual=residual)
    Kp = (K + 31) // 32 * 32
    xp = torch.zeros(tuple(x.shape[:-1]) + (Kp,), dtype=torch.float32, device=x.device)
    xp[..., :K] = x
    return split_linear(xp, _cached_planes(lin, w, pad_k=Kp), bias, gelu=gelu, out_features=N, relu=relu)


def _cached_planes(lin, w, pad_k=None):
    def build():
        w2 = w.detach().contiguous()
        if pad_k is not None:
            w2 = torch.nn.functional.pad(w2, (0, pad_k - w2.shape[1]))
        return split_weight(w2)

    return derived(lin, ("planes", _split_mode()), (w,), build, pad_k)


@contextlib.contextmanager
def split_mode(mode):
    if mode not in ("f16x3", "bf16x6"):
        raise RbaHipError(f"unknown split mode {mode!r}")
    prev = _split_mode()
    _SPLIT.mode = mode
    try:
        yield
    finally:
        _SPLIT.mode = prev


SPLIT_ACTIVATIONS = os.environ.get("RBA_SPLIT_ACTIVATIONS", "1") != "0"


SPLIT_MIN_K = int(os.environ.get("RBA_SPLIT_MIN_K", "128"))


def linear_takes_split(M, N, K):
    if not (SPLIT_ACTIVATIONS and _split_mode() == "f16x3" and K >= SPLIT_MIN_K and K % 32 == 0):
        return False
    tiles = _tiles128(M, N)
    return tiles >= 160 or (tiles >= 32 and K % 64 == 0 and K >= 256 and N % 32 == 0)


MLP_FUSED_MIN_ROWS = 32768


def mlp_fused_ok(M, C, hidden):
    return SPLIT_ACTIVATIONS and _split_mode() == "f16x3" and C == 128 and hidden % 32 == 0 and hidden >= 64 and M >= MLP_FUSED_MIN_ROWS


@_hip_op
def mlp_fused(x, fc1, fc2, residual):
    _chk(x, "x")
    _chk(residual, "residual")
    C, hidden = fc1.weight.shape[1], fc1.weight.shape[0]
    M = x.numel() // C
    if (x.shape[-1] != C or tuple(fc2.weight.shape) != (C, hidden) or tuple(residual.shape) != tuple(x.shape) or C != 128 or hidden % 32
            or _split_mode() != "f16x3"):
        raise RbaHipError("mlp_fused needs C == 128, hidden % 32 == 0, matching fc1 / fc2 and the f16x3 mode")
    _launch("rba_swin_mlp_fused_f16x3_f32", _p(x), _p(_cached_planes(fc1, fc1.weight)), _p(fc1.bias), _p(_cached_planes(fc2, fc2.weight)), _p(fc2.bias),
            _p(residual), _p(residual), M, C, hidden)
    return residual


@_hip_op
def mlp_fused_ln(x, norm, fc1, fc2):
    _chk(x, "x")
    g, b, eps = norm
    C, hidden = fc1.weight.shape[1], fc1.weight.shape[0]
    _vec(g, "norm.weight", C)
    _vec(b, "norm.bias", C)
    M = x.numel() // C
    if x.shape[-1] != C or tuple(fc2.weight.shape) != (C, hidden) or C != 128 or hidden % 32 or _split_mode() != "f16x3":
        raise RbaHipError("mlp_fused_ln needs C == 128, hidden % 32 == 0, matching fc1 / fc2 and the f16x3 mode")
    _launch("rba_swin_mlp_fused_ln_f16x3_f32", _p(x), _p(g), _p(b), float(eps), _p(_cached_planes(fc1, fc1.weight)), _p(fc1.bias),
            _p(_cached_planes(fc2, fc2.weight)), _p(fc2.bias), M, C, hidden)
    return x


def linear_residual_fused(M, N, K):
    return _split_mode() == "f16x3" and split_linear_pays(M, N, K)


@_hip_op
def split_linear(x, planes, bias=None, gelu=False, out_features=None, relu=False, residual=None, split_out=False):
    xp, pre = _split_x(x, "split_linear")
    K = x.shape[-1]
    N, f16 = _packed(planes, K, out_features)
    M = x.numel() // K if K else 0
    lead = tuple(x.shape[:-1])
    if not split_linear_supported(N, K):
        raise RbaHipError("split_linear needs x [..., K] and split_weight(W) of a weight [N,K] with K % 32 == 0")
    _vec(bias, "bias", N, optional=True)
    act = 1 if gelu else (2 if relu else 0)
    if split_out:
        if not f16 or act != 1 or residual is not None or N % 32:
            raise RbaHipError("split_out needs f16x3 planes, gelu=True, no residual and N % 32 == 0")
        out = SplitActivations.empty(lead + (N,), x.device)
        _launch("rba_split_linear_f16x3_gelu_split_out", xp, 1 if pre else 0, _p(planes), _p(bias), _p(out.data), M, N, K)
        return out
    if residual is not None:
        _chk(residual, "residual")
        if not f16 or act or tuple(residual.shape) != lead + (N,):
            raise RbaHipError("residual needs f16x3 planes, no activation and a [..., N] tensor")
        if pre:
            _launch("rba_split_linear_f16x3_frag_f32", xp, _p(planes), _p(bias), _p(residual), _p(residual), M, N, K, 0)
        else:
            _launch("rba_split_linear_f16x3_res_f32", xp, _p(planes), _p(bias), _p(residual), _p(residual), M, N, K)
        return residual
    if pre and not f16:
        raise RbaHipError("SplitActivations need f16x3 planes")
    out = torch.empty(lead + (N,), dtype=torch.float32, device=x.device)
    if pre:
        _launch("rba_split_linear_f16x3_frag_f32", xp, _p(planes), _p(bias), 0, _p(out), M, N, K, act)
    else:
        _launch("rba_split_linear_f16x3_f32" if f16 else "rba_split_linear_f32", xp, _p(planes), _p(bias), _p(out), M, N, K, act)
    return out


@_hip_op
def split_linear_nchw_out(x, planes, bias, rows_per_image, out_features=None):
    _chk(x, "x", dim=2)
    M, K = x.shape
    N, f16 = _packed(planes, K, out_features)
    if rows_per_image < 1 or M % rows_per_image:
        raise RbaHipError("split_linear_nchw_out needs x [B*P, K] with M % rows_per_image == 0")
    _vec(bias, "bias", N, optional=True)
    out = torch.empty((M // rows_per_image, N, rows_per_image), dtype=torch.float32, device=x.device)
    _launch("rba_split_linear_nchw_out_f16x3_f32" if f16 else "rba_split_linear_nchw_out_f32", _p(x), _p(planes), _p(bias), _p(out), M, N, K, rows_per_image)
    return out


GN_MOMENTS = os.environ.get("RBA_GN_MOMENTS", "1") != "0"


def _gn_moments_ok(rows_per_image, N, num_groups):
    return (GN_MOMENTS and _split_mode() == "f16x3" and rows_per_image % 128 == 0 and N % 128 == 0 and N % num_groups == 0
            and (N // num_groups) in (4, 8, 16, 32))


def linear_emits_gn_moments(M, N, K, rows_per_image, num_groups):
    return _gn_moments_ok(rows_per_image, N, num_groups) and K <= 256 and K % 32 == 0 and _tiles128(M, N) >= 160 and M % rows_per_image == 0


def conv3x3_emits_gn_moments(B, H, W, N, num_groups):
    return _gn_moments_ok(H * W, N, num_groups) and conv3x3_takes_split(B * H * W, N)


def _merge_gn_moments(moments, B, G, splits, eps):
    mr = torch.empty((B, G, 2), dtype=torch.float32, device=moments.device)
    _launch("rba_group_norm_nhwc_merge_f32", _p(moments), _p(mr), B, G, splits, float(eps))
    return mr


@_hip_op
def linear_gn_stats(x, lin, num_groups, eps, rows_per_image, use_bias=True):
    _chk(x, "x")
    w = lin.weight
    N, K = w.shape
    M = x.numel() // K
    if not linear_emits_gn_moments(M, N, K, rows_per_image, num_groups) or x.shape[-1] != K:
        raise RbaHipError("linear_gn_stats: check linear_emits_gn_moments(M, N, K, rows_per_image, G) first")
    bias = lin.bias if use_bias else None
    planes = _cached_planes(lin, w)
    B, splits = M // rows_per_image, rows_per_image // 128
    out = torch.empty(tuple(x.shape[:-1]) + (N,), dtype=torch.float32, device=x.device)
    mom = torch.empty((B, num_groups, splits, 3), dtype=torch.float32, device=x.device)
    _launch("rba_split_linear_f16x3_gn_moments_f32", _p(x), _p(planes), _p(bias), _p(out), M, N, K, rows_per_image, int(num_groups), _p(mom))
    return out, _merge_gn_moments(mom, B, int(num_groups), splits, eps)


@_hip_op
def conv3x3_nhwc_gn_stats(x, planes, num_groups, eps, bias=None, out_features=None):
    if not isinstance(x, SplitActivations):
        raise RbaHipError("conv3x3_nhwc_gn_stats needs SplitActivations of logical shape [B,H,W,C]")
    xp, _ = _split_x(x, "conv3x3_nhwc_gn_stats", dim=4)
    B, H, W, C = x.shape
    N, _ = _packed(planes, 9 * C, out_features, bf16x6=False)
    if C % 32 or not conv3x3_emits_gn_moments(B, H, W, N, num_groups):
        raise RbaHipError("conv3x3_nhwc_gn_stats: check conv3x3_emits_gn_moments(B, H, W, N, G) first")
    _vec(bias, "bias", N, optional=True)
    splits = H * W // 128
    out = torch.empty((B, H, W, N), dtype=torch.float32, device=x.device)
    mom = torch.empty((B, num_groups, splits, 3), dtype=torch.float32, device=x.device)
    _launch("rba_conv3x3_nhwc_f16x3_split_in_gn_moments_f32", xp, _p(planes), _p(bias), _p(out), B, H, W, C, N, int(num_groups), _p(mom))
    return out, _merge_gn_moments(mom, B, int(num_groups), splits, eps)


def split_linear_nchw_out_takes_gn(planes, rows_per_image, K, num_groups):
    return planes.dtype == torch.float16 and rows_per_image % 128 == 0 and K % num_groups == 0 and (K // num_groups) % 4 == 0 and K % 32 == 0


@_hip_op
def split_linear_nchw_out_gn(x, mr, weight, bias_gn, num_groups, relu, planes, bias, rows_per_image, out_features=None):
    _chk(x, "x", dim=2)
    _chk(mr, "mr", dim=3)
    M, K = x.shape
    N, _ = _packed(planes, K, out_features, bf16x6=False)
    if rows_per_image < 1 or M % rows_per_image or not split_linear_nchw_out_takes_gn(planes, rows_per_image, K, num_groups):
        raise RbaHipError("split_linear_nchw_out_gn needs x [B*P, K], P % 128 == 0 and (K / G) % 4 == 0")
    B = M // rows_per_image
    if tuple(mr.shape) != (B, num_groups, 2):
        raise RbaHipError("mr must be [B, G, 2]")
    _vec(weight, "weight", K)
    _vec(bias_gn, "bias_gn", K)
    _vec(bias, "bias", N, optional=True)
    out = torch.empty((B, N, rows_per_image), dtype=torch.float32, device=x.device)
    _launch("rba_split_linear_nchw_out_gn_f16x3_f32", _p(x), _p(mr), _p(weight), _p(bias_gn), int(num_groups), int(bool(relu)), _p(planes), _p(bias), _p(out),
            M, N, K, rows_per_image)
    return out


COMPOSED_MASK_HEAD = os.environ.get("RBA_COMPOSED_MASK_HEAD", "1") != "0"


class RowIndex:
    __slots__ = ("data", "rows_per_image")

    def __init__(self, data, rows_per_image):
        self.data, self.rows_per_image = data, rows_per_image


def row_index(idx, rows_per_image):
    if not isinstance(idx, torch.Tensor) or not idx.is_cuda or idx.dtype not in (torch.int32, torch.int64) or idx.dim() != 2 or idx.numel() == 0:
        raise RbaHipError("row_index needs a HIP int32 / int64 tensor [B, R]")
    lo, hi = int(idx.min()), int(idx.max())
    if lo < 0 or hi >= rows_per_image:
        raise RbaHipError(f"row_index: values must lie in [0, {rows_per_image}), got [{lo}, {hi}]")
    return RowIndex(idx.to(torch.int32).contiguous(), int(rows_per_image))


def _image_planes(planes, K, out_features, B):
    if planes.dim() != 7:
        return _packed(planes, K, out_features, bf16x6=False)[0], 0
    _chk(planes, "planes", dtype=torch.float16, dim=7)
    if planes.shape[0] != B:
        raise RbaHipError(f"per-image planes must be [B = {B}, ...], got {tuple(planes.shape)}")
    return _packed(planes[0], K, out_features, bf16x6=False)[0], planes.stride(0) * 2


@_hip_op
def split_linear_nchw_out_gn_rows(x, mr, weight, bias_gn, num_groups, relu, planes, bias, rows_per_image, out_features=None, rows=None):
    _chk(x, "x", dim=2)
    _chk(mr, "mr", dim=3)
    M, K = x.shape
    P = int(rows_per_image)
    if P < 1 or M % P or planes.dtype != torch.float16 or not split_linear_nchw_out_takes_gn(planes, P, K, num_groups) or P * K >= 1 << 30:
        raise RbaHipError("split_linear_nchw_out_gn_rows needs x [B*P, K], float16 planes, P % 128 == 0, (K / G) % 4 == 0 and P * K < 2^30")
    B = M // P
    N, wstride = _image_planes(planes, K, out_features, B)
    if tuple(mr.shape) != (B, num_groups, 2):
        raise RbaHipError("mr must be [B, G, 2]")
    _vec(weight, "weight", K)
    _vec(bias_gn, "bias_gn", K)
    bstride = 0
    if bias is not None and bias.dim() == 2:
        _shaped(bias, "bias", (B, N))
        bstride = N
    else:
        _vec(bias, "bias", N, optional=True)
    R = P
    if rows is not None:
        if not isinstance(rows, RowIndex) or rows.rows_per_image != P or rows.data.shape[0] != B or rows.data.shape[1] % 128 or rows.data.device != x.device:
            raise RbaHipError("rows must be ops.row_index(idx [B, R], rows_per_image) for this x, with R % 128 == 0")
        R = rows.data.shape[1]
    out = torch.empty((B, N, R), dtype=torch.float32, device=x.device)
    _launch("rba_split_linear_nchw_out_gn_rows_f16x3_f32", _p(x), _p(mr), _p(weight), _p(bias_gn), int(num_groups), int(bool(relu)), _p(planes), wstride, _p(bias),
            bstride, _p(None if rows is None else rows.data), _p(out), B, P, R, N, K)
    return out


@_hip_op
def compose_query_operand(embed, weight, bias):
    _chk(embed, "embed", dim=3)
    _chk(weight, "weight", dim=2)
    B, Q, C = embed.shape
    K = weight.shape[1]
    if weight.shape[0] != C or not (1 <= Q <= 128 and 4 <= C <= 256 and C % 4 == 0 and K >= 32 and K % 32 == 0):
        raise RbaHipError("compose_query_operand needs embed [B, Q <= 128, C <= 256] (C % 4 == 0) and weight [C, K] with K % 32 == 0")
    _vec(bias, "bias", C, optional=True)
    planes = torch.empty((B, 1, K // 16, 2, 128, 2, 8), dtype=torch.float16, device=embed.device)
    bias_q = torch.empty((B, Q), dtype=torch.float32, device=embed.device)
    _launch("rba_compose_query_operand_f16x2", _p(embed), _p(weight), _p(bias), _p(planes), _p(bias_q), B, Q, C, K)
    return planes, bias_q


def composed_mask_head_pays(rows_per_image, sparse_rows):
    return 2 * sparse_rows <= rows_per_image


@_hip_op
def conv3x3_weight(weight, mode=None):
    _chk(weight, "weight", dim=4)
    N, C, kh, kw = weight.shape
    if (kh, kw) != (3, 3) or C % 32:
        raise RbaHipError("conv3x3_weight needs a [N, C, 3, 3] weight with C % 32 == 0")
    return split_weight(weight.permute(0, 2, 3, 1).reshape(N, 9 * C).contiguous(), mode=mode)


def conv3x3_takes_split(M, N):
    return SPLIT_ACTIVATIONS and _split_mode() == "f16x3" and _tiles128(M, N) >= 256


@_hip_op
def conv3x3_nhwc(x, planes, bias=None, out_features=None):
    xp, pre = _split_x(x, "conv3x3_nhwc", dim=4)
    B, H, W, C = x.shape
    N, f16 = _packed(planes, 9 * C, out_features)
    if C % 32:
        raise RbaHipError("conv3x3_nhwc needs x [B,H,W,C] with C % 32 == 0")
    _vec(bias, "bias", N, optional=True)
    if pre and not (f16 and conv3x3_takes_split(B * H * W, N)):
        raise RbaHipError("conv3x3_nhwc: SplitActivations need f16x3 planes and conv3x3_takes_split(B*H*W, N)")
    out = torch.empty((B, H, W, N), dtype=torch.float32, device=x.device)
    _launch("rba_conv3x3_nhwc_f16x3_split_in_f32" if pre else "rba_conv3x3_nhwc_f16x3_f32" if f16 else "rba_conv3x3_nhwc_f32",
            xp, _p(planes), _p(bias), _p(out), B, H, W, C, N)
    return out


_CONCURRENT_STREAMS = {}


def set_concurrent_streams(n):
    n = max(1, int(n))
    prev = int(_query("rba_set_concurrent_streams", n))
    _CONCURRENT_STREAMS[id(_lib.load())] = n
    return prev


def concurrent_streams():
    return _CONCURRENT_STREAMS.get(id(_lib.load()), 1)


TOKEN_LINEAR = os.environ.get("RBA_TOKEN_LINEAR", "1") != "0"


def token_linear_ok(N, K):
    return TOKEN_LINEAR and _split_mode() == "f16x3" and 1 <= N <= 256 and K >= 32 and K % 32 == 0


TOKEN_MAX_ROWS = 8192


def token_linear_pays(M, N, K):
    return token_linear_ok(N, K) and N % 4 == 0 and 1 <= M <= TOKEN_MAX_ROWS


def _token_planes(lin):
    w = lin.weight

    def build():
        w2 = w.detach().contiguous()
        _chk(w2, "weight", dim=2)
        N, K = w2.shape
        packed = torch.empty((((N + 15) // 16) * (K // 32) * 128, 4), dtype=torch.int32, device=w.device)
        _launch("rba_token_linear_pack_f16x2", _p(w2), _p(packed), N, K)
        return packed

    return derived(lin, "token_planes", (w,), build)


@_hip_op
def token_linear(x, lin, x_add=None, use_bias=True, relu=False, residual=None, norm=None):
    _chk(x, "x")
    N, K = lin.weight.shape
    if x.shape[-1] != K or not token_linear_ok(N, K):
        raise RbaHipError("token_linear: x [..., K] with K % 32 == 0, N <= 256 and the f16x3 mode (see token_linear_ok)")
    M = x.numel() // K
    _shaped(x_add, "x_add", x.shape, optional=True)
    bias = _vec(lin.bias if use_bias else None, "bias", N, optional=True)
    if (residual is None) != (norm is None):
        raise RbaHipError("token_linear: residual and norm come together")
    ln_w, ln_b, ln_eps, act = 0, 0, 0.0, 2 if relu else 0
    if norm is not None:
        _chk(residual, "residual")
        if tuple(residual.shape) != tuple(x.shape[:-1]) + (N,) or N % 16 or relu or norm.weight.numel() != N:
            raise RbaHipError("token_linear(norm=...): residual [..., N], N % 16 == 0, no activation")
        ln_w, ln_b, ln_eps = _p(norm.weight), _p(norm.bias), float(norm.eps)
    out = torch.empty(tuple(x.shape[:-1]) + (N,), dtype=torch.float32, device=x.device)
    _launch("rba_token_linear_f32", _p(x), _p(x_add), _p(_token_planes(lin)), _p(bias), _p(residual), ln_w, ln_b, ln_eps, _p(out), M, N, K, act)
    return out


@_hip_op
def token_linear_multi(x, specs):
    _chk(x, "x")
    K = x.shape[-1]
    M = x.numel() // K if K else 0
    lead = tuple(x.shape[:-1])
    if not 1 <= len(specs) <= 3:
        raise RbaHipError("token_linear_multi: one to three problems")
    arr = (_lib.TokenLinearProblem * len(specs))()
    outs, keep = [], []
    for i, (lin, x_add, out, col0, relu) in enumerate(specs):
        N, K_ = lin.weight.shape
        if K_ != K or not token_linear_ok(N, K) or N % 4:
            raise RbaHipError("token_linear_multi: weights [N <= 256, N % 4 == 0, K] with x's K % 32 == 0 (see token_linear_ok)")
        _shaped(x_add, "x_add", x.shape, optional=True)
        _vec(lin.bias, "bias", N, optional=True)
        if out is None:
            out, col0 = torch.empty(lead + (N,), dtype=torch.float32, device=x.device), 0
        else:
            _chk(out, "out")
            if tuple(out.shape[:-1]) != lead or col0 % 4 or col0 + N > out.shape[-1] or out.shape[-1] % 4:
                raise RbaHipError("token_linear_multi: out [..., ld] with ld % 4 == 0 and a column slice col0 % 4 == 0 inside it")
        planes = _token_planes(lin)
        keep.append(planes)
        arr[i] = _lib.TokenLinearProblem(_p(x_add) or None, _p(planes), _p(lin.bias) or None, out.data_ptr() + 4 * col0, N, out.shape[-1], 2 if relu else 0)
        outs.append(out)
    _launch("rba_token_linear_multi_f32", _p(x), ctypes.byref(arr), len(specs), M, K)
    return outs


@_hip_op
def patch_im2col(image, mean, std, Hp, Wp):
    if image.dtype not in (torch.uint8, torch.float32):
        raise RbaHipError("image must be uint8 or float32")
    _chk(image, "image", dtype=image.dtype, dim=3)
    if image.shape[0] != 3 or Hp % 4 or Wp % 4 or Hp < image.shape[1] or Wp < image.shape[2] or len(mean) != 3 or len(std) != 3:
        raise RbaHipError("patch_im2col needs a [3,h,w] image and Hp >= h, Wp >= w multiples of 4")
    h, w = int(image.shape[1]), int(image.shape[2])
    out = torch.empty(((Hp // 4) * (Wp // 4), 64), dtype=torch.float32, device=image.device)
    m = (ctypes.c_float * 3)(*[float(v) for v in mean])
    sd = (ctypes.c_float * 3)(*[float(v) for v in std])
    _launch("rba_patch_im2col_u8" if image.dtype == torch.uint8 else "rba_patch_im2col_f32", _p(image), _p(out), h, w, int(Hp), int(Wp),
            ctypes.addressof(m), ctypes.addressof(sd))
    return out


def _nhwc_rows(x):
    _chk(x, "x")
    if x.dim() not in (3, 4):
        raise RbaHipError("x must be [B,P,C] or [B,H,W,C]")
    B, C = x.shape[0], x.shape[-1]
    return B, (x.numel() // (B * C) if B * C else 0), C


@_hip_op
def group_norm_nhwc(x, num_groups, weight, bias, eps=1e-5, relu=False):
    B, P, C = _nhwc_rows(x)
    _vec(weight, "weight", C)
    _vec(bias, "bias", C)
    if not _gn_nhwc_ok(C, num_groups):
        raise RbaHipError("group_norm_nhwc needs C % G == 0, (C/G) % 4 == 0, C <= 1024 and 256 % (C/4) == 0")
    ws = _scratch(_query("rba_group_norm_nhwc_workspace_bytes", B, P, C, num_groups), x.device)
    y = torch.empty_like(x)
    _launch("rba_group_norm_nhwc_f32", _p(x), _p(weight), _p(bias), _p(y), _p(ws), B, P, C, num_groups, float(eps), int(bool(relu)))
    return y


@_hip_op
def resample_bilinear_nhwc(x, size, add=None, split_into=None, image=0):
    _chk(x, "x", dim=3)
    h, w, C = x.shape
    H, W = int(size[0]), int(size[1])
    if C % 4:
        raise RbaHipError("resample_bilinear_nhwc needs C % 4 == 0")
    _shaped(add, "add", (H, W, C), optional=True)
    if split_into is not None:
        _split_into_ok(split_into, image, H, W, C)
        _launch("rba_resample_bilinear_nhwc_split_out_f32", _p(x), _p(add), _p(split_into.data), C, h, w, H, W, image * H * W)
        return split_into
    out = torch.empty((H, W, C), dtype=torch.float32, device=x.device)
    _launch("rba_resample_bilinear_nhwc_f32", _p(x), _p(add), _p(out), C, h, w, H, W)
    return out


@_hip_op
def group_norm_nhwc_stats(x, num_groups, eps=1e-5):
    B, P, C = _nhwc_rows(x)
    if not _gn_nhwc_ok(C, num_groups):
# ... 119 lines not shown
```

Baseline: 151.8.

## Fold backbone stage LayerNorm into FPN lateral GEMM prologue

The final LayerNorm of Swin stages with C=128/256 (res2, res3 feeding only the FPN lateral path) is deferred. The lateral 1x1 projection kernel computes per-row mean and rstd itself and applies the affine before staging the operand. This removes a separate LayerNorm launch and its full write and read of the normalized feature map. In exchange, the GEMM prologue does extra reads and reductions, and more Python plumbing is needed to carry deferred-norm objects, with a fallback that materializes them.

```diff
diff --git a/include/rba_hip.h b/include/rba_hip.h
--- a/include/rba_hip.h
+++ b/include/rba_hip.h
@@ -209,6 +209,9 @@
 
 int rba_split_linear_f16x3_gn_moments_f32(const float* x, const void* weight_packed, const float* bias, float* out, int64_t M, int N, int K,
                                           int rows_per_image, int G, float* moments, void* stream);
+int rba_split_linear_f16x3_ln_gn_moments_f32(const float* x, const float* ln_gamma, const float* ln_beta, float ln_eps, const void* weight_packed,
+                                             const float* bias, float* out, int64_t M, int N, int K, int rows_per_image, int G, float* moments,
+                                             void* stream);
 int rba_conv3x3_nhwc_f16x3_split_in_gn_moments_f32(const void* x_frag, const void* weight_packed, const float* bias, float* out, int B, int H,
                                                    int W, int C, int N, int G, float* moments, void* stream);
 int rba_group_norm_nhwc_merge_f32(const float* moments, float* mr, int B, int G, int splits, float eps, void* stream);
diff --git a/rba_amd/_lib.py b/rba_amd/_lib.py
--- a/rba_amd/_lib.py
+++ b/rba_amd/_lib.py
@@ -80,6 +80,7 @@
     "rba_split_linear_nchw_out_f32": [_vp, _vp, _vp, _vp, _i64, _i, _i, _i, _vp],
     "rba_split_linear_nchw_out_f16x3_f32": [_vp, _vp, _vp, _vp, _i64, _i, _i, _i, _vp],
     "rba_split_linear_f16x3_gn_moments_f32": [_vp, _vp, _vp, _vp, _i64, _i, _i, _i, _i, _vp, _vp],
+    "rba_split_linear_f16x3_ln_gn_moments_f32": [_vp, _vp, _vp, ctypes.c_float, _vp, _vp, _vp, _i64, _i, _i, _i, _i, _vp, _vp],
     "rba_conv3x3_nhwc_f16x3_split_in_gn_moments_f32": [_vp, _vp, _vp, _vp, _i, _i, _i, _i, _i, _i, _vp, _vp],
     "rba_group_norm_nhwc_merge_f32": [_vp, _vp, _i, _i, _i, ctypes.c_float, _vp],
     "rba_split_linear_nchw_out_gn_f16x3_f32": [_vp, _vp, _vp, _vp, _i, _i, _vp, _vp, _vp, _i64, _i, _i, _i, _vp],
diff --git a/rba_amd/csrc/build.py b/rba_amd/csrc/build.py
--- a/rba_amd/csrc/build.py
+++ b/rba_amd/csrc/build.py
@@ -6,7 +6,7 @@
 HERE = os.path.dirname(os.path.abspath(__file__))
 SOURCES = ["rba_reduce.hip", "rba_reduce_bwd.hip", "resample.hip", "ms_deform_attn.hip", "ms_deform_attn_bwd.hip", "masked_xattn.hip", "mask_logits.hip", "mask_logits_bwd.hip", "point_loss.hip", "outlier_tail.hip", "dense_hybrid_loss.hip", "pebal_loss.hip", "tta_merge.hip", "resize_u8.hip", "confusion.hip", "train_view.hip",
            "swin_window_attn.hip", "swin_attn_block.hip", "group_norm.hip", "layer_norm.hip", "skinny_linear.hip", "split_linear.hip", "split_linear_dma.hip", "split_linear_gnf.hip", "gaussian_blur.hip", "open_panoptic.hip", "dense_hybrid.hip", "patch_embed.hip", "token_linear.hip", "decoder_small.hip"]
-HEADERS = ["common.h", "knobs.h", "bilinear_ac.h", "rba_reduce_kernels.h", "split_linear_dma.h", "split_linear_h3.h", "split_linear_h3q.h", "mlp_fused_h3.h", "swin_window_attn_h3.h", "swin_attn_block.h",
+HEADERS = ["common.h", "knobs.h", "layer_norm_row.h", "bilinear_ac.h", "rba_reduce_kernels.h", "split_linear_dma.h", "split_linear_h3.h", "split_linear_h3q.h", "mlp_fused_h3.h", "swin_window_attn_h3.h", "swin_attn_block.h",
            os.path.join("..", "..", "include", "rba_hip.h")]
 TUNE_SOURCES = [os.path.join("tune", "rba_reduce_tune.hip"), os.path.join("tune", "split_linear_tune.hip"), os.path.join("tune", "split_linear_ws.hip"), os.path.join("tune", "mlp_fused_h1.hip"), os.path.join("tune", "k5_timing.hip"), os.path.join("tune", "k5_wpe_ab.hip"), os.path.join("tune", "k5_wpe_plain.hip"), os.path.join("tune", "k5_persist.hip"), os.path.join("tune", "k7_timing.hip")] + [os.path.join("tune", f"gnf_form{f}_dbg{d}.hip") for f in (0, 1) for d in (0, 1)] + [os.path.join("tune", "gnf_form0_dbg1_unpacked.hip"), os.path.join("tune", "gnf_form1_dbg0_unpacked.hip")]
 TUNE_LIB = os.path.join(HERE, "tune", "librba_tune.so")
diff --git a/rba_amd/csrc/layer_norm.hip b/rba_amd/csrc/layer_norm.hip
--- a/rba_amd/csrc/layer_norm.hip
+++ b/rba_amd/csrc/layer_norm.hip
@@ -1,4 +1,5 @@
 #include "common.h"
+#include "layer_norm_row.h"
 #include "../../include/rba_hip.h"
 
 namespace {
@@ -58,25 +59,22 @@
       }
       if (t) a += *reinterpret_cast<const f32x4*>(t + base + 4 * c4);
       if (tb) a += *reinterpret_cast<const f32x4*>(tb + 4 * c4);
-      sum += (a.x + a.y) + (a.z + a.w);
+      sum += rba_ln_sum4(a);
     }
     v[j] = a;
   }
 #pragma unroll
   for (int o = G / 2; o > 0; o >>= 1) sum += __shfl_xor(sum, o, RBA_WAVE);
-  const float mean = sum / (float)C;
+  const float mean = rba_ln_mean(sum, C);
   float sq = 0.f;
 #pragma unroll
   for (int j = 0; j < NV; ++j) {
     const int c4 = sub + j * G;
-    if (c4 < nv4) {
-      const f32x4 d = v[j] - mean;
-      sq += (d.x * d.x + d.y * d.y) + (d.z * d.z + d.w * d.w);
-    }
+    if (c4 < nv4) sq += rba_ln_sq4(v[j], mean);
   }
 #pragma unroll
   for (int o = G / 2; o > 0; o >>= 1) sq += __shfl_xor(sq, o, RBA_WAVE);
-  const float rstd = 1.0f / sqrtf(sq / (float)C + eps);
+  const float rstd = rba_ln_rstd(sq, C, eps);
   if (!TR && !rvalid) return;
 #pragma unroll
   for (int j = 0; j < NV; ++j) {
@@ -85,7 +83,7 @@
       if (sum_out && rvalid) *reinterpret_cast<f32x4*>(sum_out + base + 4 * c4) = v[j];
       const f32x4 gj = EARLY ? g4[EARLY ? j : 0] : *reinterpret_cast<const f32x4*>(gamma + 4 * c4);
       const f32x4 bj = EARLY ? b4[EARLY ? j : 0] : *reinterpret_cast<const f32x4*>(beta + 4 * c4);
-      const f32x4 o = (v[j] - mean) * rstd * gj + bj;
+      const f32x4 o = rba_ln_apply(v[j], mean, rstd, gj, bj);
       if (FRAG) {
         uint32_t h[2], l[2];
         rba_split_f16x2(o.x, o.y, h[0], l[0]);
diff --git a/rba_amd/csrc/layer_norm_row.h b/rba_amd/csrc/layer_norm_row.h
--- /dev/null
+++ b/rba_amd/csrc/layer_norm_row.h
@@ -0,0 +1,11 @@
+#pragma once
+#include "common.h"
+
+#define rba_ln_sum4(a) (((a).x + (a).y) + ((a).z + (a).w))
+__device__ __forceinline__ float rba_ln_mean(float sum, int C) { return sum / (float)C; }
+__device__ __forceinline__ float rba_ln_sq4(const f32x4 v, float mean) {
+  const f32x4 d = v - mean;
+  return (d.x * d.x + d.y * d.y) + (d.z * d.z + d.w * d.w);
+}
+__device__ __forceinline__ float rba_ln_rstd(float sq, int C, float eps) { return 1.0f / sqrtf(sq / (float)C + eps); }
+__device__ __forceinline__ f32x4 rba_ln_apply(const f32x4 v, float mean, float rstd, const f32x4 g, const f32x4 b) { return (v - mean) * rstd * g + b; }
diff --git a/rba_amd/csrc/split_linear_gnf.hip b/rba_amd/csrc/split_linear_gnf.hip
--- a/rba_amd/csrc/split_linear_gnf.hip
+++ b/rba_amd/csrc/split_linear_gnf.hip
@@ -31,3 +31,16 @@
   if (per_image) return rba_gemm_status(wide ? launch_h3l<0, 4, F | H3_PERIMG>(a) : launch_h3l<0, 2, F | H3_PERIMG>(a));
   return rba_gemm_status(wide ? launch_h3l<0, 4, F>(a) : launch_h3l<0, 2, F>(a));
 }
+
+extern "C" int rba_split_linear_f16x3_ln_gn_moments_f32(const float* x, const float* ln_gamma, const float* ln_beta, float ln_eps, const void* weight_packed,
+                                                        const float* bias, float* out, int64_t M, int N, int K, int rows_per_image, int G, float* moments,
+                                                        void* stream) {
+  RBA_CHECK_ARG(N >= 128 && (N % 128) == 0 && (K == 128 || K == 256) && G >= 1 && (N % G) == 0 && rows_per_image >= 128);
+  const int cpg = N / G;
+  RBA_CHECK_ARG((cpg == 4 || cpg == 8 || cpg == 16 || cpg == 32) && (rows_per_image % 128) == 0);
+  RBA_GEMM_PROLOGUE(M, K, x && ln_gamma && ln_beta && weight_packed && out && moments && (M % rows_per_image) == 0, x, weight_packed, out, ln_gamma, ln_beta);
+  H3Args a{x, reinterpret_cast<const u32x4_t*>(weight_packed), bias, out, M, N, K, (hipStream_t)stream};
+  a.gm = GnMoments{moments, G, cpg, rows_per_image};
+  a.ln = LnFold{ln_gamma, ln_beta, ln_eps};
+  return rba_gemm_status(launch_h3l<0, 4, H3_GNM | H3_LNF>(a));
+}
diff --git a/rba_amd/csrc/split_linear_h3.h b/rba_amd/csrc/split_linear_h3.h
--- a/rba_amd/csrc/split_linear_h3.h
+++ b/rba_amd/csrc/split_linear_h3.h
@@ -1,6 +1,7 @@
 #pragma once
 #include <type_traits>
 
+#include "layer_norm_row.h"
 #include "split_linear_dma.h"
 
 RBA_KNOB_EXTERN(rba_k6_stagger, 0);
@@ -204,11 +205,12 @@
   H3_RS2 = 1u << 11,
   H3_ROWIDX = 1u << 12,
   H3_PERIMG = 1u << 13,
+  H3_LNF = 1u << 14,
   H3_PROBE_SHIFT = 16,
 };
 constexpr unsigned h3_probe(int p) { return (unsigned)p << H3_PROBE_SHIFT; }
 constexpr int h3_probe_of(unsigned form) { return (int)(form >> H3_PROBE_SHIFT); }
-constexpr unsigned H3_FORMS = H3_TIMING | H3_RES, H3L_FORMS = H3_FORMS | H3_GNM | H3_CONV | H3_NCHW | H3_GNF | H3_ROWIDX | H3_PERIMG,
+constexpr unsigned H3_FORMS = H3_TIMING | H3_RES, H3L_FORMS = H3_FORMS | H3_GNM | H3_CONV | H3_NCHW | H3_GNF | H3_ROWIDX | H3_PERIMG | H3_LNF,
                    H3P_FORMS = H3_FORMS | H3_GNM | H3_PRE | H3_FOUT | H3_CONVP | H3_OCC1 | H3_KS2 | H3_RS2;
 constexpr bool h3_form_within(unsigned form, unsigned allowed) { return (form & ~allowed & ((1u << H3_PROBE_SHIFT) - 1)) == 0; }
 constexpr int h3_tile_rows(unsigned form) { return (form & H3_RS2) ? 256 : 128; }
@@ -362,17 +364,75 @@
   int bstride;
   int64_t wstride;
 };
+struct LnFold {
+  const float* gamma;
+  const float* beta;
+  float eps;
+};
+template <int NBK>
+__device__ __forceinline__ void h3_ln_row_stats(const char* xbase, const uint32_t (&xoff)[4], int C, float eps, float (&mean)[4], float (&rstd)[4]) {
+  constexpr int RG = NBK <= 4 ? 4 : 2;
+#pragma unroll
+  for (int q0 = 0; q0 < 4; q0 += RG) {
+    f32x4 v[RG][NBK];
+    float s[RG][NBK], r[RG];
+#pragma unroll
+    for (int q = 0; q < RG; ++q)
+#pragma unroll
+      for (int b = 0; b < NBK; ++b) v[q][b] = *reinterpret_cast<const f32x4*>(xbase + b * 128 + xoff[q0 + q]);
+    auto butterfly = [&]() {
+#pragma unroll
+      for (int q = 0; q < RG; ++q) {
+#pragma unroll
+        for (int o = NBK / 2; o > 0; o >>= 1) {
+          float t[NBK];
+#pragma unroll
+          for (int b = 0; b < NBK; ++b) t[b] = s[q][b] + s[q][b ^ o];
+#pragma unroll
+          for (int b = 0; b < NBK; ++b) s[q][b] = t[b];
+        }
+        r[q] = s[q][0];
+      }
+#pragma unroll
+      for (int o = 4; o > 0; o >>= 1)
+#pragma unroll
+        for (int q = 0; q < RG; ++q) r[q] += __shfl_xor(r[q], o, RBA_WAVE);
+    };
+#pragma unroll
+    for (int q = 0; q < RG; ++q)
+#pragma unroll
+      for (int b = 0; b < NBK; ++b) {
+        s[q][b] = 0.f;
+        s[q][b] += rba_ln_sum4(v[q][b]);
+      }
+    butterfly();
+#pragma unroll
+    for (int q = 0; q < RG; ++q) mean[q0 + q] = rba_ln_mean(r[q], C);
+#pragma unroll
+    for (int q = 0; q < RG; ++q)
+#pragma unroll
+      for (int b = 0; b < NBK; ++b) {
+        s[q][b] = 0.f;
+        s[q][b] += rba_ln_sq4(v[q][b], mean[q0 + q]);
+      }
+    butterfly();
+#pragma unroll
+    for (int q = 0; q < RG; ++q) rstd[q0 + q] = rba_ln_rstd(r[q], C, eps);
+  }
+}
 template <int ACT, int CT, unsigned FORM = 0>
 __global__ __launch_bounds__(256, 2) void split_linear_h3l_kernel(const float* __restrict__ A, const u32x4_t* __restrict__ Wp,
                                                                  const float* __restrict__ bias, float* C, int M, int N,
                                                                  int K, int MT, int NT, unsigned long long* dbg = nullptr,
                                                                  ConvShape cs = ConvShape{0, 0, 0}, const float* R = nullptr, int rows_per_image = 0,
                                                                  GnFold gn = GnFold{nullptr, nullptr, nullptr, 1, 1, 0},
-                                                                 GnMoments gm = GnMoments{nullptr, 1, 1, 128}, H3Rows rw = H3Rows{nullptr, 0, 0, 0}) {
-  static_assert(h3_form_within(FORM, H3L_FORMS), "split_linear_h3l_kernel: H3_TIMING, H3_RES, H3_GNM, H3_CONV, H3_NCHW, H3_GNF, H3_ROWIDX, H3_PERIMG, h3_probe()");
+                                                                 GnMoments gm = GnMoments{nullptr, 1, 1, 128}, H3Rows rw = H3Rows{nullptr, 0, 0, 0},
+                                                                 LnFold ln = LnFold{nullptr, nullptr, 0.f}) {
+  static_assert(h3_form_within(FORM, H3L_FORMS), "split_linear_h3l_kernel: H3_TIMING, H3_RES, H3_GNM, H3_CONV, H3_NCHW, H3_GNF, H3_ROWIDX, H3_PERIMG, H3_LNF, h3_probe()");
   constexpr int PROBE = h3_probe_of(FORM);
   constexpr bool TIMING = FORM & H3_TIMING, CONV = FORM & H3_CONV, RES = FORM & H3_RES, NCHW = FORM & H3_NCHW, GNF = FORM & H3_GNF, GNM = FORM & H3_GNM;
-  constexpr bool ROWIDX = FORM & H3_ROWIDX, PERIMG = FORM & H3_PERIMG;
+  constexpr bool ROWIDX = FORM & H3_ROWIDX, PERIMG = FORM & H3_PERIMG, LNF = FORM & H3_LNF;
+  static_assert(!LNF || !(CONV || GNF || ROWIDX), "H3_LNF: plain fp32 rows (K = 128 or 256: the launcher checks)");
   static_assert(!(ROWIDX || PERIMG) || (NCHW && GNF && !CONV && !RES && !GNM), "H3_ROWIDX / H3_PERIMG: forms of the GroupNorm-folded channel-major projection");
   unsigned long long tm[4];
   if (TIMING) tm[0] = wall_clock64();
@@ -441,6 +501,11 @@
   f32x4 xr[4];
   f32x4 gga = {0.f, 0.f, 0.f, 0.f}, gbe = {0.f, 0.f, 0.f, 0.f};
   float gmean = 0.f, grstd = 0.f;
+  float lmean[4] = {0.f, 0.f, 0.f, 0.f}, lrstd[4] = {0.f, 0.f, 0.f, 0.f};
+  if (LNF) {
+    if (NB == 8) h3_ln_row_stats<8>(xbase, xoff, K, ln.eps, lmean, lrstd);
+    else h3_ln_row_stats<4>(xbase, xoff, K, ln.eps, lmean, lrstd);
+  }
   const float* gmr = GNF ? gn.mr + (int64_t)(m0 / rows_per_image) * gn.G * 2 : nullptr;
   const int last = NB - 1;
   auto gload = [&](int c) {
@@ -455,6 +520,11 @@
       const int g = ch / gn.cpg;
       gmean = gmr[2 * g];
       grstd = gmr[2 * g + 1];
+    }
+    if (LNF) {
+      const int ch = cc * 32 + 4 * (tid & 7);
+      gga = *reinterpret_cast<const f32x4*>(ln.gamma + ch);
+      gbe = *reinterpret_cast<const f32x4*>(ln.beta + ch);
     }
     if (CONV) {
       const int k0 = cc * 32, tap = k0 / cs.Cin, ch0 = k0 - tap * cs.Cin;
@@ -514,6 +584,9 @@
 #endif
 #pragma unroll
       for (int q = 0; q < 4; ++q) buf[xdst + 256 * q] = __builtin_bit_cast(u32x4_t, xst[q]);
+    } else if (LNF) {
+#pragma unroll
+      for (int q = 0; q < 4; ++q) buf[xdst + 256 * q] = __builtin_bit_cast(u32x4_t, rba_ln_apply(xr[q], lmean[q], lrstd[q], gga, gbe));
     } else {
 #pragma unroll
       for (int q = 0; q < 4; ++q) buf[xdst + 256 * q] = __builtin_bit_cast(u32x4_t, xr[q]);
@@ -909,6 +982,7 @@
   GnMoments gm = GnMoments{nullptr, 1, 1, 128};
   int stagger = 0;
   H3Rows rw = H3Rows{nullptr, 0, 0, 0};
+  LnFold ln = LnFold{nullptr, nullptr, 0.f};
 };
 
 inline bool h3_grid(const H3Args& a, int rows, int cols, int& MT, int& NT) {
@@ -932,7 +1006,7 @@
   int MT, NT;
   if (!h3_grid(a, 128, 32 * CT, MT, NT)) return (int)hipErrorInvalidValue;
   hipLaunchKernelGGL((split_linear_h3l_kernel<ACT, CT, FORM>), dim3((unsigned)MT * NT), dim3(256), 0, a.stream, reinterpret_cast<const float*>(a.x), a.wp, a.bias,
-                     reinterpret_cast<float*>(a.out), (int)a.M, a.N, a.K, MT, NT, a.dbg, a.cs, a.res, a.rows_per_image, a.gn, a.gm, a.rw);
+                     reinterpret_cast<float*>(a.out), (int)a.M, a.N, a.K, MT, NT, a.dbg, a.cs, a.res, a.rows_per_image, a.gn, a.gm, a.rw, a.ln);
   return 0;
 }
 
diff --git a/rba_amd/maskformer_model.py b/rba_amd/maskformer_model.py
--- a/rba_amd/maskformer_model.py
+++ b/rba_amd/maskformer_model.py
@@ -72,8 +72,13 @@
         return batch, sizes
 
     @torch.no_grad()
+    def _deferred_norms(self):
+        takes = getattr(self.sem_seg_head.pixel_decoder, "takes_deferred_norm", None)
+        return takes if ops.BOUNDARY_FOLDS and takes is not None and hasattr(self.backbone, "_stages") else None
+
     def _predict_outputs(self, batched_inputs):
         pe = getattr(self.backbone, "patch_embed", None)
+        defer = self._deferred_norms()
         if (self.fused_front_end and pe is not None and hasattr(self.backbone, "forward_images") and pe.fused_ok()
                 and all(x["image"].dim() == 3 and x["image"].shape[0] == 3 and x["image"].dtype in (torch.uint8, torch.float32)
                         for x in batched_inputs)):
@@ -82,10 +87,11 @@
             d = self.size_divisibility
             H = (max(s[0] for s in sizes) + d - 1) // d * d
             W = (max(s[1] for s in sizes) + d - 1) // d * d
-            features = self.backbone.forward_images(images, self._mean3, self._std3, H, W)
+            features = self.backbone.forward_images(images, self._mean3, self._std3, H, W, defer_norm=defer) if defer is not None \
+                else self.backbone.forward_images(images, self._mean3, self._std3, H, W)
             return self.sem_seg_head(features), sizes, (H, W)
         batch, sizes = self.preprocess(batched_inputs)
-        features = self.backbone(batch)
+        features = self.backbone(batch, defer_norm=defer) if defer is not None else self.backbone(batch)
         return self.sem_seg_head(features), sizes, tuple(batch.shape[-2:])
 
     @torch.no_grad()
@@ -288,7 +294,7 @@
         return GraphKey(tuple(image.shape), image.dtype, image.device, torch.cuda.current_stream(image.device).cuda_stream, bool(return_argmax), score,
                         self.fused_upsample, self.fused_front_end, ops.SPLIT_MODE, ops.SPLIT_ACTIVATIONS, ops.TILES_MIN, ops.MLP_FUSED_MIN_ROWS,
                         ops.concurrent_streams(), ops.SWIN_ATTN_FUSED,
-                        (getattr(self.sem_seg_head.predictor, "sparse_intermediate_heads", None), ops.COMPOSED_MASK_HEAD), self._weights_version())
+                        (getattr(self.sem_seg_head.predictor, "sparse_intermediate_heads", None), ops.COMPOSED_MASK_HEAD, ops.BOUNDARY_FOLDS), self._weights_version())
 
     def drop_graphs(self, release_constants=False):
         if release_constants:
diff --git a/rba_amd/modeling/backbone/swin.py b/rba_amd/modeling/backbone/swin.py
--- a/rba_amd/modeling/backbone/swin.py
+++ b/rba_amd/modeling/backbone/swin.py
@@ -194,24 +194,29 @@
     def size_divisibility(self):
         return 32
 
-    def forward_images(self, images, mean, std, Hp, Wp):
-        return self._stages(*self.patch_embed.forward_images(images, mean, std, Hp, Wp))
-
-    def forward(self, x):
+    def forward_images(self, images, mean, std, Hp, Wp, defer_norm=None):
+        return self._stages(*self.patch_embed.forward_images(images, mean, std, Hp, Wp), defer_norm=defer_norm)
+
+    def forward(self, x, defer_norm=None):
         if x.dim() != 4:
             raise ValueError(f"SwinTransformer takes an input of shape (N, C, H, W). Got {tuple(x.shape)} instead!")
-        return self._stages(*self.patch_embed(x))
-
-    def _stages(self, x, Wh, Ww):
+        return self._stages(*self.patch_embed(x), defer_norm=defer_norm)
+
+    def _stages(self, x, Wh, Ww, defer_norm=None):
         outs = {}
         for i, layer in enumerate(self.layers):
             pending = None
             for blk in layer.blocks:
                 x, pending = blk(x, Wh, Ww, pending)
             norm = getattr(self, f"norm{i}")
-            t, tb = pending if pending is not None else (None, None)
-            x, y = ops.add_layer_norm(x, norm.weight, norm.bias, norm.eps, t, tb, inplace_sum=True)
-            outs[f"res{i + 2}"] = y.view(-1, Wh, Ww, self.num_features[i]).permute(0, 3, 1, 2)
+            C = self.num_features[i]
+            if (defer_norm is not None and pending is None and ops.BOUNDARY_FOLDS and ops.SPLIT_MODE == "f16x3" and C in (128, 256)
+                    and x.is_cuda and x.dtype == torch.float32 and x.is_contiguous() and defer_norm(f"res{i + 2}", x.shape[0], C, Wh, Ww)):
+                outs[f"res{i + 2}"] = ops.DeferredLayerNorm(x.view(-1, Wh * Ww, C), norm.weight, norm.bias, norm.eps, (Wh, Ww))
+            else:
+                t, tb = pending if pending is not None else (None, None)
+                x, y = ops.add_layer_norm(x, norm.weight, norm.bias, norm.eps, t, tb, inplace_sum=True)
+                outs[f"res{i + 2}"] = y.view(-1, Wh, Ww, self.num_features[i]).permute(0, 3, 1, 2)
             if layer.downsample is not None:
                 x = layer.downsample(x, Wh, Ww)
                 Wh, Ww = (Wh + 1) // 2, (Ww + 1) // 2
diff --git a/rba_amd/modeling/pixel_decoder/msdeformattn.py b/rba_amd/modeling/pixel_decoder/msdeformattn.py
--- a/rba_amd/modeling/pixel_decoder/msdeformattn.py
+++ b/rba_amd/modeling/pixel_decoder/msdeformattn.py
@@ -202,12 +202,22 @@
             return ops.token_linear(tok, lin, use_bias=use_bias)
         return ops.linear(tok, lin, use_bias=use_bias)
 
+    def takes_deferred_norm(self, f, B, C, h, w):
+        d = self.mask_features.weight.shape[1]
+        return (f in self.in_features[:self.num_fpn_levels] and f not in self.transformer_in_features
+                and ops.linear_gn_stats_takes_ln(B * h * w, d, C, h * w, 32))
+
+    def _resolve_deferred_norms(self, features):
+        if not any(isinstance(x, ops.DeferredLayerNorm) for x in features.values()):
+            return features
+        return {f: x.materialize() if isinstance(x, ops.DeferredLayerNorm) and not self.takes_deferred_norm(f, *x.shape) else x for f, x in features.items()}
+
     def _channels_last_ok(self, features):
         d = self.mask_features.weight.shape[1]
         if d % 32 or (d // 32) % 4 or 256 % (d // 4) or d > 1024:
             return False
         need = set(self.transformer_in_features) | set(self.in_features[:self.num_fpn_levels])
-        return all(self._tokens(features[f]) is not None and features[f].shape[1] % 32 == 0 for f in need)
+        return all((isinstance(features[f], ops.DeferredLayerNorm) or self._tokens(features[f]) is not None) and features[f].shape[1] % 32 == 0 for f in need)
 
     def _encode_channels_last(self, features):
         srcs, pos, tks = [], [], []
@@ -229,8 +239,10 @@
         B, d = prev.shape[0], prev.shape[-1]
         h, w = int(x.shape[-2]), int(x.shape[-1])
         ad, ly = getattr(self, f"adapter_{j}"), getattr(self, f"layer_{j}")
-        tok = self._tokens(x)
-        if tok.is_contiguous() and ops.linear_emits_gn_moments(B * h * w, d, tok.shape[-1], h * w, 32):
+        tok = None if isinstance(x, ops.DeferredLayerNorm) else self._tokens(x)
+        if tok is None:
+            lat, lat_mr = ops.linear_gn_stats(x.tokens, _cached_linear_view(ad), 32, ad.norm.eps, h * w, use_bias=False, ln=x.ln)
+        elif tok.is_contiguous() and ops.linear_emits_gn_moments(B * h * w, d, tok.shape[-1], h * w, 32):
             lat, lat_mr = ops.linear_gn_stats(tok, _cached_linear_view(ad), 32, ad.norm.eps, h * w, use_bias=False)
         else:
             lat = self._conv1x1(tok, ad, use_bias=False)
@@ -274,8 +286,10 @@
         return self._mask_features(prev, prev_norm, defer_mask_features), outs[0], outs[:self.maskformer_num_feature_levels]
 
     def forward_features(self, features, defer_mask_features=False):
+        features = self._resolve_deferred_norms(features)
         if self.num_fpn_levels > 0 and self._channels_last_ok(features):
             return self._forward_features_channels_last(features, defer_mask_features)
+        features = {f: x.materialize() if isinstance(x, ops.DeferredLayerNorm) else x for f, x in features.items()}
         srcs, pos = [], []
         for idx, f in enumerate(self.transformer_in_features[::-1]):
             x = features[f].float().contiguous()
diff --git a/rba_amd/ops.py b/rba_amd/ops.py
--- a/rba_amd/ops.py
+++ b/rba_amd/ops.py
@@ -1386,20 +1386,49 @@
     return mr
 
 
-@_hip_op
-def linear_gn_stats(x, lin, num_groups, eps, rows_per_image, use_bias=True):
+BOUNDARY_FOLDS = os.environ.get("RBA_BOUNDARY_FOLDS", "1") != "0"
+
+
+def linear_gn_stats_takes_ln(M, N, K, rows_per_image, num_groups):
+    return BOUNDARY_FOLDS and K in (128, 256) and linear_emits_gn_moments(M, N, K, rows_per_image, num_groups)
+
+
+class DeferredLayerNorm:
+    __slots__ = ("tokens", "ln", "shape", "_map")
+
+    def __init__(self, tokens, weight, bias, eps, hw):
+        B, P, C = tokens.shape
+        self.tokens, self.ln, self.shape, self._map = tokens, (weight, bias, float(eps)), (B, C, int(hw[0]), int(hw[1])), None
+
+    def materialize(self):
+        if self._map is None:
+            B, C, h, w = self.shape
+            self._map = add_layer_norm(self.tokens, *self.ln)[1].view(B, h, w, C).permute(0, 3, 1, 2)
+        return self._map
+
+
+@_hip_op
+def linear_gn_stats(x, lin, num_groups, eps, rows_per_image, use_bias=True, ln=None):
     _chk(x, "x")
     w = lin.weight
     N, K = w.shape
     M = x.numel() // K
     if not linear_emits_gn_moments(M, N, K, rows_per_image, num_groups) or x.shape[-1] != K:
         raise RbaHipError("linear_gn_stats: check linear_emits_gn_moments(M, N, K, rows_per_image, G) first")
+    if ln is not None and not linear_gn_stats_takes_ln(M, N, K, rows_per_image, num_groups):
+        raise RbaHipError("linear_gn_stats(ln=): check linear_gn_stats_takes_ln(M, N, K, rows_per_image, G) first")
     bias = lin.bias if use_bias else None
     planes = _cached_planes(lin, w)
     B, splits = M // rows_per_image, rows_per_image // 128
     out = torch.empty(tuple(x.shape[:-1]) + (N,), dtype=torch.float32, device=x.device)
     mom = torch.empty((B, num_groups, splits, 3), dtype=torch.float32, device=x.device)
-    _launch("rba_split_linear_f16x3_gn_moments_f32", _p(x), _p(planes), _p(bias), _p(out), M, N, K, rows_per_image, int(num_groups), _p(mom))
+    if ln is not None:
+        _vec(ln[0], "ln weight", K)
+        _vec(ln[1], "ln bias", K)
+        _launch("rba_split_linear_f16x3_ln_gn_moments_f32", _p(x), _p(ln[0]), _p(ln[1]), float(ln[2]), _p(planes), _p(bias), _p(out), M, N, K, rows_per_image,
+                int(num_groups), _p(mom))
+    else:
+        _launch("rba_split_linear_f16x3_gn_moments_f32", _p(x), _p(planes), _p(bias), _p(out), M, N, K, rows_per_image, int(num_groups), _p(mom))
     return out, _merge_gn_moments(mom, B, int(num_groups), splits, eps)
 
 
```

Measured after the change: 152.0, median of 6. Within noise of the previous version (+0.2%).
